# HAHHHD/mllp

Hardware: AMD Instinct MI355X
Metric: LP instances/sec (fwd+bwd) on Netlib batch; achieved HBM GB/s on CSR SpMM (higher is better)
Workload: dtype f32; 1 GPU; netlib_full: BASELINE.json configs[2], 97 instances / 1,074,147 nnz per global batch, one block-diagonal batch per GPU, one Adam step per global batch: fwd + BCE + bwd + gradient all-reduce + Adam, fp32; global_batch=97, instances_rank0=97, nnz_rank0=1074147, hip_graph=False, parallelism=dp1

## Files before the change

### include/mllp_hip.h

```cpp
#ifndef MLLP_HIP_H
#define MLLP_HIP_H

#include <stdint.h>

#ifdef __cplusplus
extern "C" {
#endif

#define MLLP_ABI_VERSION 6
#define MLLP_FEAT 16
#define MLLP_NUM_PARAMS 4721

#define MLLP_OK 0
#define MLLP_EINVAL (-1)
#define MLLP_EHIP (-2)
#define MLLP_ENOMEM (-3)
#define MLLP_ERANGE (-4)

typedef struct mllp_graph mllp_graph_t;

const char* mllp_last_error(void);
int mllp_abi_version(void);


int mllp_graph_create_host(int64_t n_inst, const int64_t* inst_m, const int64_t* inst_n,
                           const int64_t* indptr, const int32_t* indices, const double* values,
                           int32_t tier_wave, int32_t tier_block, mllp_graph_t** out);

int mllp_csr_transpose_device(int64_t n_rows, int64_t n_cols, int64_t nnz, const int32_t* d_ptr, const int32_t* d_idx,
                              const float* d_val, int32_t* d_t_ptr, int32_t* d_t_idx, float* d_t_val, void* stream);

int mllp_graph_create_device(int64_t n_inst, const int64_t* inst_ptr_m, const int64_t* inst_ptr_n,
                             int64_t nnz,
                             const int32_t* d_csr_ptr, const int32_t* d_csr_idx, const float* d_csr_val,
                             const int32_t* d_csc_ptr, const int32_t* d_csc_idx, const float* d_csc_val,
                             int32_t tier_wave, int32_t tier_block, void* stream, mllp_graph_t** out);

int mllp_graph_destroy(mllp_graph_t* g);

int mllp_graph_dims(const mllp_graph_t* g, int64_t dims[12]);

int mllp_graph_export(const mllp_graph_t* g, int which, void* host_dst, int64_t capacity_bytes);

int mllp_graph_set_path(mllp_graph_t* g, int path);

int mllp_graph_invalidate_inputs(mllp_graph_t* g);

int mllp_graph_set_values(mllp_graph_t* g, const float* d_val, void* stream);
int mllp_graph_set_values_bytes(const mllp_graph_t* g, int64_t* bytes);
int mllp_graph_scale_values(mllp_graph_t* g, const float* d_row_scale, const float* d_col_scale, void* stream);

int mllp_graph_normalize(mllp_graph_t* g, float* d_x1, float* d_x2, float rhs_cap, int flags, float* d_row_scale,
                         float* d_obj_scale, void* stream);
int mllp_normalize_row_tier(int64_t row_nnz, int* tier);

int mllp_spmm_csr_f32(const mllp_graph_t* g, int transpose, const float* d_H, float* d_Y, void* stream);
int mllp_spmm_csr_bf16(const mllp_graph_t* g, int transpose, const void* d_H_bf16, float* d_Y, void* stream);

int mllp_graph_build_spmm_copy(mllp_graph_t* g, int transpose, int where, void* stream);
int mllp_graph_drop_spmm_copy(mllp_graph_t* g, int transpose);
int mllp_graph_spmm_copy_info(const mllp_graph_t* g, int transpose, int64_t info[8]);
int mllp_graph_export_spmm_copy(const mllp_graph_t* g, int transpose, int which, void* host_dst, int64_t capacity_bytes);

int mllp_graph_build_stream_copy(mllp_graph_t* g, int transpose, int geom, int where, void* stream);
int mllp_graph_drop_stream_copy(mllp_graph_t* g, int transpose, int geom);
int mllp_graph_stream_copy_info(const mllp_graph_t* g, int transpose, int geom, int64_t info[8]);
int mllp_graph_export_stream_copy(const mllp_graph_t* g, int transpose, int geom, int which, void* host_dst,
                                  int64_t capacity_bytes);

int mllp_tiled_geometry(int variant, int32_t* rows_per_tile, int32_t* cols_per_block, int32_t* bundle_capacity);
int mllp_graph_attach_tiled(mllp_graph_t* g, int transpose, int variant, int64_t n_tiles, int64_t n_tb,
                            int32_t max_blocks_per_tile ,
                            const int32_t* d_tile_blk, const int32_t* d_blk_id, const int32_t* d_ptr2,
                            const int32_t* d_perm, const int32_t* d_ent);
int mllp_graph_build_tiled(mllp_graph_t* g, int transpose, int variant, void* stream);
int mllp_graph_tiled_info(const mllp_graph_t* g, int transpose, int variant, int64_t info[5]);
int mllp_graph_export_tiled(const mllp_graph_t* g, int transpose, int variant, int which, int32_t* d_dst, int64_t count,
                            void* stream);

int mllp_tconv_workspace_floats(const mllp_graph_t* g, int dst_is_var, int cin, int64_t* n_floats);
int mllp_tconv_fwd(const mllp_graph_t* g, int dst_is_var, int cin, const float* d_conv_params,
                   const float* d_x_src, const float* d_x_dst, float* d_h_out, float* d_ws, void* stream);
int mllp_tconv_bwd(const mllp_graph_t* g, int dst_is_var, int cin, const float* d_conv_params,
                   const float* d_x_src, const float* d_x_dst, const float* d_h_out, float* d_ws,
                   float* d_dh, float* d_dx_dst, float* d_dx_src, int accumulate,
                   float* d_param_grads, void* stream);

int mllp_gnn_workspace_bytes(const mllp_graph_t* g, int64_t* bytes);
int mllp_gnn_forward(const mllp_graph_t* g, const float* d_params, const float* d_x1, const float* d_x2,
                     void* d_ws, float* d_logits, void* stream);
int mllp_gnn_backward(const mllp_graph_t* g, const float* d_params, const float* d_x1, const float* d_x2,
                      void* d_ws, const float* d_dlogits, float* d_grads, void* stream);
int mllp_gnn_loss_step(const mllp_graph_t* g, const float* d_params, const float* d_x1, const float* d_x2,
                       const float* d_labels, float inv_batch, void* d_ws, float* d_logits,
                       float* d_loss, float* d_grads, void* stream);

int mllp_gnn_input_grads_scratch_bytes(const mllp_graph_t* g, int64_t* bytes);
int mllp_gnn_backward_inputs(const mllp_graph_t* g, const float* d_params, const float* d_x1, const float* d_x2,
                             void* d_ws, const float* d_dlogits, float* d_grads, float* d_dx1, float* d_dx2,
                             float* d_dvalues, void* d_scratch, void* stream);

int mllp_gnn_input_grads(const mllp_graph_t* g, const float* d_params, const float* d_x1, const float* d_x2,
                         void* d_ws, const float* d_dlogits, float* d_grads, float* d_dx1, float* d_dx2,
                         float* d_dvalues, void* d_scratch, void* stream);
int mllp_gnn_loss_step_inputs(const mllp_graph_t* g, const float* d_params, const float* d_x1, const float* d_x2,
                              const float* d_labels, float inv_batch, void* d_ws, float* d_logits, float* d_loss,
                              float* d_grads, float* d_dx1, float* d_dx2, float* d_dvalues, void* stream);

int mllp_weighted_loss(const mllp_graph_t* g, const float* d_logits, const float* d_labels,
                       const float* d_inst_weight, const float* d_pos_weight, float* d_dlogits,
                       float* d_inst_loss, float* d_loss, void* stream);
int mllp_balanced_pos_weight(const mllp_graph_t* g, const float* d_labels, float* d_pos_weight, void* stream);
int mllp_gnn_loss_step_weighted(const mllp_graph_t* g, const float* d_params, const float* d_x1, const float* d_x2,
                                const float* d_labels, const float* d_inst_weight, const float* d_pos_weight,
                                void* d_ws, float* d_logits, float* d_loss, float* d_inst_loss, float* d_grads,
                                float* d_dlogits, void* stream);

int mllp_adam_step(float* d_params, const float* d_grads, float* d_exp_avg, float* d_exp_avg_sq,
                   float* d_state, float eps, float grad_scale, int64_t n, void* stream);

int mllp_gnn_train_step(const mllp_graph_t* g, float* d_params, const float* d_x1, const float* d_x2,
                        const float* d_labels, float inv_batch, void* d_ws, float* d_logits, float* d_loss,
                        float* d_grads, float* d_exp_avg, float* d_exp_avg_sq, float* d_state, float eps, int flags,
                        void* stream);

int mllp_gnn_small_step_limits(int64_t limits[4]);
int mllp_gnn_small_step_fits(const mllp_graph_t* g, int* fits);
int mllp_gnn_train_step_small(const mllp_graph_t* g, float* d_params, const float* d_x1, const float* d_x2,
                              const float* d_labels, float inv_batch, void* d_ws, float* d_logits, float* d_loss,
                              float* d_grads, float* d_exp_avg, float* d_exp_avg_sq, float* d_state, float eps,
                              void* stream);

int mllp_metrics_scratch_bytes(const mllp_graph_t* g, int64_t* bytes);
int mllp_topm_metrics(const mllp_graph_t* g, const float* d_logits, const float* d_labels,
                      void* d_scratch, float* d_out, void* stream);

int mllp_topm_select(const mllp_graph_t* g, const float* d_logits, uint8_t* d_mask, int32_t* d_index,
                     float* d_stats, void* stream);
int mllp_topm_select_dense(int64_t n, int64_t m, const float* d_logits, uint8_t* d_mask, int32_t* d_index,
                           float* d_stats, void* stream);

typedef struct mllp_lp mllp_lp_t;
int mllp_mps_read(const char* path, int normalize, mllp_lp_t** out);
int mllp_lp_dims(const mllp_lp_t* lp, int64_t dims[6]);
int mllp_lp_export(const mllp_lp_t* lp, int64_t* indptr, int32_t* indices, double* values, double* coefs,
                   double* rhs, int32_t* slack_rows);
int mllp_lp_free(mllp_lp_t* lp);

int mllp_angle_num_params(int feat_dim, int64_t* out);
int mllp_angle_workspace_floats(int64_t n_nodes, int feat_dim, int64_t* out);
int mllp_angle_forward(int64_t n_nodes, int feat_dim, const float* d_cos, const float* d_x, const float* d_params,
                       float* d_ws, float* d_logits, void* stream);
int mllp_angle_backward(int64_t n_nodes, int feat_dim, const float* d_cos, const float* d_x, const float* d_params,
                        float* d_ws, const float* d_dlogits, float* d_grads, void* stream);

int mllp_angle_backward_inputs(int64_t n_nodes, int feat_dim, const float* d_cos, const float* d_x,
                               const float* d_params, float* d_ws, const float* d_dlogits, float* d_grads,
                               float* d_dx, float* d_dcos, void* stream);

#ifdef __cplusplus
}
#endif
#endif
```

### mllp_amd/_lib.py

```python
import ctypes
import os
import subprocess
from ctypes import POINTER, c_char_p, c_double, c_float, c_int, c_int32, c_int64, c_void_p

_HERE = os.path.dirname(os.path.abspath(__file__))
LIB_PATH = os.path.join(_HERE, "csrc", "libmllp_hip.so")
HEADER_PATH = os.path.abspath(os.path.join(_HERE, "..", "include", "mllp_hip.h"))

ABI_VERSION = 6

FEAT = 16
CONV_NAMES = ("gconv1_w2s", "gconv1_s2w", "gconv2_w2s", "gconv2_s2w", "gconv3_w2s", "gconv3_s2w")
CONV_CIN = (1, 1, 16, 16, 16, 16)


def conv_param_count(cin):
    return 4 * FEAT * cin + 5 * FEAT


_CONV_OFFSETS = [0]
for _cin in CONV_CIN:
    _CONV_OFFSETS.append(_CONV_OFFSETS[-1] + conv_param_count(_cin))
FC_OFFSET = _CONV_OFFSETS[-1]
NUM_PARAMS = FC_OFFSET + FEAT + 1


def conv_param_slice(conv):
    i = CONV_NAMES.index(conv) if isinstance(conv, str) else range(len(CONV_NAMES))[conv]
    return slice(_CONV_OFFSETS[i], _CONV_OFFSETS[i + 1])


class MllpError(RuntimeError):
    pass


_PROTOTYPES = {
    "mllp_last_error": (c_char_p, []),
    "mllp_abi_version": (c_int, []),
    "mllp_graph_create_host": (c_int, [c_int64, POINTER(c_int64), POINTER(c_int64), POINTER(c_int64),
                                       POINTER(c_int32), POINTER(c_double), c_int32, c_int32,
                                       POINTER(c_void_p)]),
    "mllp_graph_create_device": (c_int, [c_int64, POINTER(c_int64), POINTER(c_int64), c_int64,
                                         c_void_p, c_void_p, c_void_p, c_void_p, c_void_p, c_void_p,
                                         c_int32, c_int32, c_void_p, POINTER(c_void_p)]),
    "mllp_graph_destroy": (c_int, [c_void_p]),
    "mllp_graph_dims": (c_int, [c_void_p, POINTER(c_int64)]),
    "mllp_graph_export": (c_int, [c_void_p, c_int, c_void_p, c_int64]),
    "mllp_graph_set_path": (c_int, [c_void_p, c_int]),
    "mllp_graph_invalidate_inputs": (c_int, [c_void_p]),
    "mllp_graph_set_values": (c_int, [c_void_p, c_void_p, c_void_p]),
    "mllp_graph_set_values_bytes": (c_int, [c_void_p, POINTER(c_int64)]),
    "mllp_graph_scale_values": (c_int, [c_void_p, c_void_p, c_void_p, c_void_p]),
    "mllp_graph_normalize": (c_int, [c_void_p, c_void_p, c_void_p, c_float, c_int, c_void_p, c_void_p, c_void_p]),
    "mllp_normalize_row_tier": (c_int, [c_int64, POINTER(c_int)]),
    "mllp_graph_build_spmm_copy": (c_int, [c_void_p, c_int, c_int, c_void_p]),
    "mllp_graph_drop_spmm_copy": (c_int, [c_void_p, c_int]),
    "mllp_graph_spmm_copy_info": (c_int, [c_void_p, c_int, POINTER(c_int64)]),
    "mllp_graph_export_spmm_copy": (c_int, [c_void_p, c_int, c_int, c_void_p, c_int64]),
    "mllp_graph_build_stream_copy": (c_int, [c_void_p, c_int, c_int, c_int, c_void_p]),
    "mllp_graph_drop_stream_copy": (c_int, [c_void_p, c_int, c_int]),
    "mllp_graph_stream_copy_info": (c_int, [c_void_p, c_int, c_int, POINTER(c_int64)]),
    "mllp_graph_export_stream_copy": (c_int, [c_void_p, c_int, c_int, c_int, c_void_p, c_int64]),
    "mllp_csr_transpose_device": (c_int, [c_int64, c_int64, c_int64, c_void_p, c_void_p, c_void_p, c_void_p, c_void_p,
                                          c_void_p, c_void_p]),
    "mllp_graph_build_tiled": (c_int, [c_void_p, c_int, c_int, c_void_p]),
    "mllp_graph_tiled_info": (c_int, [c_void_p, c_int, c_int, POINTER(c_int64)]),
    "mllp_graph_export_tiled": (c_int, [c_void_p, c_int, c_int, c_int, c_void_p, c_int64, c_void_p]),
    "mllp_spmm_csr_f32": (c_int, [c_void_p, c_int, c_void_p, c_void_p, c_void_p]),
    "mllp_spmm_csr_bf16": (c_int, [c_void_p, c_int, c_void_p, c_void_p, c_void_p]),
    "mllp_angle_num_params": (c_int, [c_int, POINTER(c_int64)]),
    "mllp_angle_workspace_floats": (c_int, [c_int64, c_int, POINTER(c_int64)]),
    "mllp_angle_forward": (c_int, [c_int64, c_int, c_void_p, c_void_p, c_void_p, c_void_p, c_void_p, c_void_p]),
    "mllp_angle_backward": (c_int, [c_int64, c_int, c_void_p, c_void_p, c_void_p, c_void_p, c_void_p, c_void_p, c_void_p]),
    "mllp_angle_backward_inputs": (c_int, [c_int64, c_int, c_void_p, c_void_p, c_void_p, c_void_p, c_void_p, c_void_p,
                                           c_void_p, c_void_p, c_void_p]),
    "mllp_tiled_geometry": (c_int, [c_int, POINTER(c_int32), POINTER(c_int32), POINTER(c_int32)]),
    "mllp_graph_attach_tiled": (c_int, [c_void_p, c_int, c_int, c_int64, c_int64, c_int32, c_void_p, c_void_p, c_void_p, c_void_p,
                                        c_void_p]),
    "mllp_tconv_workspace_floats": (c_int, [c_void_p, c_int, c_int, POINTER(c_int64)]),
    "mllp_tconv_fwd": (c_int, [c_void_p, c_int, c_int, c_void_p, c_void_p, c_void_p, c_void_p, c_void_p, c_void_p]),
    "mllp_tconv_bwd": (c_int, [c_void_p, c_int, c_int, c_void_p, c_void_p, c_void_p, c_void_p, c_void_p,
                               c_void_p, c_void_p, c_void_p, c_int, c_void_p, c_void_p]),
    "mllp_gnn_workspace_bytes": (c_int, [c_void_p, POINTER(c_int64)]),
    "mllp_gnn_forward": (c_int, [c_void_p, c_void_p, c_void_p, c_void_p, c_void_p, c_void_p, c_void_p]),
    "mllp_gnn_backward": (c_int, [c_void_p, c_void_p, c_void_p, c_void_p, c_void_p, c_void_p, c_void_p, c_void_p]),
    "mllp_gnn_input_grads_scratch_bytes": (c_int, [c_void_p, POINTER(c_int64)]),
    "mllp_gnn_backward_inputs": (c_int, [c_void_p, c_void_p, c_void_p, c_void_p, c_void_p, c_void_p, c_void_p, c_void_p,
                                         c_void_p, c_void_p, c_void_p, c_void_p]),
    "mllp_gnn_input_grads": (c_int, [c_void_p, c_void_p, c_void_p, c_void_p, c_void_p, c_void_p, c_void_p, c_void_p,
                                     c_void_p, c_void_p, c_void_p, c_void_p]),
    "mllp_gnn_loss_step_inputs": (c_int, [c_void_p, c_void_p, c_void_p, c_void_p, c_void_p, c_float, c_void_p, c_void_p,
                                          c_void_p, c_void_p, c_void_p, c_void_p, c_void_p, c_void_p]),
    "mllp_gnn_loss_step": (c_int, [c_void_p, c_void_p, c_void_p, c_void_p, c_void_p, c_float, c_void_p,
                                   c_void_p, c_void_p, c_void_p, c_void_p]),
    "mllp_gnn_train_step": (c_int, [c_void_p, c_void_p, c_void_p, c_void_p, c_void_p, c_float, c_void_p, c_void_p,
                                    c_void_p, c_void_p, c_void_p, c_void_p, c_void_p, c_float, c_int, c_void_p]),
    "mllp_gnn_small_step_limits": (c_int, [POINTER(c_int64)]),
    "mllp_gnn_small_step_fits": (c_int, [c_void_p, POINTER(c_int)]),
    "mllp_gnn_train_step_small": (c_int, [c_void_p, c_void_p, c_void_p, c_void_p, c_void_p, c_float, c_void_p, c_void_p,
                                          c_void_p, c_void_p, c_void_p, c_void_p, c_void_p, c_float, c_void_p]),
    "mllp_weighted_loss": (c_int, [c_void_p, c_void_p, c_void_p, c_void_p, c_void_p, c_void_p, c_void_p, c_void_p, c_void_p]),
    "mllp_balanced_pos_weight": (c_int, [c_void_p, c_void_p, c_void_p, c_void_p]),
    "mllp_gnn_loss_step_weighted": (c_int, [c_void_p, c_void_p, c_void_p, c_void_p, c_void_p, c_void_p, c_void_p, c_void_p,
                                            c_void_p, c_void_p, c_void_p, c_void_p, c_void_p, c_void_p]),
    "mllp_adam_step": (c_int, [c_void_p, c_void_p, c_void_p, c_void_p, c_void_p, c_float, c_float, c_int64,
                               c_void_p]),
    "mllp_metrics_scratch_bytes": (c_int, [c_void_p, POINTER(c_int64)]),
    "mllp_topm_metrics": (c_int, [c_void_p, c_void_p, c_void_p, c_void_p, c_void_p, c_void_p]),
    "mllp_topm_select": (c_int, [c_void_p, c_void_p, c_void_p, c_void_p, c_void_p, c_void_p]),
    "mllp_topm_select_dense": (c_int, [c_int64, c_int64, c_void_p, c_void_p, c_void_p, c_void_p, c_void_p]),
    "mllp_mps_read": (c_int, [c_char_p, c_int, POINTER(c_void_p)]),
    "mllp_lp_dims": (c_int, [c_void_p, POINTER(c_int64)]),
    "mllp_lp_export": (c_int, [c_void_p, c_void_p, c_void_p, c_void_p, c_void_p, c_void_p, c_void_p]),
    "mllp_lp_free": (c_int, [c_void_p]),
}

_lib = None


def build(verbose=False):
    out = subprocess.run(["make", "-C", os.path.join(_HERE, "csrc"), "-j4"], capture_output=True, text=True)
    if verbose or out.returncode != 0:
        print(out.stdout[-4000:])
        print(out.stderr[-4000:])
    if out.returncode != 0:
        raise MllpError("building libmllp_hip.so failed")
    return LIB_PATH


def lib():
    global _lib
    if _lib is None:
        if not os.path.exists(LIB_PATH):
            raise MllpError(f"{LIB_PATH} not found: run `python -c 'import __graft_entry__ as g; g.build()'` "
                            "(or `make -C mllp_amd/csrc`). The product path has no CPU fallback.")
        L = ctypes.CDLL(LIB_PATH)
        for name, (res, args) in _PROTOTYPES.items():
            fn = getattr(L, name)
            fn.restype = res
            fn.argtypes = args
        if L.mllp_abi_version() != ABI_VERSION:
            raise MllpError("libmllp_hip.so ABI version mismatch")
        _lib = L
    return _lib


MLLP_ERANGE = -4


def check(rc):
    if rc != 0:
        msg = lib().mllp_last_error()
        raise MllpError(f"libmllp_hip error {rc}: {msg.decode() if msg else '?'}")


def ptr(t):
    if t is None:
        return c_void_p(0)
    return c_void_p(t.data_ptr())


def np_ptr(a, ctype):
    return a.ctypes.data_as(POINTER(ctype))


def current_stream():
    import torch
    return c_void_p(torch.cuda.current_stream().cuda_stream)
```

### mllp_amd/csrc/api.cpp

```cpp
#include <algorithm>

#include "internal.h"

namespace mllp {

static inline int64_t up16(int64_t x) { return (x + 15) & ~int64_t(15); }

static inline bool al16(const void* p) { return (reinterpret_cast<uintptr_t>(p) & 15) == 0; }
#define REQUIRE_ALIGNED16(cond) REQUIRE(cond, "misaligned pointer: " #cond " (these are accessed in 16-byte pieces)")

ConvWs conv_ws_carve(float* base, int64_t n, int cin, float** end) {
    const int64_t recw = cin == 16 ? REC_W : 8;
    float* p = base;
    auto take = [&](int64_t floats) {
        float* q = p;
        p += up16(floats);
        return q;
    };
    ConvWs w;
    w.derived = take(DERIVED_W);
    w.qp = take(n * cin);
    w.t = take(n);
    w.Z = take(n * cin);
    w.aux = take(n * 4);
// ... 350 lines not shown
                                 void* d_ws, const float* d_dlogits, float* d_grads, void* stream) {
    REQUIRE(g && d_params && d_x1 && d_x2 && d_ws && d_dlogits && d_grads, "null argument");
    REQUIRE_ALIGNED16(al16(d_ws) && al16(d_params) && al16(d_x1) && al16(d_x2));
    hipStream_t s = (hipStream_t)stream;
    ModelWs w = model_ws(g, (float*)d_ws);
    int rc;
    REQUIRE(g->ws_ptr == d_ws && g->ws_path == (use_fused(g) ? 1 : 0),
            "no mllp_gnn_forward on this workspace with the current path (mllp_graph_set_path between forward and backward?)");
    if (use_fused(g)) {
        const FusedModel m{d_params, w, d_x1, d_x2, nullptr, 0.0f, nullptr};
        if ((rc = fused_bind(const_cast<mllp_graph*>(g), d_x1, d_x2, nullptr, s))) return rc;
        if ((rc = fused_head_backward(g, m, d_dlogits, s))) return rc;
        return fused_backward(g, m, false, d_grads, nullptr, s);
    }
    if ((rc = launch_head(1, g->N, w.h3v, d_params + OFF_FC, d_params + OFF_FC + FEAT, g->inv_n, nullptr, 0.0f,
                          d_dlogits, nullptr, w.d3v, w.head_partials, s))) return rc;
    if ((rc = fork_to(s, g->aux, g->ev[1]))) return rc;
    if ((rc = launch_head_finalize(w.head_partials, head_blocks_for(g->N), d_grads + OFF_FC, nullptr, g->aux))) return rc;
    return model_backward_body(g, d_params, d_x1, d_x2, w, d_grads, s);
}

static int input_grads_body(const mllp_graph* g, const float* x1, const float* x2, const ModelWs& w, float* dx1,
                            float* dx2, float* dval, hipStream_t s) {
    int rc;
    auto edge = [&](int c, const float* x_src, int accumulate) {
        const bool t = MODEL_CONV[c].dst_is_var;
        return launch_edge_grad(t ? g->At : g->A, g->nnz, MODEL_CONV[c].cin, w.c[c], x_src, t ? g->at_pos : nullptr, dval,
                                accumulate, s);
    };
    if ((rc = launch_layer1_dst_grads(w.c[CONV_1V], w.d1v, dx1, g->N, w.c[CONV_1C], w.d1c, dx2, g->M, s))) return rc;
    if (dx1 && (rc = launch_attn_bwd_src1(g->At, w.c[CONV_1C], x1, dx1, 1, g->At.scratch, s))) return rc;
    if (dx2 && (rc = launch_attn_bwd_src1(g->A, w.c[CONV_1V], x2, dx2, 1, g->A.scratch, s))) return rc;
    if (!dval) return MLLP_OK;
    if ((rc = edge(CONV_1C, x1, 0)) || (rc = edge(CONV_2C, w.h1v, 1)) || (rc = edge(CONV_1V, x2, 1)) ||
        (rc = edge(CONV_2V, w.h1c, 1))) return rc;
    return edge(CONV_3V, w.h2c, 1);
}

extern "C" int mllp_gnn_loss_step(const mllp_graph_t* g, const float* d_params, const float* d_x1, const float* d_x2,
                                  const float* d_labels, float inv_batch, void* d_ws, float* d_logits, float* d_loss,
                                  float* d_grads, void* stream) {
    REQUIRE(g && d_params && d_x1 && d_x2 && d_labels && d_ws && d_logits && d_loss && d_grads, "null argument");
    REQUIRE_ALIGNED16(al16(d_ws) && al16(d_params) && al16(d_x1) && al16(d_x2));
    hipStream_t s = (hipStream_t)stream;
    ModelWs w = model_ws(g, (float*)d_ws);
    int rc;
    const_cast<mllp_graph*>(g)->folded_ws = const_cast<mllp_graph*>(g)->folded_params = nullptr;
    if (use_fused(g)) {
        const FusedModel m{d_params, w, d_x1, d_x2, d_labels, inv_batch, d_logits};
        if ((rc = fused_forward(const_cast<mllp_graph*>(g), m, 2, s))) return rc;
        return fused_backward(g, m, true, d_grads, d_loss, s);
    }
    if ((rc = model_forward_body(g, d_params, d_x1, d_x2, w, s))) return rc;
    if ((rc = launch_head(2, g->N, w.h3v, d_params + OFF_FC, d_params + OFF_FC + FEAT, g->inv_n, d_labels, inv_batch,
                          nullptr, d_logits, w.d3v, w.head_partials, s))) return rc;
    if ((rc = fork_to(s, g->aux, g->ev[1]))) return rc;
    if ((rc = launch_head_finalize(w.head_partials, head_blocks_for(g->N), d_grads + OFF_FC, d_loss, g->aux))) return rc;
    return model_backward_body(g, d_params, d_x1, d_x2, w, d_grads, s);
}

extern "C" int mllp_gnn_input_grads_scratch_bytes(const mllp_graph_t* g, int64_t* bytes) {
    REQUIRE(g && bytes, "null argument");
    *bytes = up16(MLLP_NUM_PARAMS) * (int64_t)sizeof(float);
    return MLLP_OK;
}

extern "C" int mllp_gnn_backward_inputs(const mllp_graph_t* g, const float* d_params, const float* d_x1,
                                        const float* d_x2, void* d_ws, const float* d_dlogits, float* d_grads,
                                        float* d_dx1, float* d_dx2, float* d_dvalues, void* d_scratch, void* stream) {
    REQUIRE(g && d_params && d_x1 && d_x2 && d_ws && d_dlogits, "null argument");
    REQUIRE_ALIGNED16(al16(d_ws) && al16(d_params) && al16(d_x1) && al16(d_x2));
    REQUIRE(g->ws_ptr == d_ws, "no mllp_gnn_forward on this workspace");
    REQUIRE(g->ws_path == 0, "the forward on this workspace ran on the fused path: input gradients need the generic "
                             "sweeps (mllp_graph_set_path(g, 1) before mllp_gnn_forward)");
    REQUIRE(!use_fused(g), "the graph's path selects the fused kernels: set path 1 between the forward and this call");
    REQUIRE(d_grads || d_scratch, "d_grads and d_scratch are both null (mllp_gnn_input_grads_scratch_bytes)");
    hipStream_t s = (hipStream_t)stream;
    mllp_graph* gm = const_cast<mllp_graph*>(g);
    int rc;
    if (d_dvalues && (rc = ensure_at_pos(gm, s))) return rc;
    float* grads = d_grads ? d_grads : (float*)d_scratch;
    if ((rc = mllp_gnn_backward(g, d_params, d_x1, d_x2, d_ws, d_dlogits, grads, stream))) return rc;
    return input_grads_body(g, d_x1, d_x2, model_ws(g, (float*)d_ws), d_dx1, d_dx2, d_dvalues, s);
}

extern "C" int mllp_gnn_input_grads(const mllp_graph_t* g, const float* d_params, const float* d_x1, const float* d_x2,
                                    void* d_ws, const float* d_dlogits, float* d_grads, float* d_dx1, float* d_dx2,
                                    float* d_dvalues, void* d_scratch, void* stream) {
    REQUIRE(g && d_params && d_x1 && d_x2 && d_ws && d_dlogits, "null argument");
    REQUIRE_ALIGNED16(al16(d_ws) && al16(d_params) && al16(d_x1) && al16(d_x2));
    REQUIRE(d_grads || d_scratch, "d_grads and d_scratch are both null (mllp_gnn_input_grads_scratch_bytes)");
    REQUIRE(g->ws_ptr == d_ws, "no mllp_gnn_forward on this workspace");
    REQUIRE(g->ws_path == (use_fused(g) ? 1 : 0),
            "the path was switched between the forward on this workspace and this call (mllp_graph_set_path)");
    if (!use_fused(g))
        return mllp_gnn_backward_inputs(g, d_params, d_x1, d_x2, d_ws, d_dlogits, d_grads, d_dx1, d_dx2, d_dvalues, d_scratch,
                                        stream);
    hipStream_t s = (hipStream_t)stream;
    int rc;
    if (d_dvalues && (rc = ensure_at_pos(const_cast<mllp_graph*>(g), s))) return rc;
    float* grads = d_grads ? d_grads : (float*)d_scratch;
    if ((rc = mllp_gnn_backward(g, d_params, d_x1, d_x2, d_ws, d_dlogits, grads, stream))) return rc;
    const ModelWs w = model_ws(g, (float*)d_ws);
    return fused_input_grads(g, FusedModel{d_params, w, d_x1, d_x2, nullptr, 0.0f, nullptr}, d_dx1, d_dx2, d_dvalues, s);
}

extern "C" int mllp_gnn_loss_step_inputs(const mllp_graph_t* g, const float* d_params, const float* d_x1,
                                         const float* d_x2, const float* d_labels, float inv_batch, void* d_ws,
                                         float* d_logits, float* d_loss, float* d_grads, float* d_dx1, float* d_dx2,
                                         float* d_dvalues, void* stream) {
    REQUIRE(g && d_params && d_x1 && d_x2 && d_labels && d_ws && d_logits && d_loss && d_grads, "null argument");
    REQUIRE_ALIGNED16(al16(d_ws) && al16(d_params) && al16(d_x1) && al16(d_x2));
    hipStream_t s = (hipStream_t)stream;
    int rc;
    if (d_dvalues && (rc = ensure_at_pos(const_cast<mllp_graph*>(g), s))) return rc;
    if ((rc = mllp_gnn_loss_step(g, d_params, d_x1, d_x2, d_labels, inv_batch, d_ws, d_logits, d_loss, d_grads, stream)))
        return rc;
    const ModelWs w = model_ws(g, (float*)d_ws);
    if (use_fused(g))
        return fused_input_grads(g, FusedModel{d_params, w, d_x1, d_x2, d_labels, inv_batch, d_logits}, d_dx1, d_dx2,
                                 d_dvalues, s);
    return input_grads_body(g, d_x1, d_x2, w, d_dx1, d_dx2, d_dvalues, s);
}

extern "C" int mllp_gnn_train_step(const mllp_graph_t* g, float* d_params, const float* d_x1, const float* d_x2,
                                   const float* d_labels, float inv_batch, void* d_ws, float* d_logits, float* d_loss,
                                   float* d_grads, float* d_exp_avg, float* d_exp_avg_sq, float* d_state, float eps,
                                   int flags, void* stream) {
    REQUIRE(g && d_params && d_x1 && d_x2 && d_labels && d_ws && d_logits && d_loss && d_grads, "null argument");
    REQUIRE_ALIGNED16(al16(d_ws) && al16(d_params) && al16(d_x1) && al16(d_x2));
    REQUIRE(d_exp_avg && d_exp_avg_sq && d_state, "null optimizer state");
    REQUIRE((flags & ~1) == 0, "flags: bit 0 = the folded weights in the workspace are current");
    hipStream_t s = (hipStream_t)stream;
    int rc;
    mllp_graph* gm = const_cast<mllp_graph*>(g);
    if (use_fused(g)) {
        ModelWs w = model_ws(g, (float*)d_ws);
        const FusedModel m{d_params, w, d_x1, d_x2, d_labels, inv_batch, d_logits};
        const bool skip = (flags & 1) != 0 && gm->folded_ws == d_ws && gm->folded_params == d_params;
        gm->folded_ws = gm->folded_params = nullptr;
        if ((rc = fused_forward(gm, m, 2, s, skip))) return rc;
        const FusedAdam a = {d_params, d_exp_avg, d_exp_avg_sq, d_state, eps, (int)MLLP_NUM_PARAMS};
        if ((rc = fused_backward(g, m, true, d_grads, d_loss, s, &a))) return rc;
        gm->folded_ws = d_ws;
        gm->folded_params = d_params;
        return MLLP_OK;
    }
    gm->folded_ws = gm->folded_params = nullptr;
    if ((rc = mllp_gnn_loss_step(g, d_params, d_x1, d_x2, d_labels, inv_batch, d_ws, d_logits, d_loss, d_grads, stream)))
        return rc;
    return launch_adam(d_params, d_grads, d_exp_avg, d_exp_avg_sq, d_state, eps, 1.0f, MLLP_NUM_PARAMS, s);
}

extern "C" int mllp_gnn_small_step_limits(int64_t limits[4]) {
    REQUIRE(limits, "null argument");
    limits[0] = SMALL_STEP_MAX_NODES; limits[1] = SMALL_STEP_MAX_NNZ;
    limits[2] = SMALL_STEP_THREADS; limits[3] = SMALL_STEP_LDS_BYTES;
    return MLLP_OK;
}

static std::string small_step_excess(const mllp_graph* g) {
    if (g->M + g->N > SMALL_STEP_MAX_NODES)
        return "the graph has " + std::to_string(g->M + g->N) + " nodes, the limit is " + std::to_string(SMALL_STEP_MAX_NODES);
    if (g->nnz > SMALL_STEP_MAX_NNZ)
        return "the graph has " + std::to_string(g->nnz) + " nonzeros, the limit is " + std::to_string(SMALL_STEP_MAX_NNZ);
    return std::string();
}

extern "C" int mllp_gnn_small_step_fits(const mllp_graph_t* g, int* fits) {
    REQUIRE(g && fits, "null argument");
    *fits = small_step_excess(g).empty() ? 1 : 0;
    return MLLP_OK;
}

extern "C" int mllp_gnn_train_step_small(const mllp_graph_t* g, float* d_params, const float* d_x1, const float* d_x2,
                                         const float* d_labels, float inv_batch, void* d_ws, float* d_logits,
                                         float* d_loss, float* d_grads, float* d_exp_avg, float* d_exp_avg_sq,
                                         float* d_state, float eps, void* stream) {
    REQUIRE(g && d_params && d_x1 && d_x2 && d_labels && d_ws && d_logits && d_loss && d_grads, "null argument");
    REQUIRE_ALIGNED16(al16(d_ws) && al16(d_params) && al16(d_x1) && al16(d_x2));
    const int n_opt = (d_exp_avg != nullptr) + (d_exp_avg_sq != nullptr) + (d_state != nullptr);
    REQUIRE(n_opt == 0 || n_opt == 3, "optimizer state: give d_exp_avg, d_exp_avg_sq and d_state, or none of them (loss step)");
    const std::string excess = small_step_excess(g);
    REQUIRE(excess.empty(), excess + " (mllp_gnn_small_step_limits)");
    mllp_graph* gm = const_cast<mllp_graph*>(g);
    gm->ws_ptr = nullptr;
    gm->ws_path = -1;
    gm->folded_ws = gm->folded_params = nullptr;
    return launch_small_step(g, d_params, d_x1, d_x2, d_labels, inv_batch, model_ws(g, (float*)d_ws), d_logits, d_loss,
                             d_grads, d_exp_avg, d_exp_avg_sq, d_state, eps, (hipStream_t)stream);
}

extern "C" int mllp_adam_step(float* d_params, const float* d_grads, float* d_exp_avg, float* d_exp_avg_sq,
                              float* d_state, float eps, float grad_scale, int64_t n, void* stream) {
    REQUIRE(d_params && d_grads && d_exp_avg && d_exp_avg_sq && d_state, "null argument");
    REQUIRE(n > 0 && n < (int64_t)1 << 30, "bad parameter count");
    return launch_adam(d_params, d_grads, d_exp_avg, d_exp_avg_sq, d_state, eps, grad_scale, n, (hipStream_t)stream);
}

extern "C" int mllp_metrics_scratch_bytes(const mllp_graph_t* g, int64_t* bytes) {
    REQUIRE(g && bytes, "null argument");
    *bytes = 16;
    return MLLP_OK;
}

extern "C" int mllp_topm_metrics(const mllp_graph_t* g, const float* d_logits, const float* d_labels, void* d_scratch,
                                 float* d_out, void* stream) {
    REQUIRE(g && d_logits && d_labels && d_out, "null argument");
    return launch_topm_metrics(g, d_logits, d_labels, d_scratch, d_out, (hipStream_t)stream);
}

extern "C" int mllp_topm_select(const mllp_graph_t* g, const float* d_logits, uint8_t* d_mask, int32_t* d_index,
                                float* d_stats, void* stream) {
    REQUIRE(g && d_logits, "null argument");
    REQUIRE(d_mask || d_index || d_stats, "null outputs: at least one of mask, index, stats");
    return launch_topm_select(g->inst_ptr_n, g->inst_ptr_m, g->n_inst, 0, 0, d_logits, d_mask, d_index, d_stats,
                              (hipStream_t)stream);
}

extern "C" int mllp_topm_select_dense(int64_t n, int64_t m, const float* d_logits, uint8_t* d_mask, int32_t* d_index,
                                      float* d_stats, void* stream) {
    REQUIRE(n >= 0 && m >= 0, "bad size: n and m must not be negative");
    REQUIRE(d_logits, "null argument");
    REQUIRE(d_mask || d_index || d_stats, "null outputs: at least one of mask, index, stats");
    if (n > INT32_MAX || m > INT32_MAX) return fail(MLLP_ERANGE, "mllp_topm_select_dense: sizes exceed int32 indexing");
    return launch_topm_select(nullptr, nullptr, 1, (int)n, (int)m, d_logits, d_mask, d_index, d_stats,
                              (hipStream_t)stream);
}
```

### mllp_amd/csrc/fused_kernels.hip

```cpp
#include <algorithm>
#include <vector>

#include "device_utils.h"
#include "host_graph.h"
#include "internal.h"
#include "node_bodies.h"

namespace mllp {

typedef float f32x4m __attribute__((ext_vector_type(4)));

#ifdef MLLP_TIMING_BUILD
static int g_fused_abl = [] {
    const char* e = getenv("MLLP_FUSED_ABL");
    return e ? atoi(e) : 0;
}();
#define FUSED_ABL(bit) ((J.abl & (bit)) != 0)
__device__ unsigned long long g_fused_stamps[8192 * 8];
__device__ unsigned long long g_fused_stamps1[8192 * 8];
#define FUSED_STAMP(k)                                                                      \
    {                                                                                       \
        __builtin_amdgcn_sched_barrier(0);                                                  \
        const unsigned long long now_ = __builtin_amdgcn_s_memtime();                       \
        __builtin_amdgcn_sched_barrier(0);                                                  \
        stamp_sum[k] += now_ - stamp_last;                                                  \
        stamp_last = now_;                                                                  \
    }
#else
#define FUSED_ABL(bit) false
#define FUSED_STAMP(k)
#endif

constexpr int FT = 768;
constexpr int FW = FT / 64;
constexpr int RT = 1024;
constexpr int MAXJOBS = 2;

constexpr int NP = FUSED_NP;
static_assert(NP == FUSED_PARTS, "partition count");

struct PartTiers {
    int row0, n_block, n_wave, n_group, n_base;
};
struct ItemsDev {
    const int* __restrict__ sptr;
    const int2* __restrict__ sent;
    const float2* __restrict__ sax;
    int n_dst, nnz;
    const int* __restrict__ order;
    int nw, L;
    PartTiers part[NP];
};

static ItemsDev items_dev(const FusedOrient& o, int which) {
    const bool scalar = which == 1;
    ItemsDev d;
    d.order = which == 0 ? o.lst16 : which == 1 ? o.lst1 : o.lst16x2;
    d.nw = which == 0 ? o.nw16 : which == 1 ? o.nw1 : o.nw16x2;
    d.L = which == 0 ? o.L16 : which == 1 ? o.L1 : o.L16x2;
    d.sptr = o.sptr;
    d.sent = reinterpret_cast<const int2*>(o.sent);
    d.sax = reinterpret_cast<const float2*>(o.sax);
    d.n_dst = o.n_dst;
    d.nnz = o.nnz;
    for (int q = 0; q < NP; ++q) {
        const FusedTiersDev& t = scalar ? o.t1[q] : o.t16[q];
        d.part[q].row0 = o.row0[q];
        d.part[q].n_block = t.n_block; d.part[q].n_wave = t.n_wave; d.part[q].n_group = t.n_group; d.part[q].n_base = t.n_base;
    }
    return d;
}

constexpr int TS = 17;
constexpr int TILE = 16 * TS;
__device__ __forceinline__ void tile_put(float* tile, const float4& v, int lane) {
    float* d = tile + (lane >> 2) * TS + 4 * (lane & 3);
    d[0] = v.x; d[1] = v.y; d[2] = v.z; d[3] = v.w;
}
__device__ __forceinline__ float4 tile_get(const float* tile, int lane) {
    const float* d = tile + (lane >> 2) * TS + 4 * (lane & 3);
    return make_float4(d[0], d[1], d[2], d[3]);
}
__device__ __forceinline__ void tile_rows(const float* tile, int lane, float (&a)[4]) {
#pragma unroll
    for (int s = 0; s < 4; ++s) a[s] = tile[(lane & 15) * TS + 4 * s + (lane >> 4)];
}
__device__ __forceinline__ void tile_cols(const float* tile, int lane, float (&a)[4]) {
#pragma unroll
    for (int s = 0; s < 4; ++s) a[s] = tile[(4 * s + (lane >> 4)) * TS + (lane & 15)];
}
__device__ __forceinline__ void tile_put_result(float* tile, const f32x4m& d, int lane) {
#pragma unroll
    for (int j = 0; j < 4; ++j) tile[(4 * (lane >> 4) + j) * TS + (lane & 15)] = d[j];
}
struct MatB {
    float w[4];
};
__device__ __forceinline__ MatB matB(const float* __restrict__ W, int ld, int lane) {
    MatB b;
#pragma unroll
    for (int s = 0; s < 4; ++s) b.w[s] = W[(lane & 15) * ld + 4 * s + (lane >> 4)];
    return b;
}
__device__ __forceinline__ MatB matB_t(const float* __restrict__ W, int ld, int lane) {
    MatB b;
#pragma unroll
    for (int s = 0; s < 4; ++s) b.w[s] = W[(4 * s + (lane >> 4)) * ld + (lane & 15)];
    return b;
}
__device__ __forceinline__ void matB_store(float* lds, const MatB& b, int lane) {
    *reinterpret_cast<float4*>(lds + 4 * lane) = make_float4(b.w[0], b.w[1], b.w[2], b.w[3]);
}
__device__ __forceinline__ MatB matB_lds(const float* lds, int lane) {
    const float4 v = *reinterpret_cast<const float4*>(lds + 4 * lane);
    MatB b;
    b.w[0] = v.x; b.w[1] = v.y; b.w[2] = v.z; b.w[3] = v.w;
    return b;
}
__device__ __forceinline__ f32x4m mat_apply(const float (&a)[4], const MatB& b, f32x4m acc) {
#pragma unroll
    for (int s = 0; s < 4; ++s) acc = __builtin_amdgcn_mfma_f32_16x16x4f32(a[s], b.w[s], acc, 0, 0, 0);
    return acc;
}
__device__ __forceinline__ f32x4m splat4(float v) { return (f32x4m){v, v, v, v}; }
__device__ __forceinline__ float4 lds4(const float* p) { return *reinterpret_cast<const float4*>(p); }
__device__ __forceinline__ float4 f4zero() { return make_float4(0.f, 0.f, 0.f, 0.f); }
__device__ __forceinline__ float4 f4scale(const float4& a, float s) { return make_float4(a.x * s, a.y * s, a.z * s, a.w * s); }
__device__ __forceinline__ float4 f4add(const float4& a, const float4& b) { return make_float4(a.x + b.x, a.y + b.y, a.z + b.z, a.w + b.w); }
template <int J>
__device__ __forceinline__ int quad_bcast_i(int v) {
    return __builtin_amdgcn_mov_dpp(v, J * 0x55, 0xF, 0xF, true);
}
__device__ __forceinline__ float wave_sum(float v) {
    v = row16_sum(v);
    v += __shfl_xor(v, 16, 64);
    v += __shfl_xor(v, 32, 64);
    return v;
}


struct RowSlot {
    int row;
    int first;
    int stride;
    int end;
    int mode;
    bool writer;
};
struct SlotReq {
    int row, q, stride, mode;
    int sb, se;
    bool writer;
};
template <int G>
struct Geo {
    static constexpr int U = 64 / G;
    static constexpr int QG = 4;
    static constexpr int RG = U / QG;
};
template <int G>
__device__ __forceinline__ int wave_items(const PartTiers& s) {
    return s.n_wave + (s.n_group + Geo<G>::RG - 1) / Geo<G>::RG + (s.n_base + Geo<G>::U - 1) / Geo<G>::U;
}
template <int G>
__device__ __forceinline__ SlotReq item_request(const ItemsDev& S, const PartTiers& s, int item, int lane) {
    constexpr int U = Geo<G>::U, QG = Geo<G>::QG, RG = Geo<G>::RG;
    const int unit = lane / G;
    const int n_gitems = (s.n_group + RG - 1) / RG;
    SlotReq r;
    bool valid;
    if (item < s.n_wave) {
        r.row = s.row0 + s.n_block + item; r.q = unit; r.stride = U; r.mode = 2; valid = true; r.writer = unit == 0;
    } else if (item < s.n_wave + n_gitems) {
        const int rl = (item - s.n_wave) * RG + unit / QG;
        valid = rl < s.n_group;
        r.row = s.row0 + s.n_block + s.n_wave + rl; r.q = unit % QG; r.stride = QG; r.mode = 1; r.writer = valid && r.q == 0;
    } else {
        const int rl = (item - s.n_wave - n_gitems) * U + unit;
        valid = rl < s.n_base;
        r.row = s.row0 + s.n_block + s.n_wave + s.n_group + rl; r.q = 0; r.stride = 1; r.mode = 0; r.writer = valid;
    }
    const int rc = valid ? r.row : 0;
    r.sb = S.sptr[rc];
    r.se = S.sptr[rc + 1];
    if (!valid) r.row = -1;
    return r;
}
__device__ __forceinline__ SlotReq empty_request() {
    SlotReq r;
    r.row = -1; r.q = 0; r.stride = 1; r.mode = 0; r.sb = 0; r.se = 0; r.writer = false;
    return r;
}
__device__ __forceinline__ RowSlot slot_make(const SlotReq& q) {
    RowSlot r;
    r.row = q.row; r.first = q.sb + q.q; r.stride = q.stride; r.end = q.row >= 0 ? q.se : 0; r.mode = q.mode; r.writer = q.writer;
    asm volatile("" : "+v"(r.first), "+v"(r.end));
    return r;
}
template <int G>
__device__ __forceinline__ RowSlot item_slot(const ItemsDev& S, const PartTiers& s, int item, int lane) {
    return slot_make(item_request<G>(S, s, item, lane));
}
template <int G>
__device__ __forceinline__ RowSlot block_slot(const ItemsDev& s, int k, int tid) {
    RowSlot r;
    r.row = k;
    r.mode = 3;
    r.first = s.sptr[k] + tid / G;
    r.stride = FT / G;
    r.end = s.sptr[k + 1];
    r.writer = tid < G;
    return r;
}
__device__ __forceinline__ int slot_count(const RowSlot& r) {
    return r.first < r.end ? (r.end - r.first + r.stride - 1) / r.stride : 0;
}
__device__ __forceinline__ RowSlot empty_slot() {
    RowSlot r;
    r.row = -1; r.first = 0; r.stride = 1; r.end = 0; r.mode = 0; r.writer = false;
    return r;
}
struct WaveList {
    const int* p;
    int L, chunk;
};
__device__ __forceinline__ WaveList wave_list(const ItemsDev& S, int px, int gw) {
    WaveList w;
    w.L = gw < S.nw ? S.L : 0;
    w.p = S.order + ((size_t)px * S.nw + gw) * S.L;
    w.chunk = -1;
    return w;
}
__device__ __forceinline__ void wave_list_chunk(WaveList& w, int c0, int lane) {
    int v = c0 + lane < w.L ? w.p[c0 + lane] : -1;
    asm volatile("s_waitcnt vmcnt(0)" : "+v"(v));
    w.chunk = v;
}
__device__ __forceinline__ int wave_list_get(const WaveList& w, int k) {
    return k < 64 ? __builtin_amdgcn_readlane(w.chunk, __builtin_amdgcn_readfirstlane(k)) : -1;
}
template <int LPE>
__device__ __forceinline__ int2 first_entries(const ItemsDev& s, const RowSlot& r, int part) {
    const int k = LPE == 4 ? part : (part & 1);
    return k < slot_count(r) ? s.sent[r.first + k * r.stride] : make_int2(0, 0);
}
template <int LPE>
__device__ __forceinline__ int2 first_entries_any(const ItemsDev& s, const RowSlot& r, int part) {
    const int k = LPE == 4 ? part : (part & 1);
    return s.sent[max(min(r.first + k * r.stride, s.nnz - 1), 0)];
}
__device__ __forceinline__ float shared_sum4(float v, int mode) {
    return mode == 1 ? quads_sum<16>(v) : quads_sum<64>(v);
}
__device__ __forceinline__ float shared_max4(float v, int mode) {
    return mode == 1 ? quads_max<16>(v) : quads_max<64>(v);
}
__device__ __forceinline__ float shared_sum1(float v, int mode) { return mode == 1 ? quad_sum(v) : wave_sum(v); }
__device__ __forceinline__ float shared_max1(float v, int mode) { return mode == 1 ? quad_max(v) : group_max<64>(v); }

struct FwdJob16 {
    ItemsDev s;
    const float* __restrict__ x_src;
    const float* __restrict__ x_dst;
    const float* __restrict__ D;
    ConvParams p;
    float* __restrict__ h;
    float* __restrict__ Z;
    float* __restrict__ aux;
    int head;
    const float* __restrict__ fcw;
    const float* __restrict__ fcb;
    const float* __restrict__ inv_n;
    const float* __restrict__ labels;
    const int* __restrict__ perm;
    float inv_batch;
    float* __restrict__ logits;
    float* __restrict__ g_out;
    float* __restrict__ head_part;
#ifdef MLLP_TIMING_BUILD
    int abl;
#endif
};
struct FwdLaunch16 {
    FwdJob16 job[MAXJOBS];
    int n_jobs;
};
struct FwdW16 {
    float BPq[256], BWv[256], BWs[256];
    float pq0[16], Pt[16], bv[16], we[16], bs[16], fcw[16];
    float pt0, fcb;
};
struct SoftState {
    float4 Z;
    float m, L, u;
};

struct Gather4 {
    float4 x0, x1, x2, x3;
    float a0, a1, a2, a3;
};
__device__ __forceinline__ void gather4_issue(const ItemsDev& s, const float* __restrict__ X, const RowSlot& r, int n_mine,
                                              int k0, int part, int2& en, Gather4& g) {
    const int colm = en.x;
    const float am = __int_as_float(en.y);
    const int c0 = quad_bcast_i<0>(colm), c1 = quad_bcast_i<1>(colm), c2 = quad_bcast_i<2>(colm), c3 = quad_bcast_i<3>(colm);
    g.a0 = quad_bcast<0>(am); g.a1 = quad_bcast<1>(am); g.a2 = quad_bcast<2>(am); g.a3 = quad_bcast<3>(am);
    g.x0 = ld4(X + (size_t)c0 * 16 + 4 * part);
    g.x1 = ld4(X + (size_t)c1 * 16 + 4 * part);
    g.x2 = ld4(X + (size_t)c2 * 16 + 4 * part);
    g.x3 = ld4(X + (size_t)c3 * 16 + 4 * part);
    const int kn = k0 + 4 + part;
    en = kn < n_mine ? s.sent[r.first + kn * r.stride] : make_int2(0, 0);
}

__device__ __forceinline__ void fwd16_step(const Gather4& g, int k0, int n_mine, const float4& qp, float t, SoftState& st) {
    const bool ok0 = k0 < n_mine, ok1 = k0 + 1 < n_mine, ok2 = k0 + 2 < n_mine, ok3 = k0 + 3 < n_mine;
    const float d0 = ok0 ? fmaf(g.a0, t, quad_sum(dot4(qp, g.x0))) : NEG_BIG;
    const float d1 = ok1 ? fmaf(g.a1, t, quad_sum(dot4(qp, g.x1))) : NEG_BIG;
    const float d2 = ok2 ? fmaf(g.a2, t, quad_sum(dot4(qp, g.x2))) : NEG_BIG;
    const float d3 = ok3 ? fmaf(g.a3, t, quad_sum(dot4(qp, g.x3))) : NEG_BIG;
// ... 95 lines not shown
    asm volatile("" : "+v"(nx.xd.x), "+v"(nx.xd.y), "+v"(nx.xd.z), "+v"(nx.xd.w), "+v"(nx.en.x), "+v"(nx.en.y),
                      "+v"(nx.lrow), "+v"(nx.q.sb), "+v"(nx.q.se));
    fwd16_flush(J, pend, part);
    const int lrow_cur = lrow;
    FUSED_STAMP(3)

    if (r.mode >= 1) soft_merge(st, r.mode);
    if (r.mode == 3) {
        const int wave = threadIdx.x >> 6;
        if (lane < 4) {
            float* slot = merge_lds + wave * 20;
            if (part == 0) *reinterpret_cast<float4*>(slot) = make_float4(st.m, st.L, st.u, 0.0f);
            *reinterpret_cast<float4*>(slot + 4 + 4 * part) = st.Z;
        }
        __syncthreads();
        float M = NEG_BIG;
        for (int w = 0; w < FW; ++w) M = fmaxf(M, merge_lds[w * 20]);
        float L = 0.0f, u = 0.0f;
        float4 Z = f4zero();
        for (int w = 0; w < FW; ++w) {
            const float4 hd = lds4(merge_lds + w * 20);
            const float f = exp_acc(hd.x - M);
            L = fmaf(f, hd.y, L);
            u = fmaf(f, hd.z, u);
            fma4(f, lds4(merge_lds + w * 20 + 4 + 4 * part), Z);
        }
        st.m = M; st.L = L; st.u = u; st.Z = Z;
        __syncthreads();
    }
    const bool writer = r.writer;
    const float rinv = 1.0f / (st.L + 1e-16f);
    const float S = st.L * rinv, un = st.u * rinv;
    const float4 zn = f4scale(st.Z, rinv);
    float4 o;
    {
        float ax_[4], az_[4];
        tile_rows(tiles, lane, ax_);
        tile_put(tiles + TILE, zn, lane);
        tile_rows(tiles + TILE, lane, az_);
        if (!FUSED_ABL(512))
        tile_put_result(tiles + 2 * TILE,
                        mat_apply(ax_, matB_lds(W.BWs, lane), mat_apply(az_, matB_lds(W.BWv, lane), splat4(0.0f))), lane);
        o = tile_get(tiles + 2 * TILE, lane);
    }
    o = f4add(o, lds4(W.bs + 4 * part));
    fma4(S, lds4(W.bv + 4 * part), o);
    fma4(un, lds4(W.we + 4 * part), o);
    const float4 hv = make_float4(fmaxf(o.x, 0.0f), fmaxf(o.y, 0.0f), fmaxf(o.z, 0.0f), fmaxf(o.w, 0.0f));
    FUSED_STAMP(4)
    pend.row = writer ? r.row : -1;
    pend.zn = zn; pend.hv = hv; pend.lrow = lrow_cur;
    pend.aux = make_float4(un, st.L > 0.0f ? st.m : 0.0f, rinv, S);
    pend.z = 0.0f; pend.g = f4zero();
    if (J.head) {
        const float4 fw = lds4(W.fcw + 4 * part);
        const float z = quad_sum(dot4(hv, fw)) + W.fcb;
        pend.z = z;
        if (J.head == 2 && writer) {
            const float y = J.labels[r.row];
            const float wn = J.inv_n[r.row] * J.inv_batch;
            const float e = expf(-fabsf(z));
            const float sig = z >= 0.0f ? 1.0f / (1.0f + e) : e / (1.0f + e);
            const float dz = wn * (sig - y);
            pend.g = make_float4(hv.x > 0.0f ? dz * fw.x : 0.0f, hv.y > 0.0f ? dz * fw.y : 0.0f,
                                 hv.z > 0.0f ? dz * fw.z : 0.0f, hv.w > 0.0f ? dz * fw.w : 0.0f);
            fma4(dz, hv, ha.w);
            if (part == 0) {
                ha.b += dz;
                ha.l += wn * (fmaxf(z, 0.0f) - z * y + log1pf(e));
            }
        }
    }
    FUSED_STAMP(5)
}

template <int NW>
__device__ __forceinline__ void head_partials_store(HeadAcc& ha, float* head_lds, float* head_part, int tid) {
    const int lane = tid & 63, wave = tid >> 6;
    ha.w.x = quads_sum<64>(ha.w.x); ha.w.y = quads_sum<64>(ha.w.y);
    ha.w.z = quads_sum<64>(ha.w.z); ha.w.w = quads_sum<64>(ha.w.w);
    ha.b = wave_sum(ha.b);
    ha.l = wave_sum(ha.l);
    if (lane < 4) {
        float* d = head_lds + wave * 18 + 4 * lane;
        d[0] = ha.w.x; d[1] = ha.w.y; d[2] = ha.w.z; d[3] = ha.w.w;
    }
    if (lane == 0) { head_lds[wave * 18 + 16] = ha.b; head_lds[wave * 18 + 17] = ha.l; }
    __syncthreads();
    if (tid < 18) {
        float v = 0.0f;
        for (int w = 0; w < NW; ++w) v += head_lds[w * 18 + tid];
        head_part[(size_t)blockIdx.x * 18 + tid] = v;
    }
}

__global__ __launch_bounds__(FT) void fused_fwd16_kernel(FwdLaunch16 A) {
    __shared__ FwdW16 Ws_[MAXJOBS];
    __shared__ float merge_lds[FW * 20];
    __shared__ float head_lds[FW * 18];
    __shared__ float tiles_[FW * 3 * TILE];
    const int tid = threadIdx.x, lane = tid & 63, wave = tid >> 6, part = lane & 3;
    for (int j = 0; j < A.n_jobs; ++j) {
        const FwdJob16& J = A.job[j];
        FwdW16& W = Ws_[j];
        if (wave == 0) matB_store(W.BPq, matB(J.D + OFF_PQ, 16, lane), lane);
        if (wave == 1) matB_store(W.BWv, matB(J.p.Wv, 16, lane), lane);
        if (wave == 2) matB_store(W.BWs, matB(J.p.Ws, 16, lane), lane);
        if (tid < 16) {
            W.pq0[tid] = J.D[OFF_PQ0 + tid];
            W.Pt[tid] = J.D[OFF_PT + tid];
            W.bv[tid] = J.p.bv[tid];
            W.we[tid] = J.p.we[tid];
            W.bs[tid] = J.p.bs[tid];
            W.fcw[tid] = J.head ? J.fcw[tid] : 0.0f;
        }
        if (tid == 0) {
            W.pt0 = J.D[OFF_PT0];
            W.fcb = J.head ? J.fcb[0] : 0.0f;
        }
    }
    __syncthreads();
    float* tiles = tiles_ + wave * 3 * TILE;
    HeadAcc ha;
    ha.w = f4zero(); ha.b = 0.0f; ha.l = 0.0f;
#ifdef MLLP_TIMING_BUILD
    unsigned long long stamp_sum[8] = {0, 0, 0, 0, 0, 0, 0, 0};
    unsigned long long stamp_last = __builtin_amdgcn_s_memtime();
    const unsigned long long stamp_begin = stamp_last;
#define STAMP_ARGS , stamp_sum, stamp_last
#else
#define STAMP_ARGS
#endif
    const int px = blockIdx.x % NP, bi = blockIdx.x / NP, gp = gridDim.x / NP;
    const int gw = bi * FW + wave;
    float* head_part = nullptr;
    for (int j = 0; j < A.n_jobs; ++j) {
        const FwdJob16& J = A.job[j];
        const PartTiers P = J.s.part[px];
        if (J.head == 2) head_part = J.head_part;
        const RowSlot none = empty_slot();
        FwdPending pend;
        pend.row = -1;
        for (int k = bi; k < P.n_block; k += gp) {
            const RowSlot r = block_slot<4>(J.s, P.row0 + k, tid);
            const float4 xd = ld4(J.x_dst + (size_t)r.row * 16 + 4 * part);
            int2 en = first_entries<4>(J.s, r, part);
            const int lrow = J.head ? J.perm[r.row] : 0;
            FwdNext nx;
            fwd16_row(J, Ws_[j], P, r, xd, en, lrow, empty_request(), -1, nx, pend, part, lane, merge_lds, tiles, ha STAMP_ARGS);
        }
        WaveList wl = wave_list(J.s, px, gw);
        for (int c0 = 0; c0 < wl.L; c0 += 64) {
            wave_list_chunk(wl, c0, lane);
            int it = wave_list_get(wl, 0), it1 = wave_list_get(wl, 1);
            RowSlot r = it >= 0 ? item_slot<4>(J.s, P, it, lane) : none;
            float4 xd = r.row >= 0 ? ld4(J.x_dst + (size_t)r.row * 16 + 4 * part) : f4zero();
            int2 en = first_entries<4>(J.s, r, part);
            int lrow = (J.head && r.row >= 0) ? J.perm[r.row] : 0;
            SlotReq q1 = item_request<4>(J.s, P, max(it1, 0), lane);
            if (it1 < 0) q1.row = -1;
            asm volatile("" : "+v"(xd.x), "+v"(xd.y), "+v"(xd.z), "+v"(xd.w), "+v"(en.x), "+v"(en.y), "+v"(lrow),
                              "+v"(q1.sb), "+v"(q1.se));
            for (int k = 0; it >= 0; ++k) {
                const int it2 = wave_list_get(wl, k + 2);
                FwdNext nx;
                fwd16_row(J, Ws_[j], P, r, xd, en, lrow, q1, it2, nx, pend, part, lane, merge_lds, tiles, ha STAMP_ARGS);
#ifdef MLLP_TIMING_BUILD
                stamp_sum[7] += 1;
#endif
                r = nx.r; xd = nx.xd; en = nx.en; lrow = nx.lrow; q1 = nx.q;
                it = it1; it1 = it2;
            }
        }
        fwd16_flush(J, pend, part);
    }
#ifdef MLLP_TIMING_BUILD
    if (lane == 0 && A.job[0].abl >= 0) {
        stamp_sum[6] = __builtin_amdgcn_s_memtime() - stamp_begin;
        unsigned long long* d = g_fused_stamps + (size_t)(blockIdx.x * FW + wave) * 8;
        for (int k = 0; k < 8; ++k) d[k] = stamp_sum[k];
    }
#endif
    if (head_part) head_partials_store<FW>(ha, head_lds, head_part, tid);
}

struct FwdJob1 {
    ItemsDev s;
    const float* __restrict__ x_dst;
    const float* __restrict__ D;
    ConvParams p;
    float* __restrict__ h;
    float* __restrict__ Z;
    float* __restrict__ aux;
};
struct FwdLaunch1 {
    FwdJob1 job[MAXJOBS];
    int n_jobs;
};
struct alignas(16) FwdW1 {
    float wv[16], ws[16], bv[16], we[16], bs[16];
    float pq, pq0, pt, pt0;
};
struct Soft1 {
    float m, L, u, Z;
};

struct Ent8 {
    float2 e0, e1, e2, e3, e4, e5, e6, e7;
};
__device__ __forceinline__ void ent8_load(const ItemsDev& s, const RowSlot& r, int k0, Ent8& E) {
    const int last = max(s.nnz - 1, 0), d = r.stride, b = r.first + k0 * d;
    E.e0 = s.sax[min(b, last)];         E.e1 = s.sax[min(b + d, last)];
    E.e2 = s.sax[min(b + 2 * d, last)]; E.e3 = s.sax[min(b + 3 * d, last)];
    E.e4 = s.sax[min(b + 4 * d, last)]; E.e5 = s.sax[min(b + 5 * d, last)];
    E.e6 = s.sax[min(b + 6 * d, last)]; E.e7 = s.sax[min(b + 7 * d, last)];
}

__device__ __forceinline__ void fwd1_step4(const float2& e0, const float2& e1, const float2& e2, const float2& e3, int k0,
                                           int n_mine, float qp, float t, Soft1& st) {
    const bool ok0 = k0 < n_mine, ok1 = k0 + 1 < n_mine, ok2 = k0 + 2 < n_mine, ok3 = k0 + 3 < n_mine;
    const float d0 = ok0 ? fmaf(qp, e0.y, e0.x * t) : NEG_BIG, d1 = ok1 ? fmaf(qp, e1.y, e1.x * t) : NEG_BIG;
    const float d2 = ok2 ? fmaf(qp, e2.y, e2.x * t) : NEG_BIG, d3 = ok3 ? fmaf(qp, e3.y, e3.x * t) : NEG_BIG;
    const float mi = fmaxf(fmaxf(d0, d1), fmaxf(d2, d3));
    if (__any(mi > st.m)) {
        const float mn = fmaxf(st.m, mi);
        const float sc = exp_acc(st.m - mn);
        st.L *= sc; st.u *= sc; st.Z *= sc;
        st.m = mn;
    }
    const float p0 = ok0 ? exp_acc(d0 - st.m) : 0.0f, p1 = ok1 ? exp_acc(d1 - st.m) : 0.0f;
    const float p2 = ok2 ? exp_acc(d2 - st.m) : 0.0f, p3 = ok3 ? exp_acc(d3 - st.m) : 0.0f;
    st.L += (p0 + p1) + (p2 + p3);
    st.u = fmaf(p0, e0.x, fmaf(p1, e1.x, fmaf(p2, e2.x, fmaf(p3, e3.x, st.u))));
    st.Z = fmaf(p0, e0.y, fmaf(p1, e1.y, fmaf(p2, e2.y, fmaf(p3, e3.y, st.Z))));
}
__device__ __forceinline__ void fwd1_edges(const ItemsDev& s, const RowSlot& r, float qp, float t, Soft1& st, Ent8& E) {
    const int n_mine = slot_count(r);
    for (int k0 = 0; __any(k0 < n_mine); k0 += 8) {
        Ent8 N;
        const bool more = __any(k0 + 8 < n_mine);
        if (more) ent8_load(s, r, k0 + 8, N);
        fwd1_step4(E.e0, E.e1, E.e2, E.e3, k0, n_mine, qp, t, st);
        if (__any(k0 + 4 < n_mine)) fwd1_step4(E.e4, E.e5, E.e6, E.e7, k0 + 4, n_mine, qp, t, st);
        if (more) E = N;
    }
}

__device__ __forceinline__ void fwd1_row(const FwdJob1& J, const FwdW1& W, const RowSlot& r, int lane, float* merge_lds) {
    Ent8 E;
    ent8_load(J.s, r, 0, E);
    const float x = J.x_dst[max(r.row, 0)];
    const float qp = fmaf(W.pq, x, W.pq0), t = fmaf(W.pt, x, W.pt0);
    Soft1 st;
    st.m = NEG_BIG; st.L = 0.0f; st.u = 0.0f; st.Z = 0.0f;
    fwd1_edges(J.s, r, qp, t, st, E);
    if (r.mode >= 1) {
        const float M = shared_max1(st.m, r.mode);
        const float f = exp_acc(st.m - M);
        st.m = M;
        st.L = shared_sum1(st.L * f, r.mode);
        st.u = shared_sum1(st.u * f, r.mode);
        st.Z = shared_sum1(st.Z * f, r.mode);
    }
    if (r.mode == 3) {
        const int wave = threadIdx.x >> 6;
        if (lane == 0) *reinterpret_cast<float4*>(merge_lds + wave * 4) = make_float4(st.m, st.L, st.u, st.Z);
        __syncthreads();
        float M = NEG_BIG;
        for (int w = 0; w < FW; ++w) M = fmaxf(M, merge_lds[w * 4]);
        float L = 0.0f, u = 0.0f, Z = 0.0f;
        for (int w = 0; w < FW; ++w) {
            const float4 hd = lds4(merge_lds + w * 4);
            const float f = exp_acc(hd.x - M);
            L = fmaf(f, hd.y, L);
            u = fmaf(f, hd.z, u);
            Z = fmaf(f, hd.w, Z);
        }
        st.m = M; st.L = L; st.u = u; st.Z = Z;
        __syncthreads();
    }
    const float rinv = 1.0f / (st.L + 1e-16f);
    const float S = st.L * rinv, un = st.u * rinv, zn = st.Z * rinv;
    if (r.mode == 0) {
        const int base_row = __builtin_amdgcn_readfirstlane(r.row);
        const int n_valid = __popcll(__ballot(r.row >= 0));
#pragma unroll
        for (int q = 0; q < 4; ++q) {
            const int idx = lane + 64 * q, row_l = idx >> 2, ch = (idx & 3) * 4;
            const float Sr = __shfl(S, row_l, 64), ur = __shfl(un, row_l, 64), zr = __shfl(zn, row_l, 64), xr = __shfl(x, row_l, 64);
            float4 v = lds4(W.bs + ch);
            fma4(Sr, lds4(W.bv + ch), v);
            fma4(ur, lds4(W.we + ch), v);
            fma4(zr, lds4(W.wv + ch), v);
            fma4(xr, lds4(W.ws + ch), v);
            if (row_l < n_valid)
                *reinterpret_cast<float4*>(J.h + (size_t)(base_row + row_l) * 16 + ch) =
                    make_float4(fmaxf(v.x, 0.0f), fmaxf(v.y, 0.0f), fmaxf(v.z, 0.0f), fmaxf(v.w, 0.0f));
        }
        if (r.writer) {
            J.Z[r.row] = zn;
            reinterpret_cast<float4*>(J.aux)[r.row] = make_float4(un, st.L > 0.0f ? st.m : 0.0f, rinv, S);
        }
        return;
    }
    if (!r.writer) return;
    float o[16];
#pragma unroll
    for (int c = 0; c < 16; ++c) {
        float v = W.bs[c];
        v = fmaf(S, W.bv[c], v);
        v = fmaf(un, W.we[c], v);
        v = fmaf(W.wv[c], zn, v);
        v = fmaf(W.ws[c], x, v);
        o[c] = fmaxf(v, 0.0f);
    }
    float4* hd = reinterpret_cast<float4*>(J.h + (size_t)r.row * 16);
    hd[0] = make_float4(o[0], o[1], o[2], o[3]);
    hd[1] = make_float4(o[4], o[5], o[6], o[7]);
    hd[2] = make_float4(o[8], o[9], o[10], o[11]);
    hd[3] = make_float4(o[12], o[13], o[14], o[15]);
    J.Z[r.row] = zn;
    reinterpret_cast<float4*>(J.aux)[r.row] = make_float4(un, st.L > 0.0f ? st.m : 0.0f, rinv, S);
}

__global__ __launch_bounds__(FT) void fused_fwd1_kernel(FwdLaunch1 A) {
    __shared__ FwdW1 Ws_[MAXJOBS];
    __shared__ float merge_lds[FW * 4];
    const int tid = threadIdx.x, lane = tid & 63, wave = tid >> 6;
    for (int j = 0; j < A.n_jobs; ++j) {
        const FwdJob1& J = A.job[j];
        FwdW1& W = Ws_[j];
        if (tid < 16) {
            W.wv[tid] = J.p.Wv[tid]; W.ws[tid] = J.p.Ws[tid];
            W.bv[tid] = J.p.bv[tid]; W.we[tid] = J.p.we[tid]; W.bs[tid] = J.p.bs[tid];
        }
        if (tid == 0) {
            W.pq = J.D[OFF_PQ]; W.pq0 = J.D[OFF_PQ0]; W.pt = J.D[OFF_PT]; W.pt0 = J.D[OFF_PT0];
        }
    }
    __syncthreads();
    const int px = blockIdx.x % NP, bi = blockIdx.x / NP, gp = gridDim.x / NP;
    const int gw = bi * FW + wave;
    for (int j = 0; j < A.n_jobs; ++j) {
        const FwdJob1& J = A.job[j];
        const PartTiers P = J.s.part[px];
        for (int k = bi; k < P.n_block; k += gp)
            fwd1_row(J, Ws_[j], block_slot<1>(J.s, P.row0 + k, tid), lane, merge_lds);
        WaveList wl = wave_list(J.s, px, gw);
        for (int c0 = 0; c0 < wl.L; c0 += 64) {
            wave_list_chunk(wl, c0, lane);
            int it = wave_list_get(wl, 0);
            SlotReq q = item_request<1>(J.s, P, max(it, 0), lane);
            for (int k = 0; it >= 0; ++k) {
                const int itn = wave_list_get(wl, k + 1);
                const RowSlot r = slot_make(q);
                q = item_request<1>(J.s, P, max(itn, 0), lane);
                fwd1_row(J, Ws_[j], r, lane, merge_lds);
                it = itn;
            }
        }
    }
}

struct BwdJob16 {
    ItemsDev s;
    const float* __restrict__ x_src;
    const float* __restrict__ x_dst;
    const float* __restrict__ D;
    ConvParams p;
    const float* __restrict__ h;
    const float* __restrict__ dh_a;
    const float* __restrict__ dh_b;
    const float* __restrict__ Z;
    const float* __restrict__ aux;
    float* __restrict__ rec;
    float* __restrict__ dx_dst;
    int mask_dx;
    float* __restrict__ stats;
#ifdef MLLP_TIMING_BUILD
    int abl;
#endif
};
struct BwdLaunch16 {
    BwdJob16 job[MAXJOBS];
    int n_jobs;
};
struct BwdW16 {
    float BWvT[256], BPq[256], BWsT[256], BPqT[256];
    float pq0[16], Pt[16], Pb[16], bv[16], we[16];
    float pt0;
};
struct BwdState {
    float4 dq;
    float ds, dt;
};

__device__ __forceinline__ void bwd16_step(const Gather4& g, int k0, int n_mine, const float4& qp, const float4& gv, float t,
                                           float m, float rinv, float ge, float cc, BwdState& st) {
#define MLLP_BWD_SLOT(K, A_, X_)                                                           \
    {                                                                                      \
        const float l_ = fmaf(A_, t, quad_sum(dot4(qp, X_)));                              \
        const float al_ = (k0 + K < n_mine) ? exp_acc(l_ - m) * rinv : 0.0f;               \
        const float dl_ = al_ * (quad_sum(dot4(gv, X_)) + fmaf(A_, ge, cc));               \
        st.ds += dl_;                                                                      \
        st.dt = fmaf(dl_, A_, st.dt);                                                      \
        fma4(dl_, X_, st.dq);                                                              \
    }
    MLLP_BWD_SLOT(0, g.a0, g.x0)
    MLLP_BWD_SLOT(1, g.a1, g.x1)
    MLLP_BWD_SLOT(2, g.a2, g.x2)
    MLLP_BWD_SLOT(3, g.a3, g.x3)
#undef MLLP_BWD_SLOT
}

struct BwdRow {
    float4 ga, gb, h, x, Z, ax;
};
__device__ __forceinline__ void bwd16_fetch(const BwdJob16& J, const RowSlot& r, int part, BwdRow& d) {
    const bool have = r.row >= 0;
    const size_t ro = have ? (size_t)r.row * 16 + 4 * part : 0;
    const float4 z4 = f4zero();
    d.ga = have ? ld4(J.dh_a + ro) : z4;
    d.gb = (J.dh_b && have) ? ld4(J.dh_b + ro) : z4;
    d.h = (J.h && have) ? ld4(J.h + ro) : make_float4(1.0f, 1.0f, 1.0f, 1.0f);
    d.x = have ? ld4(J.x_dst + ro) : z4;
    d.Z = have ? ld4(J.Z + ro) : z4;
    d.ax = have ? reinterpret_cast<const float4*>(J.aux)[r.row] : z4;
}

constexpr int TB_G = 0, TB_X = 1, TB_Z = 2, TB_DQ = 3, TB_SC = 4, TB_E = 5, TB_N = 6;

__device__ __forceinline__ void bwd16_row(const BwdJob16& J, const BwdW16& W, const PartTiers& P, const RowSlot& r,
                                          BwdRow& rd, int2& en, int itn, RowSlot& rn, int part,
                                          int lane, float* merge_lds, float* tiles, f32x4m (&acc)[STAT_TILES]) {
    const bool have = r.row >= 0;
    const bool writer = r.writer;
    const int n_mine = FUSED_ABL(1) ? 0 : slot_count(r);
    Gather4 gt;
    gather4_issue(J.s, J.x_src, r, n_mine, 0, part, en, gt);
    SlotReq qn = item_request<4>(J.s, P, max(itn, 0), lane);
    if (itn < 0) qn.row = -1;
    const int xpos = (rd.x.x > 0.0f ? 1 : 0) | (rd.x.y > 0.0f ? 2 : 0) | (rd.x.z > 0.0f ? 4 : 0) | (rd.x.w > 0.0f ? 8 : 0);
    float4 qp, gv;
    float t, m, rinv, ge, cc;
    {
        float4 g = f4add(rd.ga, rd.gb);
        g = make_float4(rd.h.x > 0.0f ? g.x : 0.0f, rd.h.y > 0.0f ? g.y : 0.0f, rd.h.z > 0.0f ? g.z : 0.0f, rd.h.w > 0.0f ? g.w : 0.0f);
        const float4 xd = rd.x, Zn = rd.Z, ax = rd.ax;
        float ag_[4], ax_[4];
        tile_put(tiles + TB_G * TILE, g, lane);
        tile_put(tiles + TB_X * TILE, xd, lane);
        tile_put(tiles + TB_Z * TILE, Zn, lane);
        tile_put(tiles + TB_E * TILE, (have && part == 0) ? make_float4(1.0f, ax.w, ax.x, 0.0f) : f4zero(), lane);
        tile_rows(tiles + TB_G * TILE, lane, ag_);
        tile_rows(tiles + TB_X * TILE, lane, ax_);
        if (!FUSED_ABL(16)) {
            tile_put_result(tiles + TB_DQ * TILE, mat_apply(ag_, matB_lds(W.BWvT, lane), splat4(0.0f)), lane);
            tile_put_result(tiles + TB_SC * TILE, mat_apply(ax_, matB_lds(W.BPq, lane), splat4(W.pq0[lane & 15])), lane);
        }
        gv = tile_get(tiles + TB_DQ * TILE, lane);
        qp = tile_get(tiles + TB_SC * TILE, lane);
        t = quad_sum(dot4(lds4(W.Pt + 4 * part), xd)) + W.pt0;
        ge = quad_sum(dot4(g, lds4(W.we + 4 * part)));
        const float gb = quad_sum(dot4(g, lds4(W.bv + 4 * part)));
        const float Dn = quad_sum(dot4(gv, Zn)) + gb * ax.w + ge * ax.x;
        cc = gb - Dn;
        m = ax.y; rinv = ax.z;
    }
    BwdState st;
    st.dq = f4zero(); st.ds = 0.0f; st.dt = 0.0f;
    for (int k0 = 0;;) {
        bwd16_step(gt, k0, n_mine, qp, gv, t, m, rinv, ge, cc, st);
        k0 += 4;
        if (!__any(k0 < n_mine)) break;
        gather4_issue(J.s, J.x_src, r, n_mine, k0, part, en, gt);
    }
    if (writer && J.rec && !FUSED_ABL(8)) {
        float* rr = J.rec + (size_t)r.row * REC_W;
        *reinterpret_cast<float4*>(rr + 4 * part) = qp;
        *reinterpret_cast<float4*>(rr + 16 + 4 * part) = gv;
        if (part == 0) *reinterpret_cast<float4*>(rr + 32) = make_float4(t, m, rinv, ge);
        if (part == 1) *reinterpret_cast<float4*>(rr + 36) = make_float4(cc, 0.0f, 0.0f, 0.0f);
    }
    rn = slot_make(qn);
    bwd16_fetch(J, rn, part, rd);
    en = first_entries<4>(J.s, rn, part);
    if (r.mode >= 1) {
        st.ds = shared_sum4(st.ds, r.mode);
        st.dt = shared_sum4(st.dt, r.mode);
        st.dq.x = shared_sum4(st.dq.x, r.mode); st.dq.y = shared_sum4(st.dq.y, r.mode);
        st.dq.z = shared_sum4(st.dq.z, r.mode); st.dq.w = shared_sum4(st.dq.w, r.mode);
    }
    if (r.mode == 3) {
        const int wave = threadIdx.x >> 6;
        if (lane < 4) {
            float* slot = merge_lds + wave * 20;
            if (part == 0) *reinterpret_cast<float4*>(slot) = make_float4(st.ds, st.dt, 0.0f, 0.0f);
            *reinterpret_cast<float4*>(slot + 4 + 4 * part) = st.dq;
        }
        __syncthreads();
        float ds = 0.0f, dt = 0.0f;
        float4 dq = f4zero();
        for (int w = 0; w < FW; ++w) {
            ds += merge_lds[w * 20];
            dt += merge_lds[w * 20 + 1];
            dq = f4add(dq, lds4(merge_lds + w * 20 + 4 + 4 * part));
        }
        st.ds = ds; st.dt = dt; st.dq = dq;
        __syncthreads();
        if (threadIdx.x >= 64) return;
    }
    tile_put(tiles + TB_DQ * TILE, st.dq, lane);
    if (J.dx_dst && !FUSED_ABL(4)) {
        float ag_[4], adq_[4];
        tile_rows(tiles + TB_G * TILE, lane, ag_);
        tile_rows(tiles + TB_DQ * TILE, lane, adq_);
        tile_put_result(tiles + TB_SC * TILE,
                        mat_apply(adq_, matB_lds(W.BPqT, lane), mat_apply(ag_, matB_lds(W.BWsT, lane), splat4(0.0f))), lane);
        float4 v = tile_get(tiles + TB_SC * TILE, lane);
        fma4(st.ds, lds4(W.Pb + 4 * part), v);
        fma4(st.dt, lds4(W.Pt + 4 * part), v);
        if (J.mask_dx) {
            if (!(xpos & 1)) v.x = 0.0f;
            if (!(xpos & 2)) v.y = 0.0f;
            if (!(xpos & 4)) v.z = 0.0f;
            if (!(xpos & 8)) v.w = 0.0f;
        }
        if (writer) *reinterpret_cast<float4*>(J.dx_dst + (size_t)r.row * 16 + 4 * part) = v;
    }
    if (FUSED_ABL(2)) return;
    if (r.mode >= 1 && !writer) {
        const float4 z4 = f4zero();
        tile_put(tiles + TB_G * TILE, z4, lane);
        tile_put(tiles + TB_X * TILE, z4, lane);
        tile_put(tiles + TB_Z * TILE, z4, lane);
        tile_put(tiles + TB_E * TILE, z4, lane);
        tile_put(tiles + TB_DQ * TILE, z4, lane);
    }
    tile_put(tiles + TB_SC * TILE, (writer && part == 0) ? make_float4(st.ds, st.dt, 0.0f, 0.0f) : f4zero(), lane);
    float cg[4], cdq[4], csc[4], cx[4], cz[4], ce[4];
    if (FUSED_ABL(64)) {
        for (int s = 0; s < 4; ++s) { cg[s] = cdq[s] = csc[s] = cx[s] = cz[s] = ce[s] = (float)lane; }
    } else {
    tile_cols(tiles + TB_G * TILE, lane, cg);
    tile_cols(tiles + TB_DQ * TILE, lane, cdq);
    tile_cols(tiles + TB_SC * TILE, lane, csc);
    tile_cols(tiles + TB_X * TILE, lane, cx);
    tile_cols(tiles + TB_Z * TILE, lane, cz);
    tile_cols(tiles + TB_E * TILE, lane, ce);
    }
    if (FUSED_ABL(32)) {
        asm volatile("" :: "v"(cg[0]), "v"(cdq[1]), "v"(csc[2]), "v"(cx[3]), "v"(cz[0]), "v"(ce[1]));
        return;
    }
#pragma unroll
    for (int s = 0; s < 4; ++s) {
        acc[0] = __builtin_amdgcn_mfma_f32_16x16x4f32(cg[s], cx[s], acc[0], 0, 0, 0);
        acc[1] = __builtin_amdgcn_mfma_f32_16x16x4f32(cg[s], cz[s], acc[1], 0, 0, 0);
        acc[2] = __builtin_amdgcn_mfma_f32_16x16x4f32(cg[s], ce[s], acc[2], 0, 0, 0);
        acc[3] = __builtin_amdgcn_mfma_f32_16x16x4f32(cdq[s], cx[s], acc[3], 0, 0, 0);
        acc[4] = __builtin_amdgcn_mfma_f32_16x16x4f32(cdq[s], ce[s], acc[4], 0, 0, 0);
        acc[5] = __builtin_amdgcn_mfma_f32_16x16x4f32(csc[s], cx[s], acc[5], 0, 0, 0);
        acc[6] = __builtin_amdgcn_mfma_f32_16x16x4f32(csc[s], ce[s], acc[6], 0, 0, 0);
    }
}

__global__ __launch_bounds__(FT) void fused_bwd16_kernel(BwdLaunch16 A) {
    __shared__ BwdW16 Ws_[MAXJOBS];
    __shared__ float merge_lds[FW * 20];
    __shared__ float tiles_[FW * TB_N * TILE];
    const int tid = threadIdx.x, lane = tid & 63, wave = tid >> 6, part = lane & 3;
    for (int j = 0; j < A.n_jobs; ++j) {
        const BwdJob16& J = A.job[j];
        BwdW16& W = Ws_[j];
        if (wave == 0) matB_store(W.BWvT, matB_t(J.p.Wv, 16, lane), lane);
        if (wave == 1) matB_store(W.BPq, matB(J.D + OFF_PQ, 16, lane), lane);
        if (wave == 2) matB_store(W.BWsT, matB_t(J.p.Ws, 16, lane), lane);
        if (wave == 3) matB_store(W.BPqT, matB_t(J.D + OFF_PQ, 16, lane), lane);
        if (tid < 16) {
            W.pq0[tid] = J.D[OFF_PQ0 + tid];
            W.Pt[tid] = J.D[OFF_PT + tid];
            W.Pb[tid] = J.D[OFF_PB + tid];
            W.bv[tid] = J.p.bv[tid];
            W.we[tid] = J.p.we[tid];
        }
        if (tid == 0) W.pt0 = J.D[OFF_PT0];
    }
    __syncthreads();
    float* tiles = tiles_ + wave * TB_N * TILE;
    const int px = blockIdx.x % NP, bi = blockIdx.x / NP, gp = gridDim.x / NP;
    const int gw = bi * FW + wave;
    for (int j = 0; j < A.n_jobs; ++j) {
        const BwdJob16& J = A.job[j];
        const PartTiers P = J.s.part[px];
        f32x4m acc[STAT_TILES];
#pragma unroll
        for (int i = 0; i < STAT_TILES; ++i) acc[i] = splat4(0.0f);
        const RowSlot none = empty_slot();
        for (int k = bi; k < P.n_block; k += gp) {
            const RowSlot r = block_slot<4>(J.s, P.row0 + k, tid);
            BwdRow rd;
            bwd16_fetch(J, r, part, rd);
            int2 en = first_entries<4>(J.s, r, part);
            RowSlot rn;
            bwd16_row(J, Ws_[j], P, r, rd, en, -1, rn, part, lane, merge_lds, tiles, acc);
        }
        WaveList wl = wave_list(J.s, px, gw);
        for (int c0 = 0; c0 < wl.L; c0 += 64) {
            wave_list_chunk(wl, c0, lane);
            int it = wave_list_get(wl, 0);
            RowSlot r = it >= 0 ? item_slot<4>(J.s, P, it, lane) : none;
            BwdRow rd;
            bwd16_fetch(J, r, part, rd);
            int2 en = first_entries<4>(J.s, r, part);
            for (int k = 0; it >= 0; ++k) {
                const int itn = wave_list_get(wl, k + 1);
                RowSlot rn;
                bwd16_row(J, Ws_[j], P, r, rd, en, itn, rn, part, lane, merge_lds, tiles, acc);
                r = rn;
                it = itn;
            }
        }
        __syncthreads();
        float* red = tiles_;
#pragma unroll
        for (int i = 0; i < STAT_TILES; ++i) {
#pragma unroll
            for (int q = 0; q < 4; ++q) red[wave * 256 + ((lane >> 4) * 4 + q) * 16 + (lane & 15)] = acc[i][q];
            __syncthreads();
            if (tid < 256) {
                float v = 0.0f;
                for (int w = 0; w < FW; ++w) v += red[w * 256 + tid];
                J.stats[(size_t)blockIdx.x * STAT_FLOATS + i * 256 + tid] = v;
            }
            __syncthreads();
        }
    }
}

struct SrcJob16 {
    ItemsDev s;
    const float* __restrict__ x;
    const float* __restrict__ rec;
    float* __restrict__ dx;
    const float* __restrict__ addp;
    float addw;
    int mask;
};
struct SrcLaunch16 {
    SrcJob16 job[MAXJOBS];
    int n_jobs;
};

__device__ __forceinline__ void src16_row(const SrcJob16& J, const RowSlot& r, float4& xj_io, int2& en, const SlotReq& qn,
                                          RowSlot& rn, int part, int lane, float* merge_lds) {
    const int n_mine = slot_count(r);
    const float4 xj = xj_io;
    const float4 addv = ld4(J.addp + (size_t)max(r.row, 0) * 16 + 4 * part);
    float4 acc = f4zero();
    for (int k0 = 0; __any(k0 < n_mine); k0 += 2) {
        const int colm = en.x;
        const float am = __int_as_float(en.y);
        const int c0 = quad_bcast_i<0>(colm), c1 = quad_bcast_i<1>(colm);
        const float a0 = quad_bcast<0>(am), a1 = quad_bcast<1>(am);
        const bool ok0 = k0 < n_mine, ok1 = k0 + 1 < n_mine;
        const float* rr0 = J.rec + (size_t)c0 * REC_W;
        const float* rr1 = J.rec + (size_t)c1 * REC_W;
        const float4 q0 = ld4(rr0 + 4 * part), g0 = ld4(rr0 + 16 + 4 * part), s0 = ld4(rr0 + 32);
        const float cc0 = rr0[36];
        const float4 q1 = ld4(rr1 + 4 * part), g1 = ld4(rr1 + 16 + 4 * part), s1 = ld4(rr1 + 32);
        const float cc1 = rr1[36];
        const int kn = k0 + 2 + (part & 1);
        en = kn < n_mine ? J.s.sent[r.first + kn * r.stride] : make_int2(0, 0);
        {
            const float l = fmaf(a0, s0.x, quad_sum(dot4(q0, xj)));
            const float al = ok0 ? exp_acc(l - s0.y) * s0.z : 0.0f;
            const float dl = al * (quad_sum(dot4(g0, xj)) + fmaf(a0, s0.w, cc0));
            fma4(al, g0, acc);
            fma4(dl, q0, acc);
        }
        {
            const float l = fmaf(a1, s1.x, quad_sum(dot4(q1, xj)));
            const float al = ok1 ? exp_acc(l - s1.y) * s1.z : 0.0f;
            const float dl = al * (quad_sum(dot4(g1, xj)) + fmaf(a1, s1.w, cc1));
            fma4(al, g1, acc);
            fma4(dl, q1, acc);
        }
    }
    rn = slot_make(qn);
    xj_io = rn.row >= 0 ? ld4(J.x + (size_t)rn.row * 16 + 4 * part) : f4zero();
    en = first_entries<2>(J.s, rn, part);
    if (r.mode >= 1) {
        acc.x = shared_sum4(acc.x, r.mode); acc.y = shared_sum4(acc.y, r.mode);
        acc.z = shared_sum4(acc.z, r.mode); acc.w = shared_sum4(acc.w, r.mode);
    }
    if (r.mode == 3) {
        const int wave = threadIdx.x >> 6;
        if (lane < 4) *reinterpret_cast<float4*>(merge_lds + wave * 20 + 4 * part) = acc;
        __syncthreads();
        float4 v = f4zero();
        for (int w = 0; w < FW; ++w) v = f4add(v, lds4(merge_lds + w * 20 + 4 * part));
        acc = v;
        __syncthreads();
    }
    fma4(J.addw, addv, acc);
    if (J.mask) {
        if (!(xj.x > 0.0f)) acc.x = 0.0f;
        if (!(xj.y > 0.0f)) acc.y = 0.0f;
        if (!(xj.z > 0.0f)) acc.z = 0.0f;
        if (!(xj.w > 0.0f)) acc.w = 0.0f;
    }
    if (r.writer) *reinterpret_cast<float4*>(J.dx + (size_t)r.row * 16 + 4 * part) = acc;
}

__global__ __launch_bounds__(FT) void fused_src16_kernel(SrcLaunch16 A) {
    __shared__ float merge_lds[FW * 20];
    const int tid = threadIdx.x, lane = tid & 63, wave = tid >> 6, part = lane & 3;
    const int px = blockIdx.x % NP, bi = blockIdx.x / NP, gp = gridDim.x / NP;
    const int gw = bi * FW + wave;
    for (int j = 0; j < A.n_jobs; ++j) {
        const SrcJob16& J = A.job[j];
        const PartTiers P = J.s.part[px];
        const RowSlot none = empty_slot();
        for (int k = bi; k < P.n_block; k += gp) {
            const RowSlot r = block_slot<4>(J.s, P.row0 + k, tid);
            float4 xj = ld4(J.x + (size_t)r.row * 16 + 4 * part);
            int2 en = first_entries<2>(J.s, r, part);
            RowSlot rn;
            src16_row(J, r, xj, en, empty_request(), rn, part, lane, merge_lds);
        }
        WaveList wl = wave_list(J.s, px, gw);
        for (int c0 = 0; c0 < wl.L; c0 += 64) {
            wave_list_chunk(wl, c0, lane);
            int it = wave_list_get(wl, 0);
            RowSlot r = it >= 0 ? item_slot<4>(J.s, P, it, lane) : none;
            float4 xj = r.row >= 0 ? ld4(J.x + (size_t)r.row * 16 + 4 * part) : f4zero();
            int2 en = first_entries<2>(J.s, r, part);
            for (int k = 0; it >= 0; ++k) {
                const int itn = wave_list_get(wl, k + 1);
                const SlotReq qn = itn >= 0 ? item_request<4>(J.s, P, itn, lane) : empty_request();
                RowSlot rn;
                src16_row(J, r, xj, en, qn, rn, part, lane, merge_lds);
                r = rn;
                it = itn;
            }
        }
    }
}

struct BwdJob1 {
    ItemsDev s;
    const float* __restrict__ x_dst;
    const float* __restrict__ D;
    ConvParams p;
    const float* __restrict__ g;
    const float* __restrict__ Z;
    const float* __restrict__ aux;
    float* __restrict__ stats;
};
struct BwdLaunch1 {
    BwdJob1 job[MAXJOBS];
    int n_jobs;
};
struct alignas(16) BwdW1 {
    float wv[16], bv[16], we[16];
    float pq, pq0, pt, pt0;
};
constexpr int G1S = 17, R1S = 9;
constexpr int TILE1 = 64 * G1S + 64 * R1S;

__device__ __forceinline__ void bwd1_row(const BwdJob1& J, const BwdW1& W, const RowSlot& r, int lane, float* merge_lds,
                                         float* tiles, f32x4m& accT, float (&accS)[6]
#ifdef MLLP_TIMING_BUILD
                                         , unsigned long long (&stamp_sum)[8], unsigned long long& stamp_last
#endif
) {
    FUSED_STAMP(0)
    const bool writer = r.writer;
    Ent8 E;
    ent8_load(J.s, r, 0, E);
    const int rowc = max(r.row, 0);
    float gv = 0.0f, ge = 0.0f, gb = 0.0f;
    if (r.mode == 0) {
        const int base_row = __builtin_amdgcn_readfirstlane(r.row);
        const int n_valid = __popcll(__ballot(r.row >= 0));
        float* gt = tiles;
        float* rt = tiles + 64 * G1S;
#pragma unroll
        for (int q = 0; q < 4; ++q) {
            const int idx = lane + 64 * q, row_l = idx >> 2, ch = (idx & 3) * 4;
            const size_t ro = (size_t)min(base_row + row_l, J.s.n_dst - 1) * 16 + ch;
            const float4 a = ld4(J.g + ro);
            const bool on = row_l < n_valid;
            const float4 g = make_float4(on ? a.x : 0.0f, on ? a.y : 0.0f, on ? a.z : 0.0f, on ? a.w : 0.0f);
            const float pv = quad_sum(dot4(g, lds4(W.wv + ch))), pe = quad_sum(dot4(g, lds4(W.we + ch)));
            const float pb = quad_sum(dot4(g, lds4(W.bv + ch)));
            float* d = gt + row_l * G1S + ch;
            d[0] = g.x; d[1] = g.y; d[2] = g.z; d[3] = g.w;
            if ((lane & 3) == 0) { rt[row_l * R1S + 5] = pv; rt[row_l * R1S + 6] = pe; rt[row_l * R1S + 7] = pb; }
        }
        gv = rt[lane * R1S + 5]; ge = rt[lane * R1S + 6]; gb = rt[lane * R1S + 7];
    } else {
        const float4* pa = reinterpret_cast<const float4*>(J.g + (size_t)rowc * 16);
        float* gt = tiles + lane * G1S;
#pragma unroll
        for (int q = 0; q < 4; ++q) {
            const float4 a = pa[q];
            const float g0 = a.x, g1 = a.y, g2 = a.z, g3 = a.w;
            gv = fmaf(g0, W.wv[4 * q], fmaf(g1, W.wv[4 * q + 1], fmaf(g2, W.wv[4 * q + 2], fmaf(g3, W.wv[4 * q + 3], gv))));
            ge = fmaf(g0, W.we[4 * q], fmaf(g1, W.we[4 * q + 1], fmaf(g2, W.we[4 * q + 2], fmaf(g3, W.we[4 * q + 3], ge))));
            gb = fmaf(g0, W.bv[4 * q], fmaf(g1, W.bv[4 * q + 1], fmaf(g2, W.bv[4 * q + 2], fmaf(g3, W.bv[4 * q + 3], gb))));
            gt[4 * q] = writer ? g0 : 0.0f;
            gt[4 * q + 1] = writer ? g1 : 0.0f;
            gt[4 * q + 2] = writer ? g2 : 0.0f;
            gt[4 * q + 3] = writer ? g3 : 0.0f;
        }
    }
    const float x = J.x_dst[rowc];
    const float Zn = J.Z[rowc];
    const float4 ax = reinterpret_cast<const float4*>(J.aux)[rowc];
    {
        float* rt = tiles + 64 * G1S + lane * R1S;
        rt[0] = writer ? x : 0.0f;
        rt[1] = writer ? Zn : 0.0f;
        rt[2] = writer ? 1.0f : 0.0f;
        rt[3] = writer ? ax.w : 0.0f;
        rt[4] = writer ? ax.x : 0.0f;
    }
    const float Dn = gv * Zn + gb * ax.w + ge * ax.x;
    const float cc = gb - Dn;
    const float qp = fmaf(W.pq, x, W.pq0), t = fmaf(W.pt, x, W.pt0);
    float ds = 0.0f, dt = 0.0f, dq = 0.0f;
    const int n_mine = slot_count(r);
    FUSED_STAMP(1)
    for (int k0 = 0; __any(k0 < n_mine); k0 += 8) {
        Ent8 N;
        const bool more = __any(k0 + 8 < n_mine);
        if (more) ent8_load(J.s, r, k0 + 8, N);
#define MLLP_BWD1_SLOT(K, E_)                                                              \
    {                                                                                      \
        const float l_ = fmaf(qp, E_.y, E_.x * t);                                         \
        const float al_ = (K) < n_mine ? exp_acc(l_ - ax.y) * ax.z : 0.0f;                 \
        const float dl_ = al_ * fmaf(gv, E_.y, fmaf(E_.x, ge, cc));                        \
        ds += dl_;                                                                         \
        dt = fmaf(dl_, E_.x, dt);                                                          \
        dq = fmaf(dl_, E_.y, dq);                                                          \
    }
        MLLP_BWD1_SLOT(k0, E.e0)
        MLLP_BWD1_SLOT(k0 + 1, E.e1)
        MLLP_BWD1_SLOT(k0 + 2, E.e2)
        MLLP_BWD1_SLOT(k0 + 3, E.e3)
        if (__any(k0 + 4 < n_mine)) {
            MLLP_BWD1_SLOT(k0 + 4, E.e4)
            MLLP_BWD1_SLOT(k0 + 5, E.e5)
            MLLP_BWD1_SLOT(k0 + 6, E.e6)
            MLLP_BWD1_SLOT(k0 + 7, E.e7)
        }
#undef MLLP_BWD1_SLOT
        if (more) E = N;
    }
    FUSED_STAMP(2)
    if (r.mode >= 1) {
        ds = shared_sum1(ds, r.mode); dt = shared_sum1(dt, r.mode); dq = shared_sum1(dq, r.mode);
    }
    if (r.mode == 3) {
        const int wave = threadIdx.x >> 6;
        if (lane == 0) *reinterpret_cast<float4*>(merge_lds + wave * 4) = make_float4(ds, dt, dq, 0.0f);
        __syncthreads();
        float a = 0.0f, b = 0.0f, c = 0.0f;
        for (int w = 0; w < FW; ++w) {
            const float4 v = lds4(merge_lds + w * 4);
            a += v.x; b += v.y; c += v.z;
        }
        ds = a; dt = b; dq = c;
        __syncthreads();
        if (threadIdx.x >= 64) return;
    }
    if (writer) {
        accS[0] = fmaf(dq, x, accS[0]);
        accS[1] += dq;
        accS[2] = fmaf(ds, x, accS[2]);
        accS[3] = fmaf(dt, x, accS[3]);
        accS[4] += ds;
        accS[5] += dt;
    }
    FUSED_STAMP(3)
    const float* gt = tiles;
    const float* rt = tiles + 64 * G1S;
    const int kq = lane >> 4, rr = lane & 15;
#pragma unroll
    for (int s = 0; s < 16; ++s) {
        const float a = gt[(4 * s + kq) * G1S + rr];
        const float b = rr < 5 ? rt[(4 * s + kq) * R1S + rr] : 0.0f;
        accT = __builtin_amdgcn_mfma_f32_16x16x4f32(a, b, accT, 0, 0, 0);
    }
    FUSED_STAMP(4)
}

__global__ __launch_bounds__(FT) void fused_bwd1_kernel(BwdLaunch1 A) {
    __shared__ BwdW1 Ws_[MAXJOBS];
    __shared__ float merge_lds[FW * 4];
    __shared__ float tiles_[FW * TILE1];
    const int tid = threadIdx.x, lane = tid & 63, wave = tid >> 6;
    for (int j = 0; j < A.n_jobs; ++j) {
        const BwdJob1& J = A.job[j];
        BwdW1& W = Ws_[j];
        if (tid < 16) { W.wv[tid] = J.p.Wv[tid]; W.bv[tid] = J.p.bv[tid]; W.we[tid] = J.p.we[tid]; }
        if (tid == 0) { W.pq = J.D[OFF_PQ]; W.pq0 = J.D[OFF_PQ0]; W.pt = J.D[OFF_PT]; W.pt0 = J.D[OFF_PT0]; }
    }
    __syncthreads();
    float* tiles = tiles_ + wave * TILE1;
    const int px = blockIdx.x % NP, bi = blockIdx.x / NP, gp = gridDim.x / NP;
    const int gw = bi * FW + wave;
#ifdef MLLP_TIMING_BUILD
    unsigned long long stamp_sum[8] = {0, 0, 0, 0, 0, 0, 0, 0};
    unsigned long long stamp_last = __builtin_amdgcn_s_memtime();
    const unsigned long long stamp_begin = stamp_last;
#define STAMP_ARGS1 , stamp_sum, stamp_last
#else
#define STAMP_ARGS1
#endif
    for (int j = 0; j < A.n_jobs; ++j) {
        const BwdJob1& J = A.job[j];
        const PartTiers P = J.s.part[px];
        f32x4m accT = splat4(0.0f);
        float accS[6] = {0.0f, 0.0f, 0.0f, 0.0f, 0.0f, 0.0f};
        for (int k = bi; k < P.n_block; k += gp)
            bwd1_row(J, Ws_[j], block_slot<1>(J.s, P.row0 + k, tid), lane, merge_lds, tiles, accT, accS STAMP_ARGS1);
        WaveList wl = wave_list(J.s, px, gw);
        for (int c0 = 0; c0 < wl.L; c0 += 64) {
            wave_list_chunk(wl, c0, lane);
            int it = wave_list_get(wl, 0);
            SlotReq q = item_request<1>(J.s, P, max(it, 0), lane);
            for (int k = 0; it >= 0; ++k) {
                const int itn = wave_list_get(wl, k + 1);
                const RowSlot r = slot_make(q);
                q = item_request<1>(J.s, P, max(itn, 0), lane);
                bwd1_row(J, Ws_[j], r, lane, merge_lds, tiles, accT, accS STAMP_ARGS1);
#ifdef MLLP_TIMING_BUILD
                stamp_sum[7] += 1;
#endif
                it = itn;
            }
        }
        __syncthreads();
        float* red = tiles_;
#pragma unroll
        for (int q = 0; q < 4; ++q) red[wave * 262 + ((lane >> 4) * 4 + q) * 16 + (lane & 15)] = accT[q];
#pragma unroll
        for (int i = 0; i < 6; ++i) {
            const float v = wave_sum(accS[i]);
            if (lane == 0) red[wave * 262 + 256 + i] = v;
        }
        __syncthreads();
        float* dst = J.stats + (size_t)blockIdx.x * STAT_FLOATS;
        for (int i = tid; i < STAT_FLOATS; i += FT) dst[i] = 0.0f;
        __syncthreads();
        if (tid < 262) {
            float v = 0.0f;
            for (int w = 0; w < FW; ++w) v += red[w * 262 + tid];
            const int o = tid >> 4, n = tid & 15;
            if (tid >= 256) {
                const int i = tid - 256;
                const int slot = i == 0 ? 768 : i == 1 ? 1024 : i == 2 ? 1280 : i == 3 ? 1280 + 16 : i == 4 ? 1536 : 1536 + 16;
                dst[slot] = v;
            } else if (n == 0) dst[o * 16] = v;
            else if (n == 1) dst[256 + o * 16] = v;
            else if (n < 5) dst[512 + o * 16 + (n - 2)] = v;
        }
        __syncthreads();
#ifdef MLLP_TIMING_BUILD
        stamp_last = __builtin_amdgcn_s_memtime();
#endif
    }
#ifdef MLLP_TIMING_BUILD
    if (lane == 0) {
        stamp_sum[6] = __builtin_amdgcn_s_memtime() - stamp_begin;
        unsigned long long* d = g_fused_stamps1 + (size_t)(blockIdx.x * FW + wave) * 8;
        for (int k = 0; k < 8; ++k) d[k] = stamp_sum[k];
    }
#endif
#undef STAMP_ARGS1
}

__global__ __launch_bounds__(RT) void fused_head_bwd_kernel(int n, const float* __restrict__ h3, const float* __restrict__ fcw,
                                                            const float* __restrict__ dlogits, const int* __restrict__ perm,
                                                            float* __restrict__ dh3, float* __restrict__ head_part) {
    __shared__ float head_lds[(RT / 64) * 18];
    const int tid = threadIdx.x, lane = tid & 63, part = lane & 3;
    HeadAcc ha;
    ha.w = f4zero(); ha.b = 0.0f; ha.l = 0.0f;
    const float4 fw = ld4(fcw + 4 * part);
    for (int row = blockIdx.x * (RT / 4) + (tid >> 2); row < n; row += gridDim.x * (RT / 4)) {
        const float dz = dlogits[perm[row]];
        const float4 hv = ld4(h3 + (size_t)row * 16 + 4 * part);
        *reinterpret_cast<float4*>(dh3 + (size_t)row * 16 + 4 * part) = f4scale(fw, dz);
        fma4(dz, hv, ha.w);
        if (part == 0) ha.b += dz;
    }
    head_partials_store<RT / 64>(ha, head_lds, head_part, tid);
}

struct ReduceArgs {
    const float* stats[MODEL_CONVS];
    float* out[MODEL_CONVS];
    int nblk;
    const float* head_part;
    float* head_out;
    float* loss_out;
};

__device__ __forceinline__ void fused_reduce_body(const ReduceArgs& A, int n_conv) {
    __shared__ float sh[32][32];
    const int tid = threadIdx.x;
    if ((int)blockIdx.x == n_conv * STAT_TILES) {
        if (!A.head_part) return;
        const int col = tid & 31, slice = tid >> 5;
        float v = 0.0f;
        if (col < 18)
            for (int b = slice; b < A.nblk; b += 32) v += A.head_part[(size_t)b * 18 + col];
        sh[slice][col] = v;
        __syncthreads();
        if (tid < 18) {
            float t = 0.0f;
            for (int q = 0; q < 32; ++q) t += sh[q][tid];
            if (tid < 17) A.head_out[tid] = t;
            else if (A.loss_out) A.loss_out[0] = t;
        }
        return;
    }
    float* sh4 = &sh[0][0];
    const int col = tid & 255, slice = tid >> 8;
    const int c = blockIdx.x / STAT_TILES, tile = blockIdx.x % STAT_TILES;
    const float* src = A.stats[c] + tile * 256 + col;
    float v = 0.0f;
    int b = slice;
    for (; b + 124 < A.nblk; b += 128) {
        float t[32];
#pragma unroll
        for (int q = 0; q < 32; ++q) t[q] = src[(size_t)(b + 4 * q) * STAT_FLOATS];
#pragma unroll
        for (int q = 0; q < 32; ++q) v += t[q];
    }
    for (; b + 28 < A.nblk; b += 32) {
        float t[8];
#pragma unroll
        for (int q = 0; q < 8; ++q) t[q] = src[(size_t)(b + 4 * q) * STAT_FLOATS];
#pragma unroll
        for (int q = 0; q < 8; ++q) v += t[q];
    }
    for (; b < A.nblk; b += 4) v += src[(size_t)b * STAT_FLOATS];
    sh4[slice * 256 + col] = v;
    __syncthreads();
    if (tid < 256) A.out[c][tile * 256 + tid] = (sh4[tid] + sh4[256 + tid]) + (sh4[512 + tid] + sh4[768 + tid]);
}
__global__ __launch_bounds__(RT) void fused_reduce_kernel(ReduceArgs A, int n_conv) { fused_reduce_body(A, n_conv); }

struct TailArgs {
    ReduceArgs R;
    ConvParams p[MODEL_CONVS];
    int cin[MODEL_CONVS];
    float* grads[MODEL_CONVS];
    float* zero;
    int n_zero;
    float* params; const float* grads_all; float* m; float* v; float* state;
    float eps;
    int n_params;
    float* D[MODEL_CONVS];
    unsigned long long* sync;
    unsigned* err;
};
__device__ __forceinline__ bool tail_barrier(unsigned long long* cnt, unsigned long long target, unsigned* err_host) {
    __shared__ int ok_s;
    unsigned long long* err_dev = cnt + 2;
    __syncthreads();
    if (threadIdx.x == 0) {
        __threadfence();
        __hip_atomic_fetch_add(cnt, 1ull, __ATOMIC_RELEASE, __HIP_MEMORY_SCOPE_AGENT);
        int spins = 0;
        while (__hip_atomic_load(cnt, __ATOMIC_ACQUIRE, __HIP_MEMORY_SCOPE_AGENT) < target && ++spins < (1 << 22))
            __builtin_amdgcn_s_sleep(8);
        if (spins >= (1 << 22)) {
            __hip_atomic_store(err_dev, 1ull, __ATOMIC_RELAXED, __HIP_MEMORY_SCOPE_AGENT);
            __hip_atomic_store(err_host, 1u, __ATOMIC_RELAXED, __HIP_MEMORY_SCOPE_SYSTEM);
        }
        __threadfence();
        ok_s = __hip_atomic_load(err_dev, __ATOMIC_RELAXED, __HIP_MEMORY_SCOPE_AGENT) == 0ull;
    }
    __syncthreads();
    return ok_s != 0;
}
__global__ __launch_bounds__(RT) void fused_tail_kernel(TailArgs A, int n_conv) {
    const unsigned long long G = gridDim.x, epoch = A.sync[1];
    const int b = blockIdx.x;
    const float step = A.state[0] + 1.0f, lr = A.state[1], b1 = A.state[2], b2 = A.state[3];
    fused_reduce_body(A.R, n_conv);
    if (!tail_barrier(A.sync, (epoch + 1) * G, A.err)) return;
    if (b < n_conv) {
        finalize_conv_body(A.cin[b], A.p[b], A.R.out[b], 1, A.grads[b]);
        __syncthreads();
        const int off = (int)(A.grads[b] - A.grads_all), n = 4 * FEAT * A.cin[b] + 5 * FEAT;
        adam_slice(A.params + off, A.grads_all + off, A.m + off, A.v + off, step, lr, b1, b2, A.eps, 1.0f, n);
        __syncthreads();
        if (threadIdx.x < BLOCK) param_prep_body(A.p[b], A.cin[b], A.D[b]);
    } else if (b == n_conv) {
        for (int k = threadIdx.x; k < A.n_zero; k += RT) A.zero[k] = 0.0f;
        const int off = (int)(A.R.head_out - A.grads_all);
        adam_slice(A.params + off, A.grads_all + off, A.m + off, A.v + off, step, lr, b1, b2, A.eps, 1.0f, A.n_params - off);
        if (threadIdx.x == 0) {
            A.state[0] = step;
            A.sync[1] = epoch + 1;
        }
    }
}

__global__ __launch_bounds__(256) void fused_fill_kernel(int n_dst, const int* __restrict__ perm, const int* __restrict__ ptr,
                                                         const int* __restrict__ idx, const float* __restrict__ val,
                                                         const int* __restrict__ inv_src, const int* __restrict__ sptr,
                                                         int2* __restrict__ sent) {
    const int k = blockIdx.x * 4 + (threadIdx.x >> 6), lane = threadIdx.x & 63;
    if (k >= n_dst) return;
    const int r = perm[k], beg = ptr[r], deg = ptr[r + 1] - beg, o = sptr[k];
    for (int e = lane; e < deg; e += 64) sent[o + e] = make_int2(inv_src[idx[beg + e]], __float_as_int(val[beg + e]));
}
__global__ void fused_permute_kernel(int n, const int* __restrict__ perm, const float* __restrict__ src, float* __restrict__ dst) {
    for (int i = blockIdx.x * blockDim.x + threadIdx.x; i < n; i += gridDim.x * blockDim.x) dst[i] = src[perm[i]];
}
__global__ void fused_pregather_kernel(int64_t nnz, const int2* __restrict__ sent, const float* __restrict__ xs,
                                       float2* __restrict__ sax) {
    for (int64_t e = blockIdx.x * (int64_t)blockDim.x + threadIdx.x; e < nnz; e += (int64_t)gridDim.x * blockDim.x) {
        const int2 v = sent[e];
        sax[e] = make_float2(__int_as_float(v.y), xs[v.x]);
    }
}

#ifdef MLLP_TIMING_BUILD
extern "C" int mllp_timing_read_stamps(unsigned long long* host, int n) {
    return hipMemcpyFromSymbol(host, HIP_SYMBOL(g_fused_stamps), (size_t)n * sizeof(unsigned long long)) == hipSuccess ? 0 : -1;
}
extern "C" int mllp_timing_read_stamps1(unsigned long long* host, int n) {
    return hipMemcpyFromSymbol(host, HIP_SYMBOL(g_fused_stamps1), (size_t)n * sizeof(unsigned long long)) == hipSuccess ? 0 : -1;
}
#endif

template <class T>
static int dev_alloc(mllp_graph* g, size_t count, T** out, const T* host = nullptr, size_t room = 1) {
    void* p = nullptr;
    MLLP_HIP_TRY(hipMalloc(&p, std::max<size_t>(count, room) * sizeof(T)));
    if (count < room) MLLP_HIP_TRY(hipMemset(p, 0, room * sizeof(T)));
    g->allocs.push_back(p);
    if (host && count) MLLP_HIP_TRY(hipMemcpy(p, host, count * sizeof(T), hipMemcpyHostToDevice));
    *out = static_cast<T*>(p);
    return MLLP_OK;
}

static void set_tiers(FusedTiersDev& d, const FusedTiers& t) {
    d.n_block = t.n_block; d.n_wave = t.n_wave; d.n_group = t.n_group; d.n_base = t.n_base;
}

int fused_refill_values(mllp_graph* g, hipStream_t s) {
    int rc;
    if (g->M > 0) {
        hipLaunchKernelGGL(fused_fill_kernel, dim3((unsigned)((g->M + 3) / 4)), dim3(256), 0, s, (int)g->M, g->perm_c, g->A.ptr,
                           g->A.idx, g->A.val, g->inv_v, g->FA.sptr, reinterpret_cast<int2*>(g->FA.sent));
        if ((rc = check_launch("fused_fill A"))) return rc;
    }
    if (g->N > 0) {
        hipLaunchKernelGGL(fused_fill_kernel, dim3((unsigned)((g->N + 3) / 4)), dim3(256), 0, s, (int)g->N, g->perm_v, g->At.ptr,
                           g->At.idx, g->At.val, g->inv_c, g->FAt.sptr, reinterpret_cast<int2*>(g->FAt.sent));
        if ((rc = check_launch("fused_fill At"))) return rc;
    }
    return MLLP_OK;
}

int fused_graph_build(mllp_graph* g, const int* h_csr_ptr, const int* h_csc_ptr) {
    if (g->fused_built) return MLLP_OK;
    if ((int64_t)g->h_csr_ptr.size() != g->M + 1 && !h_csr_ptr) return fail(MLLP_EINVAL, "fused path: no host row pointers");
    HostFusedOrient hc, hv;
    {
#ifdef MLLP_SCALAR_PARTITION
        const std::vector<int> part = host_partition_instances(host_instance_cost(h_csr_ptr, g->h_inst_ptr_m),
                                                               host_instance_cost(h_csc_ptr, g->h_inst_ptr_n), FUSED_PARTS);
#else
        const std::vector<int> part = host_partition_instances_v(host_instance_loads(h_csr_ptr, g->h_inst_ptr_m),
                                                                 host_instance_loads(h_csc_ptr, g->h_inst_ptr_n), FUSED_PARTS);
#endif
        host_build_fused_orient(h_csr_ptr, (int)g->M, g->h_inst_ptr_m, part, &hc);
        host_build_fused_orient(h_csc_ptr, (int)g->N, g->h_inst_ptr_n, part, &hv);
    }
    int rc;
    if ((rc = dev_alloc(g, (size_t)g->M, &g->perm_c, hc.perm.data()))) return rc;
    if ((rc = dev_alloc(g, (size_t)g->N, &g->perm_v, hv.perm.data()))) return rc;
    if ((rc = dev_alloc(g, (size_t)g->M, &g->inv_c, hc.inv.data()))) return rc;
    if ((rc = dev_alloc(g, (size_t)g->N, &g->inv_v, hv.inv.data()))) return rc;
    FusedOrient& A = g->FA;
    FusedOrient& At = g->FAt;
    A.n_dst = (int)g->M; A.n_src = (int)g->N; A.nnz = (int)g->nnz;
    At.n_dst = (int)g->N; At.n_src = (int)g->M; At.nnz = (int)g->nnz;
    for (int q = 0; q < NP; ++q) {
        set_tiers(A.t16[q], hc.t16[q]); set_tiers(A.t1[q], hc.t1[q]);
        set_tiers(At.t16[q], hv.t16[q]); set_tiers(At.t1[q], hv.t1[q]);
    }
    for (int q = 0; q <= NP; ++q) { A.row0[q] = hc.row0[q]; At.row0[q] = hv.row0[q]; }
    {
        const int gp = fused_grid(g) / NP;
        const HostFusedOrient* ho[2] = {&hc, &hv};
        FusedOrient* dv[2] = {&A, &At};
        for (int k = 0; k < 2; ++k) {
            HostWaveLists l16, l16x2, l1;
            host_build_wave_lists(*ho[k], false, gp * FW, FW, 4, &l16);
            host_build_wave_lists(*ho[k], false, 2 * gp * FW, FW, 2, &l16x2);
            host_build_wave_lists(*ho[k], true, gp * FW, FW, 8, &l1);
            FusedOrient& d = *dv[k];
            d.L16 = l16.L; d.nw16 = l16.waves_per_part;
            d.L16x2 = l16x2.L; d.nw16x2 = l16x2.waves_per_part;
            d.L1 = l1.L; d.nw1 = l1.waves_per_part;
            if ((rc = dev_alloc(g, l16.order.size(), &d.lst16, l16.order.data()))) return rc;
            if ((rc = dev_alloc(g, l16x2.order.size(), &d.lst16x2, l16x2.order.data()))) return rc;
            if ((rc = dev_alloc(g, l1.order.size(), &d.lst1, l1.order.data()))) return rc;
        }
    }
    if ((rc = dev_alloc(g, (size_t)g->M + 1, &A.sptr, hc.sptr.data(), 2))) return rc;
    if ((rc = dev_alloc(g, (size_t)g->N + 1, &At.sptr, hv.sptr.data(), 2))) return rc;
    if ((rc = dev_alloc(g, (size_t)g->nnz * 2, &A.sent, (const int*)nullptr, 2))) return rc;
    if ((rc = dev_alloc(g, (size_t)g->nnz * 2, &At.sent, (const int*)nullptr, 2))) return rc;
    if ((rc = dev_alloc(g, (size_t)g->nnz * 2, &A.sax, (const float*)nullptr, 2))) return rc;
    if ((rc = dev_alloc(g, (size_t)g->nnz * 2, &At.sax, (const float*)nullptr, 2))) return rc;
    if ((rc = dev_alloc(g, (size_t)g->N, &g->inv_n_p))) return rc;
    if ((rc = dev_alloc(g, (size_t)g->N, &g->x1_p))) return rc;
    if ((rc = dev_alloc(g, (size_t)g->M, &g->x2_p))) return rc;
    if ((rc = dev_alloc(g, (size_t)g->N, &g->labels_p))) return rc;
    if (!g->tail_sync) {
        if ((rc = dev_alloc(g, (size_t)4, &g->tail_sync))) return rc;
        MLLP_HIP_TRY(hipMemset(g->tail_sync, 0, 32));
        MLLP_HIP_TRY(hipHostMalloc((void**)&g->tail_err_host, 64, hipHostMallocMapped));
        *g->tail_err_host = 0u;
        MLLP_HIP_TRY(hipHostGetDevicePointer((void**)&g->tail_err_dev, g->tail_err_host, 0));
    }
    if ((rc = fused_refill_values(g, 0))) return rc;
    if (g->N > 0) {
        hipLaunchKernelGGL(fused_permute_kernel, dim3(256), dim3(256), 0, 0, (int)g->N, g->perm_v, g->inv_n, g->inv_n_p);
        if ((rc = check_launch("fused_permute inv_n"))) return rc;
    }
    MLLP_HIP_TRY(hipDeviceSynchronize());
    g->fused_built = true;
    return MLLP_OK;
}

int fused_bind(mllp_graph* g, const float* x1, const float* x2, const float* labels, hipStream_t s) {
    int rc;
    hipStreamCaptureStatus cap = hipStreamCaptureStatusNone;
    (void)hipStreamIsCapturing(s, &cap);
    const bool capturing = cap != hipStreamCaptureStatusNone;
    if (capturing) g->bound_x1 = g->bound_x2 = g->bound_labels = nullptr;
    if (x1 != g->bound_x1 || x2 != g->bound_x2) {
        if (g->N > 0) hipLaunchKernelGGL(fused_permute_kernel, dim3(256), dim3(256), 0, s, (int)g->N, g->perm_v, x1, g->x1_p);
        if (g->M > 0) hipLaunchKernelGGL(fused_permute_kernel, dim3(256), dim3(256), 0, s, (int)g->M, g->perm_c, x2, g->x2_p);
        if (g->nnz > 0) {
            hipLaunchKernelGGL(fused_pregather_kernel, dim3(1024), dim3(256), 0, s, g->nnz,
                               reinterpret_cast<const int2*>(g->FA.sent), g->x1_p, reinterpret_cast<float2*>(g->FA.sax));
            hipLaunchKernelGGL(fused_pregather_kernel, dim3(1024), dim3(256), 0, s, g->nnz,
                               reinterpret_cast<const int2*>(g->FAt.sent), g->x2_p, reinterpret_cast<float2*>(g->FAt.sax));
        }
        if ((rc = check_launch("fused_bind inputs"))) return rc;
        if (!capturing) { g->bound_x1 = x1; g->bound_x2 = x2; }
    }
    if (labels && labels != g->bound_labels) {
        if (g->N > 0) hipLaunchKernelGGL(fused_permute_kernel, dim3(256), dim3(256), 0, s, (int)g->N, g->perm_v, labels, g->labels_p);
        if ((rc = check_launch("fused_bind labels"))) return rc;
        if (!capturing) g->bound_labels = labels;
    }
    return MLLP_OK;
}

int fused_grid(const mllp_graph* g) { return std::max(std::min(g->n_cu, STAT_BLOCKS_MAX) / NP, 1) * NP; }

static FwdJob16 fwd_job16(const FusedOrient& o, const FusedModel& m, int c, const float* x_src, const float* x_dst, float* h) {
    const ConvWs& w = m.w.c[c];
    FwdJob16 J = {};
    J.s = items_dev(o, 0);
    J.x_src = x_src; J.x_dst = x_dst; J.D = w.derived; J.p = conv_params_at(conv_at(m.P, c), MODEL_CONV[c].cin);
    J.h = h; J.Z = w.Z; J.aux = w.aux;
    J.head = 0;
#ifdef MLLP_TIMING_BUILD
    J.abl = g_fused_abl;
#endif
    return J;
}
static FwdJob1 fwd_job1(const FusedOrient& o, const FusedModel& m, int c, const float* x_dst, float* h) {
    const ConvWs& w = m.w.c[c];
    FwdJob1 J = {};
    J.s = items_dev(o, 1);
    J.x_dst = x_dst; J.D = w.derived; J.p = conv_params_at(conv_at(m.P, c), MODEL_CONV[c].cin);
    J.h = h; J.Z = w.Z; J.aux = w.aux;
    return J;
}

int fused_forward(mllp_graph* g, const FusedModel& m, int head_mode, hipStream_t s, bool skip_prep) {
    const int G = fused_grid(g);
    const ModelWs& w = m.w;
    int rc;
    if ((rc = fused_bind(g, m.x1, m.x2, head_mode == 2 ? m.labels : nullptr, s))) return rc;
    if (!skip_prep && (rc = model_param_prep(m.P, w, s))) return rc;
    {
        FwdLaunch1 L = {};
        L.n_jobs = 2;
        L.job[0] = fwd_job1(g->FAt, m, CONV_1V, g->x1_p, w.h1v);
        L.job[1] = fwd_job1(g->FA, m, CONV_1C, g->x2_p, w.h1c);
        hipLaunchKernelGGL(fused_fwd1_kernel, dim3(G), dim3(FT), 0, s, L);
        if ((rc = check_launch("fused_fwd1"))) return rc;
    }
    {
        FwdLaunch16 L = {};
        L.n_jobs = 2;
        L.job[0] = fwd_job16(g->FAt, m, CONV_2V, w.h1c, w.h1v, w.h2v);
        L.job[1] = fwd_job16(g->FA, m, CONV_2C, w.h1v, w.h1c, w.h2c);
        L.job[0].perm = g->perm_v; L.job[1].perm = g->perm_c;
        hipLaunchKernelGGL(fused_fwd16_kernel, dim3(G), dim3(FT), 0, s, L);
        if ((rc = check_launch("fused_fwd16 layer 2"))) return rc;
    }
    {
        FwdLaunch16 L = {};
        L.n_jobs = 1;
        L.job[0] = fwd_job16(g->FAt, m, CONV_3V, w.h2c, w.h2v, w.h3v);
        FwdJob16& J = L.job[0];
        J.head = head_mode;
        J.fcw = m.P + OFF_FC; J.fcb = m.P + OFF_FC + FEAT; J.inv_n = g->inv_n_p; J.labels = g->labels_p; J.perm = g->perm_v;
        J.inv_batch = m.inv_batch;
        J.logits = m.logits; J.g_out = w.d3v; J.head_part = w.head_partials;
        hipLaunchKernelGGL(fused_fwd16_kernel, dim3(G), dim3(FT), 0, s, L);
        if ((rc = check_launch("fused_fwd16 layer 3"))) return rc;
    }
    return MLLP_OK;
}

int fused_head_backward(const mllp_graph* g, const FusedModel& m, const float* dlogits, hipStream_t s) {
    const int G = fused_grid(g);
    hipLaunchKernelGGL(fused_head_bwd_kernel, dim3(G), dim3(RT), 0, s, (int)g->N, m.w.h3v, m.P + OFF_FC, dlogits, g->perm_v,
                       m.w.d3v, m.w.head_partials);
    return check_launch("fused_head_bwd");
}

static BwdJob16 bwd_job16(const FusedOrient& o, const FusedModel& m, int c, const float* x_src, const float* x_dst,
                          const float* h, const float* dh_a, const float* dh_b, float* dx_dst, bool need_rec, bool mask_dx) {
    const ConvWs& w = m.w.c[c];
    BwdJob16 J = {};
    J.s = items_dev(o, 0);
    J.x_src = x_src; J.x_dst = x_dst; J.D = w.derived; J.p = conv_params_at(conv_at(m.P, c), MODEL_CONV[c].cin);
    J.h = h; J.dh_a = dh_a; J.dh_b = dh_b; J.Z = w.Z; J.aux = w.aux;
    J.rec = need_rec ? w.rec : nullptr;
    J.dx_dst = dx_dst;
    J.mask_dx = mask_dx ? 1 : 0;
    J.stats = w.stats;
#ifdef MLLP_TIMING_BUILD
    J.abl = g_fused_abl;
#endif
    return J;
}
static SrcJob16 src_job16(const FusedOrient& o_src_major, const ConvWs& w, const float* x_rows, float* dx, const float* add) {
    SrcJob16 J = {};
    J.s = items_dev(o_src_major, 2);
    J.x = x_rows; J.rec = w.rec; J.dx = dx;
    J.addp = add ? add : x_rows; J.addw = add ? 1.0f : 0.0f; J.mask = 1;
    return J;
}
static BwdJob1 bwd_job1(const FusedOrient& o, const FusedModel& m, int c, const float* x_dst, const float* g_masked) {
    const ConvWs& w = m.w.c[c];
    BwdJob1 J = {};
    J.s = items_dev(o, 1);
    J.x_dst = x_dst; J.D = w.derived; J.p = conv_params_at(conv_at(m.P, c), MODEL_CONV[c].cin);
    J.g = g_masked; J.Z = w.Z; J.aux = w.aux; J.stats = w.stats;
    return J;
}

int fused_backward(const mllp_graph* g, const FusedModel& m, bool premasked, float* grads, float* loss, hipStream_t s,
                   const FusedAdam* adam) {
    const int G = fused_grid(g);
    const ModelWs& w = m.w;
    int rc;
    const FusedOrient& A = g->FA;
    const FusedOrient& At = g->FAt;
    {
        BwdLaunch16 L = {};
        L.n_jobs = 1;
        L.job[0] = bwd_job16(At, m, CONV_3V, w.h2c, w.h2v, premasked ? nullptr : w.h3v, w.d3v, nullptr, w.d2v, true, true);
        hipLaunchKernelGGL(fused_bwd16_kernel, dim3(G), dim3(FT), 0, s, L);
        if ((rc = check_launch("fused_bwd16 C3"))) return rc;
    }
    {
        SrcLaunch16 S = {};
        S.n_jobs = 1;
        S.job[0] = src_job16(A, w.c[CONV_3V], w.h2c, w.d2c, nullptr);
        hipLaunchKernelGGL(fused_src16_kernel, dim3(2 * G), dim3(FT), 0, s, S);
        if ((rc = check_launch("fused_src16 C3"))) return rc;
        BwdLaunch16 L = {};
        L.n_jobs = 1;
        L.job[0] = bwd_job16(At, m, CONV_2V, w.h1c, w.h1v, nullptr, w.d2v, nullptr, w.d1v, true, true);
        hipLaunchKernelGGL(fused_bwd16_kernel, dim3(G), dim3(FT), 0, s, L);
        if ((rc = check_launch("fused_bwd16 C2V"))) return rc;
    }
    {
        BwdLaunch16 L = {};
        L.n_jobs = 1;
        L.job[0] = bwd_job16(A, m, CONV_2C, w.h1v, w.h1c, nullptr, w.d2c, nullptr, w.d1c, true, true);
        hipLaunchKernelGGL(fused_bwd16_kernel, dim3(G), dim3(FT), 0, s, L);
        if ((rc = check_launch("fused_bwd16 C2C"))) return rc;
        SrcLaunch16 S = {};
        S.n_jobs = 2;
        S.job[0] = src_job16(A, w.c[CONV_2V], w.h1c, w.d1c_b, w.d1c);
        S.job[1] = src_job16(At, w.c[CONV_2C], w.h1v, w.d1v_b, w.d1v);
        hipLaunchKernelGGL(fused_src16_kernel, dim3(2 * G), dim3(FT), 0, s, S);
        if ((rc = check_launch("fused_src16 C2V + C2C"))) return rc;
    }
    {
        BwdLaunch1 L = {};
        L.n_jobs = 2;
        L.job[0] = bwd_job1(A, m, CONV_1C, g->x2_p, w.d1c_b);
        L.job[1] = bwd_job1(At, m, CONV_1V, g->x1_p, w.d1v_b);
        hipLaunchKernelGGL(fused_bwd1_kernel, dim3(G), dim3(FT), 0, s, L);
        if ((rc = check_launch("fused_bwd1"))) return rc;
    }
    ReduceArgs R = {};
    for (int c = 0; c < MODEL_CONVS; ++c) { R.stats[c] = w.c[c].stats; R.out[c] = w.c[c].red; }
    R.nblk = G;
    R.head_part = w.head_partials;
    R.head_out = grads + OFF_FC;
    R.loss_out = loss;
    if (adam) {
        TailArgs T = {};
        T.R = R;
        for (int c = 0; c < MODEL_CONVS; ++c) {
            T.p[c] = conv_params_at(conv_at(m.P, c), MODEL_CONV[c].cin);
            T.cin[c] = MODEL_CONV[c].cin;
            T.grads[c] = conv_at(grads, c);
            T.D[c] = w.c[c].derived;
        }
        T.zero = grads + OFF_UNUSED;
        T.n_zero = LEN_UNUSED;
        T.params = adam->params; T.grads_all = grads; T.m = adam->m; T.v = adam->v; T.state = adam->state;
        T.eps = adam->eps;
        T.n_params = adam->n;
        T.sync = g->tail_sync;
        T.err = g->tail_err_dev;
        if (g->tail_err_host && *(volatile unsigned*)g->tail_err_host != 0u)
            return fail(MLLP_EHIP, "the grid barrier of fused_tail_kernel timed out in an earlier step (the device was shared with "
                                   "other work): parameters and optimizer state since then are invalid; recreate the graph");
        hipLaunchKernelGGL(fused_tail_kernel, dim3(MODEL_CONVS * STAT_TILES + 1), dim3(RT), 0, s, T, MODEL_CONVS);
        return check_launch("fused_tail");
    }
    {
        hipLaunchKernelGGL(fused_reduce_kernel, dim3(MODEL_CONVS * STAT_TILES + 1), dim3(RT), 0, s, R, MODEL_CONVS);
        if ((rc = check_launch("fused_reduce"))) return rc;
    }
    return model_finalize(g, m.P, w, true, grads, s);
}

}
```

### mllp_amd/csrc/host_graph.cpp

```cpp
#include "host_graph.h"

#include <array>

#include <algorithm>
#include <atomic>
#include <thread>

#include "../../include/mllp_hip.h"

namespace mllp {

int host_build_batch(int64_t n_inst, const int64_t* inst_m, const int64_t* inst_n, const int64_t* indptr,
                     const int32_t* indices, const double* values, HostBatch* out, std::string* err,
                     unsigned max_threads) {
    auto bad_arg = [&](int code, const char* msg) {
        if (err) *err = msg;
        return code;
    };
    if (!out) return bad_arg(MLLP_EINVAL, "host_build_batch: out is null");
    if (n_inst < 0 || (n_inst > 0 && (!inst_m || !inst_n || !indptr)))
        return bad_arg(MLLP_EINVAL, "mllp_graph_create_host: null instance arrays");
    std::vector<int64_t> pm(n_inst + 1, 0), pn(n_inst + 1, 0), pe(n_inst + 1, 0), pp(n_inst + 1, 0);
    for (int64_t k = 0; k < n_inst; ++k) {
        if (inst_m[k] < 0 || inst_n[k] < 0) return bad_arg(MLLP_EINVAL, "negative instance size");
// ... 172 lines not shown
            if (d == 4) continue;
            std::vector<double> l((size_t)n_parts, 0.0);
            double tot = 0.0;
            for (size_t i = 0; i < a.size(); ++i) {
                const double v = (double)(side ? b[i].d[d] : a[i].d[d]);
                l[(size_t)part[i]] += v;
                tot += v;
            }
            if (tot <= 0.0) continue;
            for (int q = 0; q < n_parts; ++q) worst = std::max(worst, l[(size_t)q] * n_parts / tot);
        }
    return worst;
}

std::vector<int> host_partition_instances_v(const std::vector<InstLoad>& a, const std::vector<InstLoad>& b, int n_parts) {
    const int n = (int)a.size();
    constexpr int D = VecBalance::D;
    VecBalance vb;
    vb.n_parts = n_parts;
    vb.x.assign((size_t)n, std::array<double, D>{});
    vb.load.assign((size_t)n_parts, std::array<double, D>{});
    double tot[D] = {};
    for (int i = 0; i < n; ++i)
        for (int d = 0; d < FUSED_LOAD_DIMS; ++d) { tot[d] += (double)a[i].d[d]; tot[FUSED_LOAD_DIMS + d] += (double)b[i].d[d]; }
    std::vector<double> size((size_t)n, 0.0);
    for (int i = 0; i < n; ++i)
        for (int d = 0; d < D; ++d) {
            const double v = (double)(d < FUSED_LOAD_DIMS ? a[i].d[d] : b[i].d[d - FUSED_LOAD_DIMS]);
            vb.x[(size_t)i][d] = tot[d] > 0.0 && d % FUSED_LOAD_DIMS != 4 ? v * n_parts / tot[d] : 0.0;
            size[(size_t)i] = std::max(size[(size_t)i], vb.x[(size_t)i][d]);
        }
    std::vector<int> order((size_t)n), part((size_t)n, 0);
    for (int i = 0; i < n; ++i) order[(size_t)i] = i;
    std::stable_sort(order.begin(), order.end(), [&](int p, int q) { return size[(size_t)p] > size[(size_t)q]; });
    std::vector<int> count((size_t)n_parts, 0);
    for (int i : order) {
        int best = 0;
        double best_v = 0.0;
        for (int q = 0; q < n_parts; ++q) {
            double v = 0.0;
            for (int d = 0; d < D; ++d) v = std::max(v, vb.load[(size_t)q][d] + vb.x[(size_t)i][d]);
            if (q == 0 || v < best_v - 1e-12 || (v < best_v + 1e-12 && count[(size_t)q] < count[(size_t)best])) { best = q; best_v = v; }
        }
        part[(size_t)i] = best;
        count[(size_t)best]++;
        for (int d = 0; d < D; ++d) vb.load[(size_t)best][d] += vb.x[(size_t)i][d];
    }
    if (n <= 4096) {
        for (int round = 0; round < 200; ++round) {
            int wq = 0;
            for (int q = 1; q < n_parts; ++q)
                if (vb.max_of(q) > vb.max_of(wq)) wq = q;
            const double cur = vb.max_of(wq);
            double best_gain = 1e-9;
            int bi = -1, bj = -1, bq = -1;
            auto pair_max = [&](int q1, int q2, int i, int j) {
                double m = 0.0;
                for (int d = 0; d < D; ++d) {
                    const double xi = vb.x[(size_t)i][d], xj = j >= 0 ? vb.x[(size_t)j][d] : 0.0;
                    m = std::max(m, std::max(vb.load[(size_t)q1][d] - xi + xj, vb.load[(size_t)q2][d] + xi - xj));
                }
                return m;
            };
            for (int i = 0; i < n; ++i) {
                if (part[(size_t)i] != wq) continue;
                for (int q = 0; q < n_parts; ++q) {
                    if (q == wq) continue;
                    const double m0 = pair_max(wq, q, i, -1);
                    if (cur - m0 > best_gain) { best_gain = cur - m0; bi = i; bj = -1; bq = q; }
                    for (int j = 0; j < n; ++j) {
                        if (part[(size_t)j] != q) continue;
                        const double m1 = pair_max(wq, q, i, j);
                        if (cur - m1 > best_gain) { best_gain = cur - m1; bi = i; bj = j; bq = q; }
                    }
                }
            }
            if (bi < 0) break;
            for (int d = 0; d < D; ++d) {
                const double xi = vb.x[(size_t)bi][d], xj = bj >= 0 ? vb.x[(size_t)bj][d] : 0.0;
                vb.load[(size_t)wq][d] += xj - xi;
                vb.load[(size_t)bq][d] += xi - xj;
            }
            part[(size_t)bi] = bq;
            if (bj >= 0) part[(size_t)bj] = wq;
        }
    }
    std::vector<int64_t> ca((size_t)n), cb((size_t)n);
    for (int i = 0; i < n; ++i) { ca[(size_t)i] = a[(size_t)i].d[5]; cb[(size_t)i] = b[(size_t)i].d[5]; }
    const std::vector<int> alt = host_partition_instances(ca, cb, n_parts);
    return host_partition_imbalance(a, b, alt, n_parts) < host_partition_imbalance(a, b, part, n_parts) - 1e-12 ? alt : part;
}

std::vector<int> host_partition_instances(const std::vector<int64_t>& cost_a, const std::vector<int64_t>& cost_b, int n_parts) {
    const int n = (int)cost_a.size();
    std::vector<int64_t> ca((size_t)n), cb((size_t)n);
    int64_t sa = 1, sb = 1;
    for (int i = 0; i < n; ++i) {
        ca[i] = cost_a[i] + 1;
        cb[i] = cost_b[i] + 1;
        sa += ca[i]; sb += cb[i];
    }
    std::vector<int> order((size_t)n), part((size_t)n, 0);
    for (int i = 0; i < n; ++i) order[i] = i;
    std::stable_sort(order.begin(), order.end(), [&](int a, int b) { return ca[a] + cb[a] > ca[b] + cb[b]; });
    std::vector<int64_t> la((size_t)n_parts, 0), lb((size_t)n_parts, 0);
    for (int i : order) {
        int best = 0;
        double best_v = 0.0;
        for (int q = 0; q < n_parts; ++q) {
            const double v = std::max((double)(la[q] + ca[i]) / (double)sa, (double)(lb[q] + cb[i]) / (double)sb);
            if (q == 0 || v < best_v) { best = q; best_v = v; }
        }
        part[i] = best;
        la[best] += ca[i];
        lb[best] += cb[i];
    }
    return part;
}

void host_build_fused_orient(const int* ptr, int n, const std::vector<int64_t>& inst_off, const std::vector<int>& inst_part,
                             HostFusedOrient* out) {
    HostFusedOrient& o = *out;
    o = HostFusedOrient();
    n = std::max(n, 0);
    o.perm.resize((size_t)n);
    o.inv.resize((size_t)n);
    o.sptr.assign((size_t)n + 1, 0);
    std::vector<int> node_part((size_t)n, 0);
    for (size_t k = 0; k + 1 < inst_off.size(); ++k)
        for (int64_t r = inst_off[k]; r < inst_off[k + 1] && r < n; ++r) node_part[(size_t)r] = inst_part[k];
    for (int r = 0; r < n; ++r) o.perm[r] = r;
    std::stable_sort(o.perm.begin(), o.perm.end(), [&](int a, int b) {
        if (node_part[a] != node_part[b]) return node_part[a] < node_part[b];
        return ptr[a + 1] - ptr[a] > ptr[b + 1] - ptr[b];
    });
    for (int q = 0; q <= FUSED_PARTS; ++q) o.row0[q] = 0;
    for (int k = 0; k < n; ++k) {
        const int r = o.perm[k], deg = ptr[r + 1] - ptr[r], q = node_part[r];
        o.inv[r] = k;
        o.sptr[k + 1] = o.sptr[k] + deg;
        o.row0[q + 1]++;
        for (int which = 0; which < 2; ++which) {
            const int(&T)[3] = which ? FUSED_T1 : FUSED_T16;
            FusedTiers& t = which ? o.t1[q] : o.t16[q];
            if (deg > T[2]) t.n_block++;
            else if (deg > T[1]) t.n_wave++;
            else if (deg > T[0]) t.n_group++;
            else t.n_base++;
        }
    }
    for (int q = 0; q < FUSED_PARTS; ++q) o.row0[q + 1] += o.row0[q];
}

void host_build_wave_lists(const HostFusedOrient& o, bool scalar, int waves_per_part, int waves_per_wg, int nnz_per_step,
                           HostWaveLists* out) {
    HostWaveLists& wl = *out;
    wl = HostWaveLists();
    const int nw = std::max(waves_per_part, 1), wpg = std::max(std::min(waves_per_wg, nw), 1), gp = std::max(nw / wpg, 1);
    wl.waves_per_part = nw;
    const int U = scalar ? 64 : 16, RG = U / 4;
    const int e_base = std::max(nnz_per_step, 1), e_group = 4 * e_base, e_wave = (scalar ? 64 : 16) * e_base;
    std::vector<std::vector<int>> lists((size_t)FUSED_PARTS * nw);
    for (int q = 0; q < FUSED_PARTS; ++q) {
        const FusedTiers& t = scalar ? o.t1[q] : o.t16[q];
        const int n_gitems = (t.n_group + RG - 1) / RG, n_bitems = (t.n_base + U - 1) / U;
        const int n_items = t.n_wave + n_gitems + n_bitems;
        auto deg_of = [&](int rl) { const int k = o.row0[q] + rl; return (int64_t)o.sptr[(size_t)k + 1] - o.sptr[(size_t)k]; };
        std::vector<std::pair<int64_t, int>> items((size_t)n_items);
        for (int it = 0; it < n_items; ++it) {
            int64_t steps;
            if (it < t.n_wave) steps = (deg_of(t.n_block + it) + e_wave - 1) / e_wave;
            else if (it < t.n_wave + n_gitems) steps = (deg_of(t.n_block + t.n_wave + (it - t.n_wave) * RG) + e_group - 1) / e_group;
            else steps = (deg_of(t.n_block + t.n_wave + t.n_group + (it - t.n_wave - n_gitems) * U) + e_base - 1) / e_base;
            items[(size_t)it] = {FUSED_COST_ITEM + FUSED_COST_STEP * std::max<int64_t>(steps, 1), it};
        }
        std::stable_sort(items.begin(), items.end(), [](const auto& a, const auto& b) { return a.first > b.first; });
        std::vector<int64_t> load((size_t)nw, 0), slow((size_t)nw, 0);
        for (int w = 0; w < nw; ++w) {
            const int bi = w / wpg;
            const int n_rows = bi < gp && t.n_block > bi ? (t.n_block - bi + gp - 1) / gp : 0;
            slow[(size_t)w] = 1000 + 95 * ((w % wpg) / 4);
            load[(size_t)w] = FUSED_COST_BLOCK_ROW * n_rows * slow[(size_t)w] / 1000;
        }
        for (const auto& itc : items) {
            int best = 0;
            int64_t best_t = 0;
            for (int w = 0; w < nw; ++w) {
                const int64_t tw = load[(size_t)w] + itc.first * slow[(size_t)w] / 1000;
                if (w == 0 || tw < best_t) { best = w; best_t = tw; }
            }
            lists[(size_t)q * nw + best].push_back(itc.second);
            load[(size_t)best] = best_t;
        }
        for (int w = 0; w < nw; ++w) {
            wl.max_load = std::max(wl.max_load, load[(size_t)w]);
            wl.sum_load += load[(size_t)w];
            wl.L = std::max(wl.L, (int)lists[(size_t)q * nw + w].size());
        }
    }
    wl.L = std::max(wl.L, 1);
    wl.order.assign((size_t)FUSED_PARTS * nw * wl.L, -1);
    for (size_t k = 0; k < lists.size(); ++k) std::copy(lists[k].begin(), lists[k].end(), wl.order.begin() + k * wl.L);
}

}
```

### mllp_amd/csrc/host_graph.h

```cpp
#pragma once
#include <stdint.h>

#include <string>
#include <vector>

namespace mllp {

struct HostBatch {
    int64_t M = 0, N = 0, nnz = 0, n_inst = 0;
    std::vector<int64_t> pm, pn;
    std::vector<int> csr_ptr, csr_idx;
    std::vector<float> csr_val;
    std::vector<int> csc_ptr, csc_idx;
    std::vector<float> csc_val;
};

int host_build_batch(int64_t n_inst, const int64_t* inst_m, const int64_t* inst_n, const int64_t* indptr,
                     const int32_t* indices, const double* values, HostBatch* out, std::string* err,
                     unsigned max_threads = 0);

struct TierConfig {
    int tier_wave = 0, tier_block = 0, chunk_nnz = 0;
};
TierConfig host_choose_tiers(int64_t nnz, int tier_wave, int tier_block);

struct HostTiers {
    std::vector<int> rows_wave;
    std::vector<int> chunks;
    std::vector<int> split;
    int n_group = 0, n_slots = 0;
    bool short_rows = false;
};
void host_build_tiers(const int* ptr, int n_dst, const TierConfig& cfg, HostTiers* out);

constexpr int FUSED_PARTS = 8;
struct FusedTiers {
    int n_block = 0, n_wave = 0, n_group = 0, n_base = 0;
};
struct HostFusedOrient {
    std::vector<int> perm;
    std::vector<int> inv;
    std::vector<int> sptr;
    int row0[FUSED_PARTS + 1];
    FusedTiers t16[FUSED_PARTS], t1[FUSED_PARTS];
};
constexpr int FUSED_T16[3] = {16, 64, 1024};
constexpr int FUSED_T1[3] = {16, 64, 4096};
constexpr int64_t FUSED_COST_ITEM = 5300, FUSED_COST_STEP = 2000, FUSED_COST_BLOCK_ROW = 25000;
std::vector<int64_t> host_instance_cost(const int* ptr, const std::vector<int64_t>& inst_off);
std::vector<int> host_partition_instances(const std::vector<int64_t>& cost_a, const std::vector<int64_t>& cost_b, int n_parts);
constexpr int FUSED_BLOCK_ROW_ITEMS = 10;
constexpr int FUSED_LOAD_DIMS = 6;
struct InstLoad {
    int64_t d[FUSED_LOAD_DIMS] = {0, 0, 0, 0, 0, 0};
};
std::vector<InstLoad> host_instance_loads(const int* ptr, const std::vector<int64_t>& inst_off);
std::vector<int> host_partition_instances_v(const std::vector<InstLoad>& a, const std::vector<InstLoad>& b, int n_parts);
double host_partition_imbalance(const std::vector<InstLoad>& a, const std::vector<InstLoad>& b, const std::vector<int>& part,
                                int n_parts);
void host_build_fused_orient(const int* ptr, int n, const std::vector<int64_t>& inst_off, const std::vector<int>& inst_part,
                             HostFusedOrient* out);
struct HostWaveLists {
    std::vector<int> order;
    int L = 0, waves_per_part = 0;
    int64_t max_load = 0, sum_load = 0;
};
void host_build_wave_lists(const HostFusedOrient& o, bool scalar, int waves_per_part, int waves_per_wg, int nnz_per_step,
                           HostWaveLists* out);

}
```

### mllp_amd/csrc/internal.h

```cpp
#pragma once
#include <hip/hip_runtime.h>
#include <stdint.h>

#include <algorithm>
#include <string>
#include <vector>

#include "../../include/mllp_hip.h"

namespace mllp {

constexpr int FEAT = 16;
constexpr int BLOCK = 256;
constexpr int REC_W = 40;
constexpr int STAT_TILES = 7;
constexpr int STAT_FLOATS = STAT_TILES * 256;
constexpr int STAT_BLOCKS_MAX = 256;

void set_error(const std::string& msg);
int fail(int code, const std::string& msg);
int hip_fail(hipError_t e, const char* what);

#define MLLP_HIP_TRY(expr)                                              \
    do {                                                                \
        hipError_t _e = (expr);                                         \
        if (_e != hipSuccess) return ::mllp::hip_fail(_e, #expr);       \
    } while (0)

#define REQUIRE(cond, msg) \
    if (!(cond)) return ::mllp::fail(MLLP_EINVAL, std::string(__func__) + ": " + (msg))

inline int check_launch(const char* what) {
    hipError_t e = hipGetLastError();
    return e == hipSuccess ? MLLP_OK : hip_fail(e, what);
}

template <class T>
struct DevBuf {
    T* p = nullptr;
    ~DevBuf() { if (p) (void)hipFree(p); }
    int alloc(size_t n) { return hipMalloc((void**)&p, std::max<size_t>(n, 1) * sizeof(T)) == hipSuccess ? 0 : 1; }
};

struct Tiled {
    int n_tiles = 0, n_tb = 0, max_nbt = 0, max_run = 0;
    bool owned = false;
    const int* tile_blk = nullptr;
    const int* blk_id = nullptr;
    const int* ptr2 = nullptr;
    const int* perm = nullptr;
    const int* ent = nullptr;
    int* vmap = nullptr;
};
constexpr int TILED_SPMM = 0;
constexpr int TILED_ATTN = 1;
constexpr int TILED_BSRC = 2;
constexpr int TILED_SCALAR = 3;
constexpr int TILED_BDST = 4;
constexpr int TILED_VARIANTS = 5;

struct StreamCopy {
    int n_tiles = 0, n_tb = 0;
    int64_t n_groups = 0;
    int64_t step_slots = 0;
    int* tile_row = nullptr;
    int* tile_blk = nullptr;
    int* blk_id = nullptr;
    int* rows = nullptr;
    int* hdr = nullptr;
    int* ent = nullptr;
    int* vmap = nullptr;
    double build_seconds = 0.0;
};

struct LaneCopy {
    int n_tiles = 0, n_tb = 0;
    int64_t n_groups = 0;
    int64_t nnz = 0;
    int* tile_row = nullptr;
    int* tile_blk = nullptr;
    int* tile_col = nullptr;
    int* rows = nullptr;
    int* whdr = nullptr;
    unsigned* offs = nullptr;
    float* vals = nullptr;
    int* vmap = nullptr;
    double build_seconds = 0.0;
};

struct CopyArray {
    void** p;
    int64_t bytes;
};
enum { SC_TILE_BLK, SC_BLK_ID, SC_ROWS, SC_ENT, SC_TILE_ROW, SC_HDR };
enum { LC_TILE_BLK, LC_TILE_COL, LC_ROWS, LC_OFFS, LC_TILE_ROW, LC_WHDR, LC_VALS };
enum { TL_TILE_BLK, TL_BLK_ID, TL_PTR2, TL_PERM, TL_ENT };
std::vector<CopyArray> stream_copy_arrays(StreamCopy& sc, int geom);
std::vector<CopyArray> lane_copy_arrays(LaneCopy& lc);
std::vector<CopyArray> tiled_arrays(Tiled& tl, int variant, int64_t nnz);
int copy_alloc(const CopyArray& a);
void copy_free(const std::vector<CopyArray>& arrays);

struct Orient {
    LaneCopy lane1;
    StreamCopy stream[4];
    Tiled tiled[TILED_VARIANTS];
    int n_dst = 0, n_src = 0;
    int* ptr = nullptr;
    int* idx = nullptr;
    float* val = nullptr;
    int* rows_group = nullptr;
    int* rows_wave = nullptr;
    int* chunks = nullptr;
    int* split = nullptr;
    int n_group = 0, n_wave = 0, n_chunk = 0, n_split = 0, n_slots = 0;
    float* scratch = nullptr;
    int tier_wave = 0;
    bool short_rows = false;
};
struct FusedTiersDev {
    int n_block = 0, n_wave = 0, n_group = 0, n_base = 0;
};
constexpr int FUSED_NP = 8;
struct FusedOrient {
    int n_dst = 0, n_src = 0, nnz = 0;
    int* sptr = nullptr;
    int* sent = nullptr;
    float* sax = nullptr;
    int row0[FUSED_NP + 1] = {};
    FusedTiersDev t16[FUSED_NP], t1[FUSED_NP];
    int* lst16 = nullptr; int* lst16x2 = nullptr; int* lst1 = nullptr;
    int L16 = 0, L16x2 = 0, L1 = 0, nw16 = 0, nw16x2 = 0, nw1 = 0;
};
constexpr int SCRATCH_NS = 20;

}

struct mllp_graph {
    int64_t M = 0, N = 0, nnz = 0, n_inst = 0;
    mllp::Orient A;
    mllp::Orient At;
    float* inv_n = nullptr;
    int* inst_ptr_n = nullptr;
    int* inst_ptr_m = nullptr;
    std::vector<int64_t> h_inst_ptr_n, h_inst_ptr_m;
    std::vector<int> h_csr_ptr, h_csc_ptr;
    int tier_wave = 0, tier_block = 0, chunk_nnz = 0;
    int max_inst_n = 0;
    int n_cu = 256;
    int path = 0;
    bool fused_built = false;
    mllp::FusedOrient FA, FAt;
    int* perm_v = nullptr;
    int* perm_c = nullptr;
    int* inv_v = nullptr;
    int* inv_c = nullptr;
    float* inv_n_p = nullptr;
    unsigned long long* tail_sync = nullptr;
    unsigned* tail_err_host = nullptr;
    unsigned* tail_err_dev = nullptr;
    float* x1_p = nullptr;
    float* x2_p = nullptr;
    float* labels_p = nullptr;
    const void* bound_x1 = nullptr;
    const void* bound_x2 = nullptr;
    const void* bound_labels = nullptr;
    int ws_path = -1;
    const void* ws_ptr = nullptr;
    const void* folded_ws = nullptr;
    const void* folded_params = nullptr;
    int* at_pos = nullptr;
    float* scale_buf = nullptr;
    float* norm_scale = nullptr;
    hipStream_t aux = nullptr;
    hipEvent_t ev[16] = {};
    std::vector<void*> allocs;
};

namespace mllp {

struct ConvParams {
    const float *Wk, *bk, *Wq, *bq, *Wv, *bv, *we, *Ws, *bs;
};
constexpr int conv_param_count(int cin) { return 4 * FEAT * cin + 5 * FEAT; }

enum { CONV_1V, CONV_1C, CONV_2V, CONV_2C, CONV_3V };
constexpr int MODEL_CONVS = CONV_3V + 1;
struct ConvSpec {
    bool dst_is_var;
    int cin;
};
constexpr ConvSpec MODEL_CONV[MODEL_CONVS] = {{true, 1}, {false, 1}, {true, 16}, {false, 16}, {true, 16}};
struct ConvOffsets {
    int at[MODEL_CONVS + 1];
};
constexpr ConvOffsets conv_offsets() {
    ConvOffsets o = {};
    for (int c = 0; c < MODEL_CONVS; ++c) o.at[c + 1] = o.at[c] + conv_param_count(MODEL_CONV[c].cin);
    return o;
}
constexpr ConvOffsets CONV_OFF = conv_offsets();
constexpr int OFF_UNUSED = CONV_OFF.at[MODEL_CONVS], LEN_UNUSED = conv_param_count(FEAT);
constexpr int OFF_FC = OFF_UNUSED + LEN_UNUSED;
constexpr int NUM_PARAMS = OFF_FC + FEAT + 1;
static_assert(CONV_OFF.at[CONV_1V] == 0 && CONV_OFF.at[CONV_1C] == 144 && CONV_OFF.at[CONV_2V] == 288 &&
                  CONV_OFF.at[CONV_2C] == 1392 && CONV_OFF.at[CONV_3V] == 2496,
              "conv offsets differ from GNNModel.state_dict()");
static_assert(OFF_UNUSED == 3600 && LEN_UNUSED == 1104 && OFF_FC == 4704, "gconv3_s2w / fc offsets differ from state_dict()");
static_assert(NUM_PARAMS == MLLP_NUM_PARAMS, "the layout's total differs from MLLP_NUM_PARAMS");
template <class T>
inline T* conv_at(T* base, int c) { return base + CONV_OFF.at[c]; }

inline ConvParams conv_params_at(const float* base, int cin) {
    ConvParams p;
    const float* q = base;
    p.Wk = q; q += FEAT * cin;
    p.bk = q; q += FEAT;
    p.Wq = q; q += FEAT * cin;
    p.bq = q; q += FEAT;
    p.Wv = q; q += FEAT * cin;
    p.bv = q; q += FEAT;
    p.we = q; q += FEAT;
    p.Ws = q; q += FEAT * cin;
    p.bs = q;
    return p;
}

constexpr int OFF_PQ = 0, OFF_PQT = 256, OFF_WST = 512, OFF_WVT = 768;
constexpr int OFF_PQ0 = 1024, OFF_PT = 1040, OFF_PB = 1056, OFF_PT0 = 1072;
constexpr int DERIVED_W = 1088;

struct ConvWs {
    float* derived;
    float* qp;
    float* t;
    float* Z;
    float* aux;
    float* rec;
    float* dqp;
    float* dsdt;
    float* stats;
    float* red;
};
ConvWs conv_ws_carve(float* base, int64_t n_dst, int cin, float** end = nullptr);
int64_t conv_ws_floats(int64_t n_dst, int cin);

struct ModelWs {
    ConvWs c[MODEL_CONVS];
    float *h1v, *h1c, *h2v, *h2c, *h3v;
    float *d3v, *d2v, *d2c, *d1v, *d1c;
    float *d1v_b, *d1c_b;
    float* head_partials;
    int64_t total;
};

int launch_spmm(const Orient& o, const float* H, float* Y, float* scratch, hipStream_t s);
int build_stream_device(const Orient& o, int64_t nnz, const std::vector<int>& tile_row, StreamCopy& sc, hipStream_t s,
                        int geom = 0);
void stream_copy_free(StreamCopy& sc);
int build_tiled_device(const Orient& o, int64_t nnz, int variant, Tiled& out, hipStream_t s);
void tiled_free(Tiled& tl);
int launch_spmm_stream(const StreamCopy& sc, int n_dst, int n_src, const float* H, float* Y, hipStream_t s);
struct ConvWs;
int launch_fwd16_stream(const StreamCopy& sc, int n_dst, int n_src, const float* conv_params, const ConvWs& w,
                        const float* x_src, const float* x_dst, float* h_out, hipStream_t s);
int launch_bwddst16_stream(const StreamCopy& sc, int n_dst, int n_src, const ConvWs& w, const float* x_src, const float* g,
                           float* dx_dst, int accumulate, hipStream_t s);
struct ConvWs;
int launch_fwd1_lane(const LaneCopy& lc, int n_dst, int n_src, const float* conv_params, const ConvWs& w, const float* x_src,
                     const float* x_dst, float* h_out, hipStream_t s);
int launch_bwddst1_lane(const LaneCopy& lc, int n_dst, int n_src, const ConvWs& w, const float* x_src, hipStream_t s);
int build_lane_copy(const Orient& o, int64_t nnz, const std::vector<int64_t>& seg, LaneCopy& lc, hipStream_t s);
void lane_copy_free(LaneCopy& lc);
int launch_bwdsrc16_stream(const StreamCopy& sc, int n_rows, int n_cols, const float* rec, const float* x_rows, float* dx,
                           int accumulate, hipStream_t s);
int launch_spmm_tiled(const Tiled& tl, int n_dst, int n_src, const float* H, float* Y, hipStream_t s);
int launch_spmm_tiled_bf16(const Tiled& tl, int n_dst, int n_src, const void* H_bf16, float* Y, hipStream_t s);
struct ConvWs;
int launch_fwd16_tiled(const Tiled& tl, int n_dst, int n_src, const float* conv_params, const ConvWs& w,
                       const float* x_src, const float* x_dst, float* h_out, hipStream_t s);
int launch_fwd1_tiled(const Tiled& tl, int n_dst, int n_src, const float* conv_params, const ConvWs& w,
                      const float* x_src, const float* x_dst, float* h_out, hipStream_t s);
int launch_bwddst1_tiled(const Tiled& tl, int n_dst, int n_src, const ConvWs& w, const float* x_src, hipStream_t s);
int launch_bwddst16_tiled(const Tiled& tl, int n_dst, int n_src, const ConvWs& w, const float* x_src, const float* g,
                          float* dx_dst, int accumulate, hipStream_t s);
// ... 80 lines not shown
```

### mllp_amd/graph.py

```python
import ctypes
import itertools
import time
from ctypes import c_int32, c_int64, c_double, c_void_p
from typing import List, Optional, Sequence

import numpy as np
import torch

from . import _lib
from .data import LPInstance


_B128_GROUPS = [[0, 1, 2, 3, 12, 13, 14, 15, 20, 21, 22, 23, 24, 25, 26, 27],
                [4, 5, 6, 7, 8, 9, 10, 11, 16, 17, 18, 19, 28, 29, 30, 31]]
LANE_GROUPS = [[l + h for l in grp if (l & 3) == r] for h in (0, 32) for grp in _B128_GROUPS for r in range(4)]


def build_tiled_arrays(ptr, idx, val, n_dst, R, CB, variant=0, entry_order="joint"):
    dev, nnz = idx.device, int(idx.numel())
    if nnz == 0:
        return None
    n_tiles = (n_dst + R - 1) // R
    deg = (ptr[1:] - ptr[:-1]).long()
    rows = torch.repeat_interleave(torch.arange(n_dst, device=dev, dtype=torch.int32), deg)
# ... 433 lines not shown
        n, dt = sizes[which]
        out = np.empty(n, dtype=dt)
        _lib.check(_lib.lib().mllp_graph_export(self._h, which, out.ctypes.data_as(c_void_p), out.nbytes))
        return out

    def logits_per_instance(self, logits):
        return [logits[self._n_off[k]:self._n_off[k + 1]] for k in range(self.n_inst)]

    def spmm(self, H: torch.Tensor, transpose=False, out: Optional[torch.Tensor] = None):
        n_in, n_out = (self.M, self.N) if transpose else (self.N, self.M)
        assert H.is_cuda and H.dtype == torch.float32 and H.is_contiguous() and tuple(H.shape) == (n_in, 16)
        if out is None:
            out = torch.empty(n_out, 16, device=H.device, dtype=torch.float32)
        _lib.check(_lib.lib().mllp_spmm_csr_f32(self._h, int(transpose), _lib.ptr(H), _lib.ptr(out),
                                                _lib.current_stream()))
        return out

    def spmm_bf16(self, H: torch.Tensor, transpose=False, out: Optional[torch.Tensor] = None):
        n_in, n_out = (self.M, self.N) if transpose else (self.N, self.M)
        assert H.is_cuda and H.dtype == torch.bfloat16 and H.is_contiguous() and tuple(H.shape) == (n_in, 16)
        if out is None:
            out = torch.empty(n_out, 16, device=H.device, dtype=torch.float32)
        _lib.check(_lib.lib().mllp_spmm_csr_bf16(self._h, int(transpose), _lib.ptr(H), _lib.ptr(out),
                                                 _lib.current_stream()))
        return out

    def tconv_workspace(self, dst_is_var, cin):
        n = c_int64()
        _lib.check(_lib.lib().mllp_tconv_workspace_floats(self._h, int(dst_is_var), cin, ctypes.byref(n)))
        return torch.empty(n.value, device=self.x1.device, dtype=torch.float32)

    def tconv_fwd(self, dst_is_var, cin, conv_params, x_src, x_dst, ws):
        n_dst = self.N if dst_is_var else self.M
        h = torch.empty(n_dst, 16, device=x_src.device, dtype=torch.float32)
        _lib.check(_lib.lib().mllp_tconv_fwd(self._h, int(dst_is_var), cin, _lib.ptr(conv_params), _lib.ptr(x_src),
                                             _lib.ptr(x_dst), _lib.ptr(h), _lib.ptr(ws), _lib.current_stream()))
        return h

    def tconv_bwd(self, dst_is_var, cin, conv_params, x_src, x_dst, h, ws, dh, want_input_grads=True):
        n_dst, n_src = (self.N, self.M) if dst_is_var else (self.M, self.N)
        dh = dh.clone()
        dxd = torch.empty(n_dst, cin, device=dh.device) if (want_input_grads and cin == 16) else None
        dxs = torch.empty(n_src, cin, device=dh.device) if (want_input_grads and cin == 16) else None
        pg = torch.empty(conv_params.numel(), device=dh.device, dtype=torch.float32)
        _lib.check(_lib.lib().mllp_tconv_bwd(self._h, int(dst_is_var), cin, _lib.ptr(conv_params), _lib.ptr(x_src),
                                             _lib.ptr(x_dst), _lib.ptr(h), _lib.ptr(ws), _lib.ptr(dh), _lib.ptr(dxd),
                                             _lib.ptr(dxs), 0, _lib.ptr(pg), _lib.current_stream()))
        return pg, dxd, dxs, dh

    def workspace(self):
        if self._ws is None:
            n = c_int64()
            _lib.check(_lib.lib().mllp_gnn_workspace_bytes(self._h, ctypes.byref(n)))
            self._ws = torch.empty(n.value // 4, device=self.x1.device, dtype=torch.float32)
        return self._ws

    def forward(self, params: torch.Tensor, logits: Optional[torch.Tensor] = None):
        assert params.is_cuda and params.dtype == torch.float32 and params.numel() == _lib.NUM_PARAMS
        if logits is None:
            logits = torch.empty(self.N, device=params.device, dtype=torch.float32)
        self._check_inputs()
        self._folded = None
        _lib.check(_lib.lib().mllp_gnn_forward(self._h, _lib.ptr(params), _lib.ptr(self.x1), _lib.ptr(self.x2),
                                               _lib.ptr(self.workspace()), _lib.ptr(logits), _lib.current_stream()))
        return logits

    def backward(self, params, dlogits, grads: Optional[torch.Tensor] = None):
        if grads is None:
            grads = torch.empty(_lib.NUM_PARAMS, device=params.device, dtype=torch.float32)
        dlogits = dlogits.contiguous().float()
        _lib.check(_lib.lib().mllp_gnn_backward(self._h, _lib.ptr(params), _lib.ptr(self.x1), _lib.ptr(self.x2),
                                                _lib.ptr(self.workspace()), _lib.ptr(dlogits), _lib.ptr(grads),
                                                _lib.current_stream()))
        return grads

    def backward_inputs(self, params, dlogits, x1=True, x2=True, values=True, grads=None):
        dev = params.device
        if grads is None:
            grads = torch.empty(_lib.NUM_PARAMS, device=dev, dtype=torch.float32)
        dx1 = torch.empty(self.N, device=dev, dtype=torch.float32) if x1 else None
        dx2 = torch.empty(self.M, device=dev, dtype=torch.float32) if x2 else None
        dv = torch.empty(self.nnz, device=dev, dtype=torch.float32) if values else None
        dlogits = dlogits.contiguous().float()
        _lib.check(_lib.lib().mllp_gnn_backward_inputs(self._h, _lib.ptr(params), _lib.ptr(self.x1), _lib.ptr(self.x2),
                                                       _lib.ptr(self.workspace()), _lib.ptr(dlogits), _lib.ptr(grads),
                                                       _lib.ptr(dx1), _lib.ptr(dx2), _lib.ptr(dv), c_void_p(0),
                                                       _lib.current_stream()))
        return grads, dx1, dx2, dv

    def _input_grad_outputs(self, dev, x1, x2, values):
        return (torch.empty(self.N, device=dev, dtype=torch.float32) if x1 else None,
                torch.empty(self.M, device=dev, dtype=torch.float32) if x2 else None,
                torch.empty(self.nnz, device=dev, dtype=torch.float32) if values else None)

    def input_grads(self, params, dlogits, x1=True, x2=True, values=True, grads=None):
        dev = params.device
        if grads is None:
            grads = torch.empty(_lib.NUM_PARAMS, device=dev, dtype=torch.float32)
        dx1, dx2, dv = self._input_grad_outputs(dev, x1, x2, values)
        dlogits = dlogits.contiguous().float()
        _lib.check(_lib.lib().mllp_gnn_input_grads(self._h, _lib.ptr(params), _lib.ptr(self.x1), _lib.ptr(self.x2),
                                                   _lib.ptr(self.workspace()), _lib.ptr(dlogits), _lib.ptr(grads),
                                                   _lib.ptr(dx1), _lib.ptr(dx2), _lib.ptr(dv), c_void_p(0),
                                                   _lib.current_stream()))
        return grads, dx1, dx2, dv

    def loss_step_inputs(self, params, inv_batch=None, logits=None, loss=None, grads=None, x1=True, x2=True, values=True):
        dev = params.device
        logits = torch.empty(self.N, device=dev, dtype=torch.float32) if logits is None else logits
        loss = torch.empty(1, device=dev, dtype=torch.float32) if loss is None else loss
        grads = torch.empty(_lib.NUM_PARAMS, device=dev, dtype=torch.float32) if grads is None else grads
        dx1, dx2, dv = self._input_grad_outputs(dev, x1, x2, values)
        ib = (1.0 / self.n_inst) if inv_batch is None else float(inv_batch)
        self._check_inputs()
        self._folded = None
        _lib.check(_lib.lib().mllp_gnn_loss_step_inputs(self._h, _lib.ptr(params), _lib.ptr(self.x1), _lib.ptr(self.x2),
                                                        _lib.ptr(self.labels), ib, _lib.ptr(self.workspace()),
                                                        _lib.ptr(logits), _lib.ptr(loss), _lib.ptr(grads), _lib.ptr(dx1),
                                                        _lib.ptr(dx2), _lib.ptr(dv), _lib.current_stream()))
        return loss, logits, grads, dx1, dx2, dv

    def loss_step(self, params, inv_batch=None, logits=None, loss=None, grads=None):
        dev = params.device
        logits = torch.empty(self.N, device=dev, dtype=torch.float32) if logits is None else logits
        loss = torch.empty(1, device=dev, dtype=torch.float32) if loss is None else loss
        grads = torch.empty(_lib.NUM_PARAMS, device=dev, dtype=torch.float32) if grads is None else grads
        ib = (1.0 / self.n_inst) if inv_batch is None else float(inv_batch)
        self._check_inputs()
        self._folded = None
        _lib.check(_lib.lib().mllp_gnn_loss_step(self._h, _lib.ptr(params), _lib.ptr(self.x1), _lib.ptr(self.x2),
                                                 _lib.ptr(self.labels), ib, _lib.ptr(self.workspace()),
                                                 _lib.ptr(logits), _lib.ptr(loss), _lib.ptr(grads),
                                                 _lib.current_stream()))
        return loss, logits, grads

    def train_step(self, params, exp_avg, exp_avg_sq, state, eps=1e-8, inv_batch=None, logits=None, loss=None, grads=None,
                   param_gen=None):
        dev = params.device
        logits = torch.empty(self.N, device=dev, dtype=torch.float32) if logits is None else logits
        loss = torch.empty(1, device=dev, dtype=torch.float32) if loss is None else loss
        grads = torch.empty(_lib.NUM_PARAMS, device=dev, dtype=torch.float32) if grads is None else grads
        ib = (1.0 / self.n_inst) if inv_batch is None else float(inv_batch)
        self._check_inputs()
        key = (params.data_ptr(), params._version, param_gen)
        weights_folded = param_gen is not None and getattr(self, "_folded", None) == key
        _lib.check(_lib.lib().mllp_gnn_train_step(self._h, _lib.ptr(params), _lib.ptr(self.x1), _lib.ptr(self.x2),
                                                  _lib.ptr(self.labels), ib, _lib.ptr(self.workspace()), _lib.ptr(logits),
                                                  _lib.ptr(loss), _lib.ptr(grads), _lib.ptr(exp_avg), _lib.ptr(exp_avg_sq),
                                                  _lib.ptr(state), float(eps), int(bool(weights_folded)),
                                                  _lib.current_stream()))
        self._folded = None if param_gen is None else (params.data_ptr(), params._version, param_gen + 1)
        return loss, logits, grads

    def small_step_fits(self):
        fits = ctypes.c_int()
        _lib.check(_lib.lib().mllp_gnn_small_step_fits(self._h, ctypes.byref(fits)))
        return bool(fits.value)

    def train_step_small(self, params, exp_avg=None, exp_avg_sq=None, state=None, eps=1e-8, inv_batch=None, logits=None,
                         loss=None, grads=None):
        dev = params.device
        logits = torch.empty(self.N, device=dev, dtype=torch.float32) if logits is None else logits
        loss = torch.empty(1, device=dev, dtype=torch.float32) if loss is None else loss
        grads = torch.empty(_lib.NUM_PARAMS, device=dev, dtype=torch.float32) if grads is None else grads
        ib = (1.0 / self.n_inst) if inv_batch is None else float(inv_batch)
        self._check_inputs()
        self._folded = None
        _lib.check(_lib.lib().mllp_gnn_train_step_small(self._h, _lib.ptr(params), _lib.ptr(self.x1), _lib.ptr(self.x2),
                                                        _lib.ptr(self.labels), ib, _lib.ptr(self.workspace()),
                                                        _lib.ptr(logits), _lib.ptr(loss), _lib.ptr(grads),
                                                        _lib.ptr(exp_avg), _lib.ptr(exp_avg_sq), _lib.ptr(state),
                                                        float(eps), _lib.current_stream()))
        return loss, logits, grads

    def topm_metrics(self, logits, out=None):
        if out is None:
            out = torch.empty(self.n_inst, 2, device=logits.device, dtype=torch.float32)
        _lib.check(_lib.lib().mllp_topm_metrics(self._h, _lib.ptr(logits), _lib.ptr(self.labels), c_void_p(0),
                                                _lib.ptr(out), _lib.current_stream()))
        return out

    @property
    def labels(self):
        return self._labels

    @labels.setter
    def labels(self, t):
        self._labels = t
        self._balanced_pw = None

    def balanced_pos_weight(self):
        key = (self._labels.data_ptr(), self._labels._version)
        if self._balanced_pw is None or self._balanced_pw[0] != key:
            out = torch.empty(max(self.n_inst, 1), device=self._labels.device, dtype=torch.float32)
            y = self._labels if self.N else torch.zeros(1, device=out.device)
            _lib.check(_lib.lib().mllp_balanced_pos_weight(self._h, _lib.ptr(y), _lib.ptr(out), _lib.current_stream()))
            self._balanced_pw = (key, out[:self.n_inst])
        return self._balanced_pw[1]

    def _per_instance(self, v, what, allow_balanced=False):
        if v is None:
            return None
        if isinstance(v, str):
            if allow_balanced and v == "balanced":
                return self.balanced_pos_weight()
            raise ValueError(f"{what}: {v!r} is not understood" + (" (a float, a tensor [n_inst] or 'balanced')" if allow_balanced else ""))
        if isinstance(v, torch.Tensor):
            if not (v.is_cuda and v.dtype == torch.float32 and v.is_contiguous() and v.numel() == self.n_inst):
                raise ValueError(f"{what} must be a contiguous cuda float32 tensor of {self.n_inst} elements")
            return v
        consts = self.__dict__.setdefault("_inst_consts", {})
        if float(v) not in consts:
            consts[float(v)] = torch.full((max(self.n_inst, 1),), float(v), device=self.x1.device, dtype=torch.float32)
        return consts[float(v)]

    def weighted_loss(self, logits, inst_weight=None, pos_weight=None, want=("loss", "inst_loss", "dlogits")):
        want = (want,) if isinstance(want, str) else tuple(want)
        bad = [w for w in want if w not in ("loss", "inst_loss", "dlogits")]
        if bad or not want:
            raise ValueError(f"weighted_loss: want must name some of 'loss', 'inst_loss', 'dlogits' (got {want!r})")
        if not (logits.is_cuda and logits.dtype == torch.float32 and logits.is_contiguous() and logits.numel() == self.N):
            raise ValueError(f"weighted_loss: logits must be a contiguous cuda float32 tensor of {self.N} elements")
        dev = logits.device
        iw = self._per_instance(inst_weight, "weighted_loss: inst_weight")
        pw = self._per_instance(pos_weight, "weighted_loss: pos_weight", allow_balanced=True)
        loss = torch.empty(1, device=dev, dtype=torch.float32) if "loss" in want else None
        inst = torch.empty(max(self.n_inst, 1), device=dev, dtype=torch.float32) if {"inst_loss", "loss"} & set(want) else None
        dz = torch.empty(max(self.N, 1), device=dev, dtype=torch.float32) if "dlogits" in want else None
        z, y = (logits, self._labels) if self.N else (torch.zeros(1, device=dev),) * 2
        _lib.check(_lib.lib().mllp_weighted_loss(self._h, _lib.ptr(z), _lib.ptr(y), _lib.ptr(iw), _lib.ptr(pw), _lib.ptr(dz),
                                                 _lib.ptr(inst), _lib.ptr(loss), _lib.current_stream()))
        return dict(loss=loss, inst_loss=inst[:self.n_inst] if "inst_loss" in want else None,
                    dlogits=None if dz is None else dz[:self.N])

    def loss_step_weighted(self, params, inst_weight=None, pos_weight=None, logits=None, loss=None, inst_loss=None,
                           grads=None):
        dev = params.device
        logits = torch.empty(self.N, device=dev, dtype=torch.float32) if logits is None else logits
        loss = torch.empty(1, device=dev, dtype=torch.float32) if loss is None else loss
        inst_loss = torch.empty(max(self.n_inst, 1), device=dev, dtype=torch.float32)[:self.n_inst] if inst_loss is None else inst_loss
        grads = torch.empty(_lib.NUM_PARAMS, device=dev, dtype=torch.float32) if grads is None else grads
        if getattr(self, "last_dlogits", None) is None:
            self.last_dlogits = torch.empty(max(self.N, 1), device=dev, dtype=torch.float32)[:self.N]
        iw = self._per_instance(inst_weight, "loss_step_weighted: inst_weight")
        pw = self._per_instance(pos_weight, "loss_step_weighted: pos_weight", allow_balanced=True)
        self._check_inputs()
        self._folded = None
        _lib.check(_lib.lib().mllp_gnn_loss_step_weighted(self._h, _lib.ptr(params), _lib.ptr(self.x1), _lib.ptr(self.x2),
                                                          _lib.ptr(self._labels), _lib.ptr(iw), _lib.ptr(pw),
                                                          _lib.ptr(self.workspace()), _lib.ptr(logits), _lib.ptr(loss),
                                                          _lib.ptr(inst_loss), _lib.ptr(grads), _lib.ptr(self.last_dlogits),
                                                          _lib.current_stream()))
        return loss, logits, grads, inst_loss

    def evaluate(self, params, pos_weight=None):
        logits = self.forward(params)
        inst = self.weighted_loss(logits, None, pos_weight, want="inst_loss")["inst_loss"]
        return dict(logits=logits, inst_loss=inst, metrics=self.topm_metrics(logits))

    def predict_basis(self, logits, want=("mask", "index", "stats")):
        want = (want,) if isinstance(want, str) else tuple(want)
        bad = [w for w in want if w not in ("mask", "index", "stats")]
        if bad or not want:
            raise ValueError(f"predict_basis: want must name some of 'mask', 'index', 'stats' (got {want!r})")
        if not (logits.is_cuda and logits.dtype == torch.float32 and logits.is_contiguous() and logits.numel() == self.N):
            raise ValueError(f"predict_basis: logits must be a contiguous cuda float32 tensor of {self.N} elements")
        bufs = _select_outputs(want, self.N, self.M, self.n_inst, logits.device)
        _lib.check(_lib.lib().mllp_topm_select(self._h, _lib.ptr(logits), *[_lib.ptr(b) for b in bufs], _lib.current_stream()))
        mask, index, stats = _select_views(bufs, self.N, self.M)
        return BasisPrediction(mask, index, stats, self.inst_n, self.inst_m, self.names)


def _select_outputs(want, n, m, n_seg, dev):
    return (torch.empty(max(n, 1), dtype=torch.uint8, device=dev) if "mask" in want else None,
            torch.empty(max(m, 1), dtype=torch.int32, device=dev) if "index" in want else None,
            torch.empty(max(n_seg, 1), 2, dtype=torch.float32, device=dev) if "stats" in want else None)


def _select_views(bufs, n, m):
    mask, index, stats = bufs
    return (None if mask is None else mask[:n], None if index is None else index[:m], stats)


class BasisPrediction:

    def __init__(self, mask, index, stats, seg_n, seg_m, names=None):
        self.mask, self.index, self.stats = mask, index, stats
        self.seg_n = [int(v) for v in seg_n]
        self.seg_m = [int(v) for v in seg_m]
        self.names = list(names) if names is not None else None

    def split(self):
        if self.index is None:
            raise ValueError("BasisPrediction.split needs the index output (want=('index', ...))")
        idx = self.index.cpu().numpy()
        off = np.concatenate([[0], np.cumsum(self.seg_m)])
        return [idx[off[k]:off[k] + min(self.seg_m[k], self.seg_n[k])] for k in range(len(self.seg_m))]


def topm_select_dense(logits, m, want=("mask", "index", "stats")):
    want = (want,) if isinstance(want, str) else tuple(want)
    bad = [w for w in want if w not in ("mask", "index", "stats")]
    if bad or not want:
        raise ValueError(f"topm_select_dense: want must name some of 'mask', 'index', 'stats' (got {want!r})")
    if not (logits.is_cuda and logits.dtype == torch.float32 and logits.is_contiguous() and logits.dim() == 1):
        raise ValueError("topm_select_dense: logits must be a contiguous 1-d cuda float32 tensor")
# ... 64 lines not shown
```

Before: 288,900 instances/s.

## Spill work items across fused partitions to balance per-wave load

Work items now carry their partition id in the high bits of each wave-list entry, and kernels look up per-item tier info instead of using a fixed partition. On the host, overloaded partitions can spill items to waves of underloaded partitions, using a greedy first-to-finish scheduler. A separate list is built for layer-2 forward that accounts for load already placed by the paired orientation in the same launch. The aim is to cut tail imbalance across partitions. In exchange the kernels do an extra per-item readfirstlane lookup and prefetch, and items may run on waves away from their partition's data.

```diff
diff --git a/include/mllp_hip.h b/include/mllp_hip.h
--- a/include/mllp_hip.h
+++ b/include/mllp_hip.h
@@ -131,6 +131,8 @@
                               float* d_grads, float* d_exp_avg, float* d_exp_avg_sq, float* d_state, float eps,
                               void* stream);
 
+int mllp_graph_fused_lists(const mllp_graph_t* g, int orientation, int kind, int64_t info[5]);
+
 int mllp_metrics_scratch_bytes(const mllp_graph_t* g, int64_t* bytes);
 int mllp_topm_metrics(const mllp_graph_t* g, const float* d_logits, const float* d_labels,
                       void* d_scratch, float* d_out, void* stream);
diff --git a/mllp_amd/_lib.py b/mllp_amd/_lib.py
--- a/mllp_amd/_lib.py
+++ b/mllp_amd/_lib.py
@@ -97,6 +97,7 @@
                                     c_void_p, c_void_p, c_void_p, c_void_p, c_void_p, c_float, c_int, c_void_p]),
     "mllp_gnn_small_step_limits": (c_int, [POINTER(c_int64)]),
     "mllp_gnn_small_step_fits": (c_int, [c_void_p, POINTER(c_int)]),
+    "mllp_graph_fused_lists": (c_int, [c_void_p, c_int, c_int, POINTER(c_int64)]),
     "mllp_gnn_train_step_small": (c_int, [c_void_p, c_void_p, c_void_p, c_void_p, c_void_p, c_float, c_void_p, c_void_p,
                                           c_void_p, c_void_p, c_void_p, c_void_p, c_void_p, c_float, c_void_p]),
     "mllp_weighted_loss": (c_int, [c_void_p, c_void_p, c_void_p, c_void_p, c_void_p, c_void_p, c_void_p, c_void_p, c_void_p]),
diff --git a/mllp_amd/csrc/api.cpp b/mllp_amd/csrc/api.cpp
--- a/mllp_amd/csrc/api.cpp
+++ b/mllp_amd/csrc/api.cpp
@@ -526,6 +526,15 @@
     return launch_adam(d_params, d_grads, d_exp_avg, d_exp_avg_sq, d_state, eps, 1.0f, MLLP_NUM_PARAMS, s);
 }
 
+extern "C" int mllp_graph_fused_lists(const mllp_graph_t* g, int orientation, int kind, int64_t info[5]) {
+    REQUIRE(g && info, "null argument");
+    REQUIRE(orientation >= 0 && orientation <= 1 && kind >= 0 && kind <= 3, "orientation is 0 or 1, kind is 0, 1, 2 or 3");
+    REQUIRE(g->fused_built, "the fused path of this graph is not built (mllp_graph_set_path)");
+    const mllp::FusedOrient& o = orientation ? g->FAt : g->FA;
+    for (int k = 0; k < 5; ++k) info[k] = o.lst_info[kind][k];
+    return MLLP_OK;
+}
+
 extern "C" int mllp_gnn_small_step_limits(int64_t limits[4]) {
     REQUIRE(limits, "null argument");
     limits[0] = SMALL_STEP_MAX_NODES; limits[1] = SMALL_STEP_MAX_NNZ;
diff --git a/mllp_amd/csrc/fused_kernels.hip b/mllp_amd/csrc/fused_kernels.hip
--- a/mllp_amd/csrc/fused_kernels.hip
+++ b/mllp_amd/csrc/fused_kernels.hip
@@ -55,9 +55,9 @@
 static ItemsDev items_dev(const FusedOrient& o, int which) {
     const bool scalar = which == 1;
     ItemsDev d;
-    d.order = which == 0 ? o.lst16 : which == 1 ? o.lst1 : o.lst16x2;
-    d.nw = which == 0 ? o.nw16 : which == 1 ? o.nw1 : o.nw16x2;
-    d.L = which == 0 ? o.L16 : which == 1 ? o.L1 : o.L16x2;
+    d.order = which == 0 ? o.lst16 : which == 1 ? o.lst1 : which == 2 ? o.lst16x2 : o.lst16f;
+    d.nw = which == 1 ? o.nw1 : which == 2 ? o.nw16x2 : o.nw16;
+    d.L = which == 0 ? o.L16 : which == 1 ? o.L1 : which == 2 ? o.L16x2 : o.L16f;
     d.sptr = o.sptr;
     d.sent = reinterpret_cast<const int2*>(o.sent);
     d.sax = reinterpret_cast<const float2*>(o.sax);
@@ -162,10 +162,13 @@
 __device__ __forceinline__ int wave_items(const PartTiers& s) {
     return s.n_wave + (s.n_group + Geo<G>::RG - 1) / Geo<G>::RG + (s.n_base + Geo<G>::U - 1) / Geo<G>::U;
 }
+__device__ __forceinline__ PartTiers item_tiers(const ItemsDev& S, int entry) {
+    return S.part[__builtin_amdgcn_readfirstlane(max(entry, 0) >> FUSED_ITEM_ID_BITS)];
+}
 template <int G>
-__device__ __forceinline__ SlotReq item_request(const ItemsDev& S, const PartTiers& s, int item, int lane) {
+__device__ __forceinline__ SlotReq item_request(const ItemsDev& S, const PartTiers& s, int entry, int lane) {
     constexpr int U = Geo<G>::U, QG = Geo<G>::QG, RG = Geo<G>::RG;
-    const int unit = lane / G;
+    const int unit = lane / G, item = entry & ((1 << FUSED_ITEM_ID_BITS) - 1);
     const int n_gitems = (s.n_group + RG - 1) / RG;
     SlotReq r;
     bool valid;
@@ -567,24 +570,26 @@
         WaveList wl = wave_list(J.s, px, gw);
         for (int c0 = 0; c0 < wl.L; c0 += 64) {
             wave_list_chunk(wl, c0, lane);
-            int it = wave_list_get(wl, 0), it1 = wave_list_get(wl, 1);
-            RowSlot r = it >= 0 ? item_slot<4>(J.s, P, it, lane) : none;
+            int it = wave_list_get(wl, 0), it1 = wave_list_get(wl, 1), it2 = wave_list_get(wl, 2);
+            RowSlot r = it >= 0 ? item_slot<4>(J.s, item_tiers(J.s, it), it, lane) : none;
             float4 xd = r.row >= 0 ? ld4(J.x_dst + (size_t)r.row * 16 + 4 * part) : f4zero();
             int2 en = first_entries<4>(J.s, r, part);
             int lrow = (J.head && r.row >= 0) ? J.perm[r.row] : 0;
-            SlotReq q1 = item_request<4>(J.s, P, max(it1, 0), lane);
+            SlotReq q1 = item_request<4>(J.s, item_tiers(J.s, it1), max(it1, 0), lane);
             if (it1 < 0) q1.row = -1;
+            PartTiers P2 = item_tiers(J.s, it2);
             asm volatile("" : "+v"(xd.x), "+v"(xd.y), "+v"(xd.z), "+v"(xd.w), "+v"(en.x), "+v"(en.y), "+v"(lrow),
                               "+v"(q1.sb), "+v"(q1.se));
             for (int k = 0; it >= 0; ++k) {
-                const int it2 = wave_list_get(wl, k + 2);
+                const int it3 = wave_list_get(wl, k + 3);
+                const PartTiers P3 = item_tiers(J.s, it3);
                 FwdNext nx;
-                fwd16_row(J, Ws_[j], P, r, xd, en, lrow, q1, it2, nx, pend, part, lane, merge_lds, tiles, ha STAMP_ARGS);
+                fwd16_row(J, Ws_[j], P2, r, xd, en, lrow, q1, it2, nx, pend, part, lane, merge_lds, tiles, ha STAMP_ARGS);
 #ifdef MLLP_TIMING_BUILD
                 stamp_sum[7] += 1;
 #endif
                 r = nx.r; xd = nx.xd; en = nx.en; lrow = nx.lrow; q1 = nx.q;
-                it = it1; it1 = it2;
+                it = it1; it1 = it2; it2 = it3; P2 = P3;
             }
         }
         fwd16_flush(J, pend, part);
@@ -764,14 +769,16 @@
         WaveList wl = wave_list(J.s, px, gw);
         for (int c0 = 0; c0 < wl.L; c0 += 64) {
             wave_list_chunk(wl, c0, lane);
-            int it = wave_list_get(wl, 0);
-            SlotReq q = item_request<1>(J.s, P, max(it, 0), lane);
+            int it = wave_list_get(wl, 0), itn = wave_list_get(wl, 1);
+            SlotReq q = item_request<1>(J.s, item_tiers(J.s, it), max(it, 0), lane);
+            PartTiers Pn = item_tiers(J.s, itn);
             for (int k = 0; it >= 0; ++k) {
-                const int itn = wave_list_get(wl, k + 1);
+                const int itn2 = wave_list_get(wl, k + 2);
+                const PartTiers Pn2 = item_tiers(J.s, itn2);
                 const RowSlot r = slot_make(q);
-                q = item_request<1>(J.s, P, max(itn, 0), lane);
+                q = item_request<1>(J.s, Pn, max(itn, 0), lane);
                 fwd1_row(J, Ws_[j], r, lane, merge_lds);
-                it = itn;
+                it = itn; itn = itn2; Pn = Pn2;
             }
         }
     }
@@ -1023,17 +1030,19 @@
         WaveList wl = wave_list(J.s, px, gw);
         for (int c0 = 0; c0 < wl.L; c0 += 64) {
             wave_list_chunk(wl, c0, lane);
-            int it = wave_list_get(wl, 0);
-            RowSlot r = it >= 0 ? item_slot<4>(J.s, P, it, lane) : none;
+            int it = wave_list_get(wl, 0), itn = wave_list_get(wl, 1);
+            RowSlot r = it >= 0 ? item_slot<4>(J.s, item_tiers(J.s, it), it, lane) : none;
+            PartTiers Pn = item_tiers(J.s, itn);
             BwdRow rd;
             bwd16_fetch(J, r, part, rd);
             int2 en = first_entries<4>(J.s, r, part);
             for (int k = 0; it >= 0; ++k) {
-                const int itn = wave_list_get(wl, k + 1);
+                const int itn2 = wave_list_get(wl, k + 2);
+                const PartTiers Pn2 = item_tiers(J.s, itn2);
                 RowSlot rn;
-                bwd16_row(J, Ws_[j], P, r, rd, en, itn, rn, part, lane, merge_lds, tiles, acc);
+                bwd16_row(J, Ws_[j], Pn, r, rd, en, itn, rn, part, lane, merge_lds, tiles, acc);
                 r = rn;
-                it = itn;
+                it = itn; itn = itn2; Pn = Pn2;
             }
         }
         __syncthreads();
@@ -1147,17 +1156,19 @@
         WaveList wl = wave_list(J.s, px, gw);
         for (int c0 = 0; c0 < wl.L; c0 += 64) {
             wave_list_chunk(wl, c0, lane);
-            int it = wave_list_get(wl, 0);
-            RowSlot r = it >= 0 ? item_slot<4>(J.s, P, it, lane) : none;
+            int it = wave_list_get(wl, 0), itn = wave_list_get(wl, 1);
+            RowSlot r = it >= 0 ? item_slot<4>(J.s, item_tiers(J.s, it), it, lane) : none;
+            PartTiers Pn = item_tiers(J.s, itn);
             float4 xj = r.row >= 0 ? ld4(J.x + (size_t)r.row * 16 + 4 * part) : f4zero();
             int2 en = first_entries<2>(J.s, r, part);
             for (int k = 0; it >= 0; ++k) {
-                const int itn = wave_list_get(wl, k + 1);
-                const SlotReq qn = itn >= 0 ? item_request<4>(J.s, P, itn, lane) : empty_request();
+                const int itn2 = wave_list_get(wl, k + 2);
+                const PartTiers Pn2 = item_tiers(J.s, itn2);
+                const SlotReq qn = itn >= 0 ? item_request<4>(J.s, Pn, itn, lane) : empty_request();
                 RowSlot rn;
                 src16_row(J, r, xj, en, qn, rn, part, lane, merge_lds);
                 r = rn;
-                it = itn;
+                it = itn; itn = itn2; Pn = Pn2;
             }
         }
     }
@@ -1345,17 +1356,19 @@
         WaveList wl = wave_list(J.s, px, gw);
         for (int c0 = 0; c0 < wl.L; c0 += 64) {
             wave_list_chunk(wl, c0, lane);
-            int it = wave_list_get(wl, 0);
-            SlotReq q = item_request<1>(J.s, P, max(it, 0), lane);
+            int it = wave_list_get(wl, 0), itn = wave_list_get(wl, 1);
+            SlotReq q = item_request<1>(J.s, item_tiers(J.s, it), max(it, 0), lane);
+            PartTiers Pn = item_tiers(J.s, itn);
             for (int k = 0; it >= 0; ++k) {
-                const int itn = wave_list_get(wl, k + 1);
+                const int itn2 = wave_list_get(wl, k + 2);
+                const PartTiers Pn2 = item_tiers(J.s, itn2);
                 const RowSlot r = slot_make(q);
-                q = item_request<1>(J.s, P, max(itn, 0), lane);
+                q = item_request<1>(J.s, Pn, max(itn, 0), lane);
                 bwd1_row(J, Ws_[j], r, lane, merge_lds, tiles, accT, accS STAMP_ARGS1);
 #ifdef MLLP_TIMING_BUILD
                 stamp_sum[7] += 1;
 #endif
-                it = itn;
+                it = itn; itn = itn2; Pn = Pn2;
             }
         }
         __syncthreads();
@@ -1619,20 +1632,39 @@
     for (int q = 0; q <= NP; ++q) { A.row0[q] = hc.row0[q]; At.row0[q] = hv.row0[q]; }
     {
         const int gp = fused_grid(g) / NP;
-        const HostFusedOrient* ho[2] = {&hc, &hv};
+        const char* env = getenv("MLLP_FUSED_SPILL");
+        const bool one_char = env && env[0] && !env[1];
+        const bool spill_local = !(one_char && env[0] == '0'), spill = one_char && env[0] == '1';
+        const int ID = FUSED_ITEM_ID_BITS;
+        HostWaveLists l16[2], l1[2], l16x2[2], l16f[2];
+        host_build_spill_lists(hc, false, gp * FW, FW, 4, spill, ID, &l16[0]);
+        host_build_spill_lists(hv, false, gp * FW, FW, 4, spill, ID, &l16[1]);
+        host_build_spill_lists(hc, true, gp * FW, FW, 8, spill, ID, &l1[0]);
+        host_build_spill_lists(hv, true, gp * FW, FW, 8, spill, ID, &l1[1]);
+        host_build_spill_lists(hv, false, gp * FW, FW, 4, spill_local, ID, &l16f[1]);
+        host_build_spill_lists(hc, false, gp * FW, FW, 4, spill_local, ID, &l16f[0], spill_local ? &l16f[1].load : nullptr);
+        host_build_spill_lists(hc, false, 2 * gp * FW, FW, 2, spill_local, ID, &l16x2[0]);
+        host_build_spill_lists(hv, false, 2 * gp * FW, FW, 2, spill_local, ID, &l16x2[1], spill_local ? &l16x2[0].load : nullptr);
         FusedOrient* dv[2] = {&A, &At};
         for (int k = 0; k < 2; ++k) {
-            HostWaveLists l16, l16x2, l1;
-            host_build_wave_lists(*ho[k], false, gp * FW, FW, 4, &l16);
-            host_build_wave_lists(*ho[k], false, 2 * gp * FW, FW, 2, &l16x2);
-            host_build_wave_lists(*ho[k], true, gp * FW, FW, 8, &l1);
+            if (!l16[k].id_bits || !l16x2[k].id_bits || !l1[k].id_bits || !l16f[k].id_bits)
+                return fail(MLLP_EINVAL, "fused path: too many items in one partition");
             FusedOrient& d = *dv[k];
-            d.L16 = l16.L; d.nw16 = l16.waves_per_part;
-            d.L16x2 = l16x2.L; d.nw16x2 = l16x2.waves_per_part;
-            d.L1 = l1.L; d.nw1 = l1.waves_per_part;
-            if ((rc = dev_alloc(g, l16.order.size(), &d.lst16, l16.order.data()))) return rc;
-            if ((rc = dev_alloc(g, l16x2.order.size(), &d.lst16x2, l16x2.order.data()))) return rc;
-            if ((rc = dev_alloc(g, l1.order.size(), &d.lst1, l1.order.data()))) return rc;
+            d.L16 = l16[k].L; d.nw16 = l16[k].waves_per_part;
+            d.L16x2 = l16x2[k].L; d.nw16x2 = l16x2[k].waves_per_part;
+            d.L1 = l1[k].L; d.nw1 = l1[k].waves_per_part;
+            d.L16f = l16f[k].L;
+            const HostWaveLists* built[4] = {&l16[k], &l1[k], &l16x2[k], &l16f[k]};
+            for (int w = 0; w < 4; ++w) {
+                int64_t n_items = 0;
+                for (int v : built[w]->order) n_items += v >= 0;
+                const int64_t info[5] = {n_items, built[w]->moved, built[w]->L, built[w]->max_load, built[w]->sum_load};
+                std::copy(info, info + 5, d.lst_info[w]);
+            }
+            if ((rc = dev_alloc(g, l16[k].order.size(), &d.lst16, l16[k].order.data()))) return rc;
+            if ((rc = dev_alloc(g, l16x2[k].order.size(), &d.lst16x2, l16x2[k].order.data()))) return rc;
+            if ((rc = dev_alloc(g, l1[k].order.size(), &d.lst1, l1[k].order.data()))) return rc;
+            if ((rc = dev_alloc(g, l16f[k].order.size(), &d.lst16f, l16f[k].order.data()))) return rc;
         }
     }
     if ((rc = dev_alloc(g, (size_t)g->M + 1, &A.sptr, hc.sptr.data(), 2))) return rc;
@@ -1690,10 +1722,11 @@
 
 int fused_grid(const mllp_graph* g) { return std::max(std::min(g->n_cu, STAT_BLOCKS_MAX) / NP, 1) * NP; }
 
-static FwdJob16 fwd_job16(const FusedOrient& o, const FusedModel& m, int c, const float* x_src, const float* x_dst, float* h) {
+static FwdJob16 fwd_job16(const FusedOrient& o, const FusedModel& m, int c, const float* x_src, const float* x_dst, float* h,
+                          bool layer2 = false) {
     const ConvWs& w = m.w.c[c];
     FwdJob16 J = {};
-    J.s = items_dev(o, 0);
+    J.s = items_dev(o, layer2 ? 3 : 0);
     J.x_src = x_src; J.x_dst = x_dst; J.D = w.derived; J.p = conv_params_at(conv_at(m.P, c), MODEL_CONV[c].cin);
     J.h = h; J.Z = w.Z; J.aux = w.aux;
     J.head = 0;
@@ -1728,8 +1761,8 @@
     {
         FwdLaunch16 L = {};
         L.n_jobs = 2;
-        L.job[0] = fwd_job16(g->FAt, m, CONV_2V, w.h1c, w.h1v, w.h2v);
-        L.job[1] = fwd_job16(g->FA, m, CONV_2C, w.h1v, w.h1c, w.h2c);
+        L.job[0] = fwd_job16(g->FAt, m, CONV_2V, w.h1c, w.h1v, w.h2v, true);
+        L.job[1] = fwd_job16(g->FA, m, CONV_2C, w.h1v, w.h1c, w.h2c, true);
         L.job[0].perm = g->perm_v; L.job[1].perm = g->perm_c;
         hipLaunchKernelGGL(fused_fwd16_kernel, dim3(G), dim3(FT), 0, s, L);
         if ((rc = check_launch("fused_fwd16 layer 2"))) return rc;
diff --git a/mllp_amd/csrc/host_graph.cpp b/mllp_amd/csrc/host_graph.cpp
--- a/mllp_amd/csrc/host_graph.cpp
+++ b/mllp_amd/csrc/host_graph.cpp
@@ -348,55 +348,168 @@
     for (int q = 0; q < FUSED_PARTS; ++q) o.row0[q + 1] += o.row0[q];
 }
 
+namespace {
+struct PartItems {
+    std::vector<std::pair<int64_t, int>> items;
+    std::vector<int64_t> slow, charge;
+};
+PartItems part_items(const HostFusedOrient& o, int q, bool scalar, int nw, int wpg, int gp, int nnz_per_step) {
+    PartItems p;
+    const int U = scalar ? 64 : 16, RG = U / 4;
+    const int e_base = std::max(nnz_per_step, 1), e_group = 4 * e_base, e_wave = (scalar ? 64 : 16) * e_base;
+    const FusedTiers& t = scalar ? o.t1[q] : o.t16[q];
+    const int n_gitems = (t.n_group + RG - 1) / RG, n_bitems = (t.n_base + U - 1) / U;
+    const int n_items = t.n_wave + n_gitems + n_bitems;
+    auto deg_of = [&](int rl) { const int k = o.row0[q] + rl; return (int64_t)o.sptr[(size_t)k + 1] - o.sptr[(size_t)k]; };
+    p.items.resize((size_t)n_items);
+    for (int it = 0; it < n_items; ++it) {
+        int64_t steps;
+        if (it < t.n_wave) steps = (deg_of(t.n_block + it) + e_wave - 1) / e_wave;
+        else if (it < t.n_wave + n_gitems) steps = (deg_of(t.n_block + t.n_wave + (it - t.n_wave) * RG) + e_group - 1) / e_group;
+        else steps = (deg_of(t.n_block + t.n_wave + t.n_group + (it - t.n_wave - n_gitems) * U) + e_base - 1) / e_base;
+        p.items[(size_t)it] = {FUSED_COST_ITEM + FUSED_COST_STEP * std::max<int64_t>(steps, 1), it};
+    }
+    std::stable_sort(p.items.begin(), p.items.end(), [](const auto& a, const auto& b) { return a.first > b.first; });
+    p.slow.assign((size_t)nw, 0);
+    p.charge.assign((size_t)nw, 0);
+    for (int w = 0; w < nw; ++w) {
+        const int bi = w / wpg;
+        const int n_rows = bi < gp && t.n_block > bi ? (t.n_block - bi + gp - 1) / gp : 0;
+        p.slow[(size_t)w] = 1000 + 95 * ((w % wpg) / 4);
+        p.charge[(size_t)w] = FUSED_COST_BLOCK_ROW * n_rows * p.slow[(size_t)w] / 1000;
+    }
+    return p;
+}
+int first_to_finish(const std::vector<int64_t>& load, const int64_t* slow, size_t w0, int nw, int64_t cost, int64_t* finish) {
+    int best = 0;
+    int64_t best_t = 0;
+    for (int w = 0; w < nw; ++w) {
+        const int64_t tw = load[w0 + (size_t)w] + cost * slow[w] / 1000;
+        if (w == 0 || tw < best_t) { best = w; best_t = tw; }
+    }
+    *finish = best_t;
+    return best;
+}
+void lists_finish(const std::vector<std::vector<int>>& lists, const std::vector<int64_t>& load, HostWaveLists* wl) {
+    wl->max_load = wl->sum_load = 0;
+    wl->L = 1;
+    for (size_t k = 0; k < lists.size(); ++k) {
+        wl->max_load = std::max(wl->max_load, load[k]);
+        wl->sum_load += load[k];
+        wl->L = std::max(wl->L, (int)lists[k].size());
+    }
+    wl->order.assign(lists.size() * (size_t)wl->L, -1);
+    for (size_t k = 0; k < lists.size(); ++k) std::copy(lists[k].begin(), lists[k].end(), wl->order.begin() + k * wl->L);
+}
+}
+
 void host_build_wave_lists(const HostFusedOrient& o, bool scalar, int waves_per_part, int waves_per_wg, int nnz_per_step,
                            HostWaveLists* out) {
     HostWaveLists& wl = *out;
     wl = HostWaveLists();
     const int nw = std::max(waves_per_part, 1), wpg = std::max(std::min(waves_per_wg, nw), 1), gp = std::max(nw / wpg, 1);
     wl.waves_per_part = nw;
-    const int U = scalar ? 64 : 16, RG = U / 4;
-    const int e_base = std::max(nnz_per_step, 1), e_group = 4 * e_base, e_wave = (scalar ? 64 : 16) * e_base;
     std::vector<std::vector<int>> lists((size_t)FUSED_PARTS * nw);
+    std::vector<int64_t> load((size_t)FUSED_PARTS * nw, 0);
     for (int q = 0; q < FUSED_PARTS; ++q) {
-        const FusedTiers& t = scalar ? o.t1[q] : o.t16[q];
-        const int n_gitems = (t.n_group + RG - 1) / RG, n_bitems = (t.n_base + U - 1) / U;
-        const int n_items = t.n_wave + n_gitems + n_bitems;
-        auto deg_of = [&](int rl) { const int k = o.row0[q] + rl; return (int64_t)o.sptr[(size_t)k + 1] - o.sptr[(size_t)k]; };
-        std::vector<std::pair<int64_t, int>> items((size_t)n_items);
-        for (int it = 0; it < n_items; ++it) {
-            int64_t steps;
-            if (it < t.n_wave) steps = (deg_of(t.n_block + it) + e_wave - 1) / e_wave;
-            else if (it < t.n_wave + n_gitems) steps = (deg_of(t.n_block + t.n_wave + (it - t.n_wave) * RG) + e_group - 1) / e_group;
-            else steps = (deg_of(t.n_block + t.n_wave + t.n_group + (it - t.n_wave - n_gitems) * U) + e_base - 1) / e_base;
-            items[(size_t)it] = {FUSED_COST_ITEM + FUSED_COST_STEP * std::max<int64_t>(steps, 1), it};
-        }
-        std::stable_sort(items.begin(), items.end(), [](const auto& a, const auto& b) { return a.first > b.first; });
-        std::vector<int64_t> load((size_t)nw, 0), slow((size_t)nw, 0);
-        for (int w = 0; w < nw; ++w) {
-            const int bi = w / wpg;
-            const int n_rows = bi < gp && t.n_block > bi ? (t.n_block - bi + gp - 1) / gp : 0;
-            slow[(size_t)w] = 1000 + 95 * ((w % wpg) / 4);
-            load[(size_t)w] = FUSED_COST_BLOCK_ROW * n_rows * slow[(size_t)w] / 1000;
-        }
-        for (const auto& itc : items) {
-            int best = 0;
-            int64_t best_t = 0;
-            for (int w = 0; w < nw; ++w) {
-                const int64_t tw = load[(size_t)w] + itc.first * slow[(size_t)w] / 1000;
-                if (w == 0 || tw < best_t) { best = w; best_t = tw; }
+        const PartItems p = part_items(o, q, scalar, nw, wpg, gp, nnz_per_step);
+        const size_t w0 = (size_t)q * nw;
+        std::copy(p.charge.begin(), p.charge.end(), load.begin() + w0);
+        for (const auto& itc : p.items) {
+            int64_t fin;
+            const int best = first_to_finish(load, p.slow.data(), w0, nw, itc.first, &fin);
+            lists[w0 + best].push_back(itc.second);
+            load[w0 + best] = fin;
+        }
+    }
+    lists_finish(lists, load, &wl);
+}
+
+void host_build_spill_lists(const HostFusedOrient& o, bool scalar, int waves_per_part, int waves_per_wg, int nnz_per_step,
+                            bool spill, int id_bits, HostWaveLists* out, const std::vector<int64_t>* before) {
+    HostWaveLists& wl = *out;
+    HostWaveLists own;
+    host_build_wave_lists(o, scalar, waves_per_part, waves_per_wg, nnz_per_step, &own);
+    wl = own;
+    const int nw = own.waves_per_part, wpg = std::max(std::min(waves_per_wg, nw), 1), gp = std::max(nw / wpg, 1);
+    PartItems p[FUSED_PARTS];
+    for (int q = 0; q < FUSED_PARTS; ++q) p[q] = part_items(o, q, scalar, nw, wpg, gp, nnz_per_step);
+    std::vector<int64_t> charge((size_t)FUSED_PARTS * nw, 0);
+    if (before && before->size() == charge.size()) charge = *before;
+    for (int q = 0; q < FUSED_PARTS; ++q)
+        for (int w = 0; w < nw; ++w) charge[(size_t)q * nw + w] += p[q].charge[(size_t)w];
+    std::vector<int64_t> load((size_t)FUSED_PARTS * nw, 0);
+    for (int q = 0; q < FUSED_PARTS; ++q) {
+        const size_t w0 = (size_t)q * nw;
+        std::copy(p[q].charge.begin(), p[q].charge.end(), load.begin() + w0);
+        for (const auto& itc : p[q].items) {
+            int64_t fin;
+            const int best = first_to_finish(load, p[q].slow.data(), w0, nw, itc.first, &fin);
+            load[w0 + best] = fin;
+        }
+        for (int w = 0; w < nw; ++w) load[w0 + w] += charge[w0 + w] - p[q].charge[(size_t)w];
+    }
+    wl.load = load;
+    wl.max_load = *std::max_element(load.begin(), load.end());
+    wl.sum_load = 0;
+    for (int64_t v : load) wl.sum_load += v;
+    own.max_load = wl.max_load;
+    wl.id_bits = 0;
+    if (id_bits < 1 || id_bits > FUSED_ITEM_ID_BITS) return;
+    for (int q = 0; q < FUSED_PARTS; ++q)
+        if ((int64_t)p[q].items.size() > ((int64_t)1 << id_bits)) return;
+    wl.id_bits = id_bits;
+    for (size_t k = 0; k < wl.order.size(); ++k)
+        if (wl.order[k] >= 0) wl.order[k] |= (int)(k / ((size_t)nw * wl.L)) << id_bits;
+    if (!spill) return;
+    int64_t part_sum[FUSED_PARTS] = {}, total = 0;
+    int n_pop = 0;
+    for (int q = 0; q < FUSED_PARTS; ++q) {
+        for (int w = 0; w < nw; ++w) part_sum[q] += load[(size_t)q * nw + w];
+        if (o.row0[q + 1] > o.row0[q]) { ++n_pop; total += part_sum[q]; }
+    }
+    std::vector<std::vector<int>> lists((size_t)FUSED_PARTS * nw);
+    if (n_pop < 2) return;
+    const int64_t n_wf = (int64_t)n_pop * nw;
+    const int64_t cap = total / n_wf + total / n_wf * FUSED_SPILL_SLACK_PM / 1000;
+    bool donor[FUSED_PARTS], receiver[FUSED_PARTS];
+    for (int q = 0; q < FUSED_PARTS; ++q) {
+        const bool pop = o.row0[q + 1] > o.row0[q];
+        donor[q] = pop && part_sum[q] * n_pop > total;
+        receiver[q] = pop && part_sum[q] * n_pop < total;
+    }
+    int64_t room[FUSED_PARTS];
+    for (int q = 0; q < FUSED_PARTS; ++q) room[q] = receiver[q] ? total / n_pop - part_sum[q] : 0;
+    struct Item { int64_t cost; int q, id; };
+    std::vector<Item> all;
+    for (int q = 0; q < FUSED_PARTS; ++q)
+        for (const auto& itc : p[q].items) all.push_back({itc.first, q, itc.second});
+    std::stable_sort(all.begin(), all.end(), [](const Item& a, const Item& b) { return a.cost > b.cost; });
+    load = charge;
+    int moved = 0;
+    for (const Item& it : all) {
+        int64_t fin;
+        int bq = it.q, bw = first_to_finish(load, p[bq].slow.data(), (size_t)bq * nw, nw, it.cost, &fin);
+        if (donor[it.q] && fin > cap) {
+            int rq = -1, rw = 0;
+            int64_t rt = 0;
+            for (int q = 0; q < FUSED_PARTS; ++q) {
+                if (room[q] < it.cost) continue;
+                int64_t t;
+                const int w = first_to_finish(load, p[q].slow.data(), (size_t)q * nw, nw, it.cost, &t);
+                if (rq < 0 || t < rt) { rq = q; rw = w; rt = t; }
             }
-            lists[(size_t)q * nw + best].push_back(itc.second);
-            load[(size_t)best] = best_t;
-        }
-        for (int w = 0; w < nw; ++w) {
-            wl.max_load = std::max(wl.max_load, load[(size_t)w]);
-            wl.sum_load += load[(size_t)w];
-            wl.L = std::max(wl.L, (int)lists[(size_t)q * nw + w].size());
-        }
-    }
-    wl.L = std::max(wl.L, 1);
-    wl.order.assign((size_t)FUSED_PARTS * nw * wl.L, -1);
-    for (size_t k = 0; k < lists.size(); ++k) std::copy(lists[k].begin(), lists[k].end(), wl.order.begin() + k * wl.L);
-}
-
-}
+            if (rq >= 0 && rt < fin) { bq = rq; bw = rw; fin = rt; room[rq] -= it.cost; ++moved; }
+        }
+        lists[(size_t)bq * nw + bw].push_back(it.id | it.q << id_bits);
+        load[(size_t)bq * nw + bw] = fin;
+    }
+    HostWaveLists sp;
+    lists_finish(lists, load, &sp);
+    if (moved == 0 || sp.max_load > own.max_load) return;
+    wl.order = sp.order; wl.L = sp.L; wl.max_load = sp.max_load; wl.sum_load = sp.sum_load;
+    wl.moved = moved;
+    wl.load = load;
+}
+
+}
diff --git a/mllp_amd/csrc/host_graph.h b/mllp_amd/csrc/host_graph.h
--- a/mllp_amd/csrc/host_graph.h
+++ b/mllp_amd/csrc/host_graph.h
@@ -64,8 +64,15 @@
     std::vector<int> order;
     int L = 0, waves_per_part = 0;
     int64_t max_load = 0, sum_load = 0;
+    int moved = 0;
+    int id_bits = 0;
+    std::vector<int64_t> load;
 };
 void host_build_wave_lists(const HostFusedOrient& o, bool scalar, int waves_per_part, int waves_per_wg, int nnz_per_step,
                            HostWaveLists* out);
+constexpr int FUSED_ITEM_ID_BITS = 28;
+constexpr int64_t FUSED_SPILL_SLACK_PM = 20;
+void host_build_spill_lists(const HostFusedOrient& o, bool scalar, int waves_per_part, int waves_per_wg, int nnz_per_step,
+                            bool spill, int id_bits, HostWaveLists* out, const std::vector<int64_t>* before = nullptr);
 
 }
diff --git a/mllp_amd/csrc/internal.h b/mllp_amd/csrc/internal.h
--- a/mllp_amd/csrc/internal.h
+++ b/mllp_amd/csrc/internal.h
@@ -129,8 +129,9 @@
     float* sax = nullptr;
     int row0[FUSED_NP + 1] = {};
     FusedTiersDev t16[FUSED_NP], t1[FUSED_NP];
-    int* lst16 = nullptr; int* lst16x2 = nullptr; int* lst1 = nullptr;
-    int L16 = 0, L16x2 = 0, L1 = 0, nw16 = 0, nw16x2 = 0, nw1 = 0;
+    int* lst16 = nullptr; int* lst16x2 = nullptr; int* lst1 = nullptr; int* lst16f = nullptr;
+    int L16 = 0, L16x2 = 0, L1 = 0, L16f = 0, nw16 = 0, nw16x2 = 0, nw1 = 0;
+    int64_t lst_info[4][5] = {};
 };
 constexpr int SCRATCH_NS = 20;
 
diff --git a/mllp_amd/graph.py b/mllp_amd/graph.py
--- a/mllp_amd/graph.py
+++ b/mllp_amd/graph.py
@@ -609,6 +609,11 @@
         self._folded = None if param_gen is None else (params.data_ptr(), params._version, param_gen + 1)
         return loss, logits, grads
 
+    def fused_lists(self, orientation, kind):
+        out = (c_int64 * 5)()
+        _lib.check(_lib.lib().mllp_graph_fused_lists(self._h, int(orientation), int(kind), out))
+        return dict(zip(("items", "moved", "L", "max_load", "sum_load"), (int(v) for v in out)))
+
     def small_step_fits(self):
         fits = ctypes.c_int()
         _lib.check(_lib.lib().mllp_gnn_small_step_fits(self._h, ctypes.byref(fits)))
```

Result: no change. 290,200 instances/s, median of 3 (+0.4%).
